# mycorrhiza-inc/fugu

Measured on AMD Instinct MI355X. Metric: queries/sec + p50 latency, 10M-doc Zipf corpus, 3-term AND, top-100, higher is better.
Workload: dtype u32+f32; 1 GPU; 3-term AND, BM25 top-100, 10M-doc Zipf s=1.0 corpus per namespace, batch 1024; n_docs=10000000, vocab=1048576, batch=1024, k=100, terms=3, namespaces=1, parallelism=namespace-shard x1

## Files before the change

fugu_amd/csrc/fg_host.h:

```cpp
#pragma once
#include <hip/hip_runtime.h>

#include <algorithm>
#include <atomic>
#include <chrono>
#include <condition_variable>
#include <functional>
#include <cstdint>
#include <map>
#include <memory>
#include <mutex>
#include <string>
#include <thread>
#include <vector>

#include "../../include/fugu.h"
#include "fg_internal.h"
#include "fg_pool.h"
#include "fg_trace.h"

namespace fgh {

int fail(int code, const char* fmt, ...);
int hw_threads(int req);
// ... 279 lines not shown

namespace fgh {
struct ChunkTables {
  const uint32_t *d_sc_tf = nullptr, *d_sc_tl = nullptr, *d_bk_tf = nullptr, *d_bk_tl = nullptr, *d_bk_e0 = nullptr,
                 *d_bk_e1 = nullptr, *d_kt_terms = nullptr, *d_kt_tiny = nullptr;
  const uint64_t *d_sc_e0 = nullptr, *d_sc_e1 = nullptr;
  uint32_t n_scb = 0, n_ktiny = 0;
  const uint32_t* d_tterm = nullptr;
  uint32_t n_tterm = 0, n_tiles = 0;
  const uint32_t *d_kb_terms = nullptr, *d_kb_chunk0 = nullptr, *d_kc_big = nullptr, *d_kc_start = nullptr;
  uint32_t n_sc = 0, n_bk = 0, n_kt = 0, n_kbig = 0, n_kchunks = 0;
};

struct IndexStructure : ChunkTables {
  uint32_t n_docs = 0, n_terms = 0;
  bool has_name = false;
  uint64_t n_postings = 0, dir_entries = 0, tile_entries = 0;
  uint32_t n_rank = 0;
  uint64_t n_srank_words = 0;
  bool has_positions = false;
  SharedVec<uint32_t> tmap;
  uint32_t n_vocab = 0;
  SharedVec<uint64_t> off;
  SharedVec<uint32_t> df_text, df_name;
  SharedVec<uint32_t> first_doc, last_doc;
  std::shared_ptr<const std::vector<uint32_t>> h_doc;
  SharedVec<uint32_t> tmeta;
  SharedVec<uint32_t> dir_off;
  uint64_t tot_local[2] = {0, 0};
  uint32_t n_fterms = 0;
  uint64_t tot_f_local = 0;
  SharedVec<uint64_t> foff;
  SharedVec<uint32_t> df_facet_local, ffirst, flast;
  std::shared_ptr<DevAllocs> smem;
  std::shared_ptr<ScorePool> spool;
  uint64_t struct_bytes = 0;
  fg::DevIndex d{};
};

struct IndexBounds {
  std::shared_ptr<ScoreBlock> sblock;
  const float* ktop = nullptr;
  const float* tmaxs = nullptr;
  SharedVec<float> wb_text, wb_name;
  float cache_b[512];
  SharedVec<uint32_t> h_alive_b;
  SharedVec<uint64_t> dtab_map;
  uint64_t dtab_bytes = 0;
  SharedVec<uint64_t> dtab8_map;
  uint64_t dtab8_bytes = 0;
  uint64_t device_bytes = 0;
};

inline uint32_t doctab_lead() {
  const char* e = getenv("FUGU_DOCTAB_LEAD");
  return e && *e ? (uint32_t)std::max(0l, atol(e)) : fg::kDocTabLead;
}

inline uint32_t doctab_slot(const IndexBounds& b, uint32_t t) {
  const auto it = std::lower_bound(b.dtab_map.begin(), b.dtab_map.end(), (uint64_t)t << 32);
  return it != b.dtab_map.end() && (uint32_t)(*it >> 32) == t ? (uint32_t)*it + 1u : 0u;
}

inline uint32_t doctab8_lead() {
  const char* e = getenv("FUGU_DOCTAB8_LEAD");
  return e && *e ? (uint32_t)std::max(0l, atol(e)) : fg::kDocTab8Lead;
}

inline bool conj_hist_thr() {
  const char* e = getenv("FUGU_CONJ_HIST_THR");
  return !(e && *e) || atol(e) != 0;
}

inline float hist_lo_div() {
  const char* e = getenv("FUGU_HIST_LO_DIV");
  const double v = e && *e ? atof(e) : 0.0;
  return v >= 1.0 ? (float)v : 256.0f;
}

inline uint32_t doctab8_slot(const IndexBounds& b, uint32_t t) {
  const auto it = std::lower_bound(b.dtab8_map.begin(), b.dtab8_map.end(), (uint64_t)t << 32);
  return it != b.dtab8_map.end() && (uint32_t)(*it >> 32) == t ? (uint32_t)*it + 1u : 0u;
}
}

struct fg_index : fgh::IndexStructure, fgh::IndexBounds {
  std::atomic<int> refs{1};
  int dev = 0;
  uint32_t n_dense = 0;
  uint64_t tot[2] = {0, 0};
  uint64_t n_stats = 0;
  float avgdl[2] = {0, 0};
  float cache[512];
  fgh::SharedVec<float> w_text, w_name;
  fgh::SharedVec<float> idf_text, idf_name;
  uint64_t tot_f = 0;
  float avgdl_f = 0.0f, cache_f1 = 0.0f;
  std::vector<uint32_t> df_facet;
  std::vector<float> fscore;
  fgh::SharedVec<uint32_t> h_alive;
  uint32_t n_dead = 0;
  bool same_stats = true;
  double cup[2] = {1, 1}, cdn[2] = {1, 1};
  std::shared_ptr<void> alive_hold;
  std::shared_ptr<const std::vector<float>> kth_floor;
  DevAllocs mem;
  std::shared_ptr<WsPool> pool;
  std::shared_ptr<PinnedPool> pinned;
};

struct fg_plan {
  fg_index* ix = nullptr;
  uint32_t nq = 0, k = 0, total_chunks = 0, n_scan = 0, nq_batch = 0, n_segs = 1;
  std::vector<fg_index*> segs;
  int mode = FG_MODE_AND;
  fg::DevPlan d{};
  fg::DevIndex d0{};
  void* ws = nullptr;
  size_t ws_got = 0;
  float* own_score = nullptr;
  uint32_t* own_doc = nullptr;
  uint32_t* own_n = nullptr;
  void* zero_region = nullptr;
  size_t zero_bytes = 0;
  size_t diag_words = 0;
  uint64_t ws_bytes = 0;
  DevAllocs mem;
  hipStream_t last_stream = nullptr;
  bool profile = false;
  std::vector<hipEvent_t> pending;
  double ms[2] = {0, 0};
  uint32_t n_prof = 0;
  ~fg_plan() {
    for (hipEvent_t e : pending) (void)hipEventDestroy(e);
    if (pin) {
      (void)hipSetDevice(ix->dev);
      (void)hipStreamSynchronize(up_stream);
    }
    if (ws) {
      if (last_stream_used) {
        (void)hipSetDevice(ix->dev);
        (void)hipStreamSynchronize(last_stream);
      }
      if (pin) ix->pinned->put(pin, pin_n);
      ix->pool->put(ws, ws_got);
    }
    if (!ipc_maps.empty()) {
      (void)hipSetDevice(ix->dev);
      for (void* m : ipc_maps) (void)hipIpcCloseMemHandle(m);
    }
    if (ix) fg_index_release(ix);
    for (fg_index* x : segs) fg_index_release(x);
  }
  bool last_stream_used = false;
  std::vector<uint32_t> h_lo, h_hi;
  std::vector<uint8_t> h_any;
  double part_next = 0.0;
  bool zeroed = false;
  void* pin = nullptr;
  size_t pin_n = 0;
  std::vector<void*> ipc_maps;
  hipStream_t up_stream = hipStreamPerThread;
};

extern "C" int fg_plan_seed_thr0(fg_plan* p, const float* score, uint32_t n);

namespace fgh {
inline uint32_t local_term(const fg_index* ix, uint32_t t) {
  if (ix->tmap.empty()) return t;
  const auto it = std::lower_bound(ix->tmap.begin(), ix->tmap.end(), t);
  return it != ix->tmap.end() && *it == t ? (uint32_t)(it - ix->tmap.begin()) : 0xFFFFFFFFu;
}
void term_ratio(const fg_index* ix, uint32_t t, float* rdn, float* rup);
float term_max_now(const fg_index* ix, uint32_t t);
float term_max_scaled(const fg_index* ix, uint32_t t, float rup);
float term_kth_now(const fg_index* ix, uint32_t t, uint32_t k, bool with_floor);

struct Bins { uint32_t lo, hi, shift; };
Bins union_bins(uint32_t lo, uint32_t hi);
int plan_create_multi(fg_index* const* ixs, uint32_t n_segs, const fg_query_batch* q, uint32_t k, fg_plan** out,
                      bool sync, hipStream_t up);
void run_parallel(uint32_t n, const std::function<void(uint32_t)>& f);

hipStream_t build_stream();
bool on_background();
uint32_t bg_grid_cap(int dev);
uint8_t fieldnorm_id(uint64_t n);
void bm25_weights(uint64_t Ns, const uint32_t* df_t, const uint32_t* df_n, uint32_t V, std::vector<float>& wt,
                  std::vector<float>& wn, std::vector<float>& it, std::vector<float>& in);
void set_stats(fg_index* ix, uint64_t Ns, const uint64_t tot2[2], const uint32_t* df_t, const uint32_t* df_n,
               uint64_t tot_f, const uint32_t* df_f, const Weights* wts);
void relate_stats(fg_index* ix);
int dev_upload_bytes(DevAllocs& m, const void* src, size_t n, void** out, uint64_t* bytes);
template <class T>
int dev_upload(DevAllocs& m, const T* src, size_t n, T** out, uint64_t* bytes) {
  return dev_upload_bytes(m, src, n * sizeof(T), reinterpret_cast<void**>(out), bytes);
}
struct UploadBatch {
  struct E { const void* src; size_t bytes; void** out; };
  std::vector<E> es;
  size_t total = 0;
  static size_t slot(size_t bytes) { return (std::max<size_t>(bytes, 16) + 16 + 255) & ~size_t(255); }
  template <class T>
  void add(const T* src, size_t n, T** out) {
    es.push_back(E{src, n * sizeof(T), reinterpret_cast<void**>(out)});
    total += slot(n * sizeof(T));
  }
  int commit(DevAllocs& m, uint64_t* bytes);
};
struct BuildTrace {
  bool on = false;
  std::chrono::steady_clock::time_point t;
  void start();
  void mark(const char* what);
};
extern thread_local BuildTrace g_bt;
}
```

fugu_amd/csrc/fg_internal.h:

```cpp
#pragma once
#include <algorithm>
#include <cstdint>
#include <initializer_list>

#include <hip/hip_runtime.h>

namespace fg {

constexpr uint32_t kBlock = 128;
#ifndef FG_BUCKET
#define FG_BUCKET 4
#endif
constexpr uint32_t kBucketTarget = FG_BUCKET;
constexpr uint32_t kThreads = 256;
#ifndef FG_ITEMS
#define FG_ITEMS 8
#endif
constexpr uint32_t kItems = FG_ITEMS;
constexpr uint32_t kChunk = kThreads * kItems;
constexpr uint32_t kWaveSpan = kChunk / 4;
constexpr uint32_t kMaxTerms = 16;
constexpr uint32_t kMaxK = 1024;
#ifndef FG_FINALCAP
#define FG_FINALCAP 4096
#endif
constexpr uint32_t kFinalCap = FG_FINALCAP;
static_assert(FG_FINALCAP >= 1024, "the final sort runs in place for up to kMaxK keys");
#ifndef FG_RANK_DIV
#define FG_RANK_DIV 16384
#endif
#ifndef FG_RANK_GIB
#define FG_RANK_GIB 64
#endif
constexpr uint32_t kRankDiv = FG_RANK_DIV;
constexpr uint64_t kRankBudget = (uint64_t)FG_RANK_GIB << 30;
#ifndef FG_RANK_FACTOR
#define FG_RANK_FACTOR 4.0
#endif
constexpr double kRankFactor = FG_RANK_FACTOR;
#ifndef FG_RANK_PLAIN_DIV
#define FG_RANK_PLAIN_DIV 32
#endif
constexpr uint32_t kRankPlainDiv = FG_RANK_PLAIN_DIV;
constexpr uint32_t kMaxDense = 32767;
#ifndef FG_DOCTAB_DIV
#define FG_DOCTAB_DIV 4
#endif
#ifndef FG_DOCTAB_LEAD
#define FG_DOCTAB_LEAD 8
#endif
constexpr uint32_t kDocTabDiv = FG_DOCTAB_DIV;
constexpr uint32_t kDocTabLead = FG_DOCTAB_LEAD;
constexpr uint32_t kDocTabFrac = 8;
constexpr uint32_t kDocTabMax = 64;
constexpr uint32_t kDocTabMinDocs = 8192;
#ifndef FG_DOCTAB8_DIV
#define FG_DOCTAB8_DIV 0
#endif
#ifndef FG_DOCTAB8_LEAD
#define FG_DOCTAB8_LEAD 8
#endif
constexpr uint32_t kDocTab8Div = FG_DOCTAB8_DIV;
constexpr uint32_t kDocTab8Lead = FG_DOCTAB8_LEAD;
constexpr uint32_t kRankChunkWords = 2048;
#ifndef FG_DISJ_GPQ
#define FG_DISJ_GPQ 64
#endif
constexpr uint32_t kGroupsPerQuery = FG_DISJ_GPQ;
#ifndef FG_DISJ_SPREAD
#define FG_DISJ_SPREAD 16
#endif
constexpr uint32_t kDisjSmallSpread = FG_DISJ_SPREAD;
#ifndef FG_GPQ
#define FG_GPQ 4
#endif
constexpr uint32_t kConjGroupsPerQuery = FG_GPQ;
#ifndef FG_MAXGROUP
#define FG_MAXGROUP 16
#endif
constexpr uint32_t kMaxGroup = FG_MAXGROUP;
#ifndef FG_HIST_BITS
#define FG_HIST_BITS 10
#endif
constexpr uint32_t kHistBits = 11;
constexpr uint32_t kHistBins = 1u << kHistBits;
constexpr uint32_t kConjHistBits = FG_HIST_BITS;
#ifndef FG_TILE_SHIFT
#define FG_TILE_SHIFT 12
#endif
constexpr uint32_t kDisjTileShift = FG_TILE_SHIFT;
#ifndef FG_DISJ_ROUND
#define FG_DISJ_ROUND 512
#endif
#ifndef FG_DISJ_HBITS
#define FG_DISJ_HBITS 9
#endif
#ifndef FG_DISJ_WAVES
#define FG_DISJ_WAVES 5
#endif
#ifndef FG_DISJ_G
#define FG_DISJ_G 1
#endif
#ifndef FG_DISJ_MAXGROUP
#define FG_DISJ_MAXGROUP 32
#endif
constexpr uint32_t kDisjMaxGroup = FG_DISJ_MAXGROUP;
constexpr uint32_t kDisjMaxPairs = 256;
constexpr uint32_t kNumTopK = 5;
constexpr uint32_t kTopKs[kNumTopK] = {1, 10, 20, 100, 1000};
constexpr uint32_t kNumLadderExtra = 9;
constexpr uint32_t kLadderExtra[kNumLadderExtra] = {2, 3, 5, 13, 25, 50, 125, 250, 500};
constexpr uint32_t kNumLadder = kNumTopK + kNumLadderExtra;
constexpr uint32_t kLadderKs[kNumLadder] = {1, 2, 3, 5, 10, 13, 20, 25, 50, 100, 125, 250, 500, 1000};

constexpr uint32_t kPhraseMaxGroup = 4;
constexpr uint32_t kMaxFacetClauses = 8;
constexpr uint32_t kFmaskChunk = 8192;
constexpr uint32_t kScanMaxGroup = 32;

constexpr uint32_t kModeAnd = 0;
constexpr uint32_t kModeOr = 1;

constexpr uint32_t kQBins = 512;

__host__ __device__ inline uint32_t qbin(uint64_t key, uint32_t lo, uint32_t sh) {
  const uint32_t bits = (uint32_t)(key >> 32);
  if (bits < lo) return kQBins;
  const uint32_t b = (bits - lo) >> sh;
  return b < kQBins - 1 ? b : kQBins - 1;
}

__host__ __device__ inline uint64_t hist_kth_edge(const uint32_t* c, uint32_t n, uint32_t first, uint32_t before,
                                                  uint32_t K, uint32_t lo, uint32_t sh) {
  for (uint32_t i = 0; i < n; ++i) {
    if (before < K && before + c[i] >= K) return (uint64_t)(lo + ((first - i) << sh)) << 32;
    before += c[i];
  }
  return 0ull;
}

__host__ __device__ inline uint32_t qm_terms(uint32_t qm) { return qm & 0xFFu; }
__host__ __device__ inline uint32_t qm_must(uint32_t qm) { return (qm >> 8) & 0xFFu; }
__host__ __device__ inline uint32_t qm_not(uint32_t qm) { return (qm >> 16) & 0xFFu; }
__host__ __device__ inline uint32_t qm_pack(uint32_t m, uint32_t nm, uint32_t nx) { return m | (nm << 8) | (nx << 16); }
__host__ __device__ inline uint32_t qm_phrase(uint32_t distinct, uint32_t n) { return distinct | (n << 24); }
__host__ __device__ inline uint32_t qm_phrase_terms(uint32_t qm) { return qm >> 24; }

__host__ __device__ inline uint32_t rank_word(uint32_t d) { return d >> 5; }
__host__ __device__ inline uint32_t rank_pos(uint64_t x, uint32_t d) {
#if defined(__HIP_DEVICE_COMPILE__)
  asm volatile("" : "+v"(d));
#endif
  const uint32_t b = d & 31u;
  if (!((x >> b) & 1ull)) return 0xFFFFFFFFu;
  const uint32_t below = (uint32_t)x & ((1u << b) - 1u);
#if defined(__HIP_DEVICE_COMPILE__)
  return (uint32_t)(x >> 32) + (uint32_t)__popc(below);
#else
  return (uint32_t)(x >> 32) + (uint32_t)__builtin_popcount(below);
#endif
}

__host__ __device__ inline uint32_t srank_block(uint32_t d) { return d >> 10; }
__host__ __device__ inline uint32_t srank_index(uint64_t e, uint32_t d) {
#if defined(__HIP_DEVICE_COMPILE__)
  asm volatile("" : "+v"(d));
#endif
  const uint32_t w = (d >> 5) & 31u;
  const uint32_t below = (uint32_t)e & ((1u << w) - 1u);
#if defined(__HIP_DEVICE_COMPILE__)
  const uint32_t i = (uint32_t)(e >> 32) + (uint32_t)__popc(below);
#else
  const uint32_t i = (uint32_t)(e >> 32) + (uint32_t)__builtin_popcount(below);
#endif
  return ((e >> w) & 1ull) ? i : 0u;
}

__host__ __device__ inline float q8_step(float M) { return M * (1.0f / 255.0f); }
__host__ __device__ inline float q8_bound(uint32_t q, float M) { return q >= 255u ? M : (float)q * q8_step(M); }
__host__ __device__ inline uint32_t quant8(float s, float M) {
  const float st = q8_step(M);
  if (!(st > 0.0f) || !(s < M)) return 255u;
  uint32_t q = (uint32_t)fminf(254.0f, ceilf(s / st));
  while (q < 255u && q8_bound(q, M) < s) ++q;
  return q;
}
constexpr uint32_t kSubShift = 9;

__host__ __device__ inline uint32_t meta_slot(uint32_t meta) { return (meta >> 16) & 0x7FFFu; }
__host__ __device__ inline bool meta_rank(uint32_t meta) { return (meta >> 31) != 0; }

constexpr uint32_t kTfEsc = 255;
__host__ __device__ inline uint32_t tfn_pack(uint32_t tf, uint32_t fn) { return (fn << 8) | (tf < kTfEsc ? tf : kTfEsc); }
struct DevIndex {
  const uint32_t* doc;
  const float* psc;
  const uint16_t* tfn;
  const uint16_t* tfn_name;
  const uint64_t* esc_pos;
  const uint32_t* esc_tf;
  const float* cache;
  const uint64_t* off;
  const uint32_t* dir;
  const uint32_t* dir_off;
  const uint32_t* tmeta;
  const uint64_t* rank;
  const uint64_t* srank;
  const uint64_t* srank_w;
  const float* tmaxs;
  const uint32_t* alive;
  const float* bmax;
  const float* tmax;
  const uint32_t* toff;
  const uint32_t* tdir;
  const uint64_t* tsub;
  const float* cmax;
  const uint32_t* coff;
  const float* dtab;
  const uint8_t* dtab8;
  const uint32_t* fdoc;
  const uint64_t* foff;
  uint64_t n_esc;
  uint32_t n_docs;
  uint32_t n_terms;
  uint32_t has_name;
  uint32_t n_fterms;
  uint32_t rank_words;
  uint32_t n_prank;
  uint32_t srank_blocks;
  uint32_t dtab_stride;
  uint32_t dtab8_stride;
  const uint64_t* fwd_off;
  const uint32_t* fwd;
  const uint64_t* fwd_off_name;
  const uint32_t* fwd_name;
};
constexpr uint32_t kFwdNone = 0xFFFFFFFFu;

__host__ __device__ inline uint32_t tf_escaped(const uint64_t* esc_pos, const uint32_t* esc_tf, uint64_t n, uint64_t p) {
  uint64_t lo = 0, hi = n;
  while (lo < hi) {
    const uint64_t mid = (lo + hi) >> 1;
    if (esc_pos[mid] < p) lo = mid + 1; else hi = mid;
  }
  return lo < n ? esc_tf[lo] : 0u;
}

__host__ __device__ inline float field_score(uint32_t tf, uint32_t fn, float w, const float* cache) {
  const float f = (float)tf;
  return w * (f / (f + cache[fn]));
}

struct ProbeDesc {
  uint32_t base_lo;
  uint32_t bytes;
  uint32_t sc_lo;
  uint32_t sc_bytes;
  uint32_t aux_lo;
  uint32_t hi;
  uint32_t kind;
  uint32_t ub;
};
static_assert(sizeof(ProbeDesc) == 32, "one s_load_dwordx8");
constexpr uint32_t kPdDir = 1u << 12;
constexpr uint32_t kPdWide = 1u << 13;
constexpr uint32_t kPdSparse = 1u << 14;
constexpr uint32_t kPdTab = 1u << 15;
constexpr uint32_t kPdBound = 1u << 6;
constexpr uint32_t kPdMaxBytes = 0x80000000u;
constexpr uint32_t kPdDead8 = 0xFFFFFFF8u, kPdDead4 = 0xFFFFFFFCu, kPdDead2 = 0xFFFFFFFEu;
// ... 30 lines not shown
  if (lead) {
    base = (uint64_t)(uintptr_t)(ix.doc + t.off);
    bytes = df * 4;
    kind = 0;
  } else if (!qt && t.tab && ix.dtab && probe_uses_table(ix.n_docs, df, lead_df, tab_lead)) {
    base = (uint64_t)(uintptr_t)(ix.dtab + (uint64_t)(t.tab - 1) * ix.dtab_stride);
    bytes = (uint64_t)ix.n_docs * 4;
    kind = kPdTab;
  } else if (slot && slot <= ix.n_prank) {
    base = (uint64_t)(uintptr_t)(ix.rank + (uint64_t)(slot - 1) * ix.rank_words);
    bytes = (uint64_t)ix.rank_words * 8;
    kind = 5u;
  } else if (slot) {
    base = (uint64_t)(uintptr_t)(ix.srank + (uint64_t)(slot - 1 - ix.n_prank) * ix.srank_blocks);
    bytes = (uint64_t)ix.srank_blocks * 8;
    kind = 10u | kPdSparse;
  } else {
    const uint32_t B = t.meta & 0xFFu, S = (t.meta >> 8) & 0xFFu;
    base = (uint64_t)(uintptr_t)(ix.dir + t.dir_off);
    bytes = ((((uint64_t)(ix.n_docs ? ix.n_docs - 1 : 0)) >> B) + 2) * 4;
    aux = (uint64_t)(uintptr_t)(ix.doc + t.off);
    kind = (B & 0x3Fu) | ((S & 0x3Fu) << 6) | kPdDir;
  }
  const bool tab = (kind & kPdTab) != 0;
  const uint64_t sc = tab ? base : qt ? (uint64_t)(uintptr_t)(ix.tfn + t.off) : (uint64_t)(uintptr_t)(ix.psc + t.off);
  const uint64_t sc_bytes = tab ? bytes : df * (qt ? 2 : 4);
  if (bytes > kPdMaxBytes || sc_bytes > kPdMaxBytes) kind |= kPdWide;
  ProbeDesc p;
  p.base_lo = (uint32_t)base;
  p.bytes = (uint32_t)std::min<uint64_t>(bytes, 0xFFFFFFFFull);
  p.sc_lo = (uint32_t)sc;
  p.sc_bytes = (uint32_t)std::min<uint64_t>(sc_bytes, 0xFFFFFFFFull);
  p.aux_lo = (uint32_t)aux;
  p.hi = (uint32_t)((base >> 32) & 0xFFFFu) | (uint32_t)((sc >> 32) & 0xFFFFu) << 16;
  p.kind = kind | (uint32_t)((aux >> 32) & 0xFFFFu) << 16;
  union { float f; uint32_t u; } c;
  c.f = ub;
  p.ub = c.u;
  return p;
}

inline bool probe_uses_bound(uint64_t n_docs, uint64_t df, uint64_t lead_df, uint32_t tab8_lead) {
  return lead_df * 128 >= n_docs * tab8_lead || df * 2 >= n_docs;
}

inline bool probe_desc_bound(const DevIndex& ix, ProbeDesc& lead, ProbeDesc& p1, uint32_t tab8, float M, bool deferred,
                             bool qt, uint64_t df, uint64_t lead_df, uint32_t tab8_lead = kDocTab8Lead) {
  if (!deferred || qt || !tab8 || !ix.dtab8 || !(M > 0.0f)) return false;
  if (p1.kind & (kPdDir | kPdWide)) return false;
  if (!probe_uses_bound(ix.n_docs, df, lead_df, tab8_lead)) return false;
  const uint64_t a = (uint64_t)(uintptr_t)(ix.dtab8 + (uint64_t)(tab8 - 1) * ix.dtab8_stride);
  p1.aux_lo = (uint32_t)a;
  p1.kind = (p1.kind & 0xFFFFu) | kPdBound | (uint32_t)((a >> 32) & 0xFFFFu) << 16;
  union { float f; uint32_t u; } c;
  c.f = M;
  lead.aux_lo = c.u;
  return true;
}

struct DevFilters {
  uint32_t n_filters;
  uint32_t n_chunks;
  const uint32_t* q_filter;
  const uint32_t* f_shift;
  const uint64_t* f_woff;
  const float* f_tab;
  const float* f_max;
  const uint32_t* ch_filter;
  const uint32_t* ch_clause;
  const uint32_t* ch_term;
  const uint32_t* ch_start;
  const uint32_t* f_seg;
  uint32_t* fmask;
};

__host__ __device__ inline uint32_t filter_bits(const uint32_t* mask, uint32_t shift, uint32_t d) {
  const uint32_t bit = d << shift;
  return (mask[bit >> 5] >> (bit & 31)) & ((1u << (1u << shift)) - 1u);
}

constexpr uint32_t kMaxPeers = 15;
constexpr uint32_t kOptConjHistThr = 1u;

struct DevPlan {
  uint32_t n_queries;
  uint32_t total_chunks;
  uint32_t k;
  uint32_t n_conj;
  const uint32_t* q_m;
  const uint32_t* q_terms;
  const uint32_t* q_lead_df;
  const uint32_t* work_q;
  const uint32_t* work_c;
  const uint32_t* work_n;
  const uint64_t* cand_off;
  const uint64_t* q_thr0;
  const float* q_ub;
  const ProbeDesc* q_probe;
  const float* q_wt;
  const float* q_wn;
  const float* q_rup;
  const uint32_t* q_hlo;
  const uint32_t* q_hsh;
  uint64_t* thresh;
  uint32_t* hist;
  uint64_t pub_mask;
  uint32_t* cand_cnt;
  uint64_t* cand_keys;
  uint64_t* diag;
  uint32_t feat;
  uint32_t opts;
  uint32_t n_single;
  uint32_t n_scan;
  uint32_t n_phrase;
  const uint32_t* q_pterm;
  const uint32_t* q_ppos;
  const DevIndex* segs;
  uint32_t seg_nq;
  uint32_t n_segs;
  const uint32_t* seg_base;
  DevFilters f;
  uint32_t n_peers;
  uint32_t* peer_hist[kMaxPeers];
  uint64_t* peer_thr[kMaxPeers];
};

__host__ __device__ inline uint32_t slot_query(const DevPlan& pl, uint32_t v) {
  return pl.seg_nq ? v % pl.seg_nq : v;
}

constexpr uint32_t kCountItems = 8;
constexpr uint32_t kCountChunk = kThreads * kCountItems;
constexpr uint32_t kCountFacetChunk = kFmaskChunk;
constexpr uint32_t kCountFacetItems = kCountFacetChunk / kThreads;
constexpr uint32_t kCountWordChunk = 2048;
constexpr uint32_t kCountTile = 64;
constexpr uint32_t kCountText = 0, kCountFacet = 1, kCountFill = 2;
struct DevCount {
  uint32_t nq;
  uint32_t q0;
  uint32_t words;
  uint32_t n_count;
  uint32_t n_fchunks, n_items, n_cchunks;
  uint32_t* match;
  uint32_t* fbits;
  unsigned long long* total;
  unsigned long long* count;
  const uint32_t* fc_filter;
  const uint32_t* fc_term;
  const uint32_t* fc_start;
  const uint32_t* w_q;
  const uint32_t* w_kind;
  const uint32_t* w_term;
  const uint32_t* w_start;
  const uint32_t* q_m;
  const uint32_t* q_terms;
  const uint32_t* q_filter;
  const uint32_t* cc_j;
  const uint32_t* cc_term;
  const uint32_t* cc_start;
};

constexpr uint32_t kDiagPerWg = 16;

__host__ __device__ inline uint64_t make_key(float score, uint32_t doc) {
  union { float f; uint32_t u; } c;
  c.f = score;
  return ((uint64_t)c.u << 32) | (uint64_t)(0xFFFFFFFFu - doc);
}
__host__ __device__ inline float key_score(uint64_t k) {
  union { float f; uint32_t u; } c;
  c.u = (uint32_t)(k >> 32);
  return c.f;
}
__host__ __device__ inline uint32_t key_doc(uint64_t k) { return 0xFFFFFFFFu - (uint32_t)k; }

constexpr uint32_t kScoreChunk = kChunk;
constexpr uint32_t kBucketChunk = 2048;
static_assert(kScoreChunk == kChunk, "DevIndex::cmax: a k_score chunk is a k_conj lead chunk");
struct ScoreJob {
  const uint32_t* doc;
  const uint16_t* tfn;
  const uint16_t* tfn_name;
  const uint64_t* esc_pos;
  const uint32_t* esc_tf;
  uint64_t n_esc;
  const uint64_t* off;
  const uint32_t* dir;
  const uint32_t* dir_off;
  const uint32_t* tmeta;
  const uint32_t* toff;
  const uint32_t* alive;
  const float* w_text;
  const float* w_name;
  const float* cache;
  float* psc;
  float* bmax;
// ... 12 lines not shown
  const uint64_t* sc_e0;
  const uint64_t* sc_e1;
  const uint32_t* bk_tf;
  const uint32_t* bk_tl;
  const uint32_t* bk_e0;
  const uint32_t* bk_e1;
  uint32_t n_terms;
  uint32_t grid_cap;
  uint64_t n_dir;
  const uint32_t* kt_tiny;
  uint32_t n_tiny;
  const uint32_t* kt_terms;
  const uint32_t* kb_terms;
  const uint32_t* kb_chunk0;
  const uint32_t* kc_big;
  const uint32_t* kc_start;
  uint64_t* kc_keys;
  uint32_t* kc_cnt;
  uint32_t* kb_stat;
  uint32_t n_big;
};
#ifndef FG_KTOP_CHUNK
#define FG_KTOP_CHUNK 32768
#endif
constexpr uint32_t kKtopChunk = FG_KTOP_CHUNK;
constexpr uint32_t kKtopTiny = 64;
constexpr uint32_t kPackTerms = 256;

struct DocTabJob {
  const uint32_t* doc;
  const float* psc;
  float* tab;
  uint64_t stride;
  uint32_t n;
  uint32_t df[kDocTabMax];
  uint64_t off[kDocTabMax];
};

struct DocTab8Job {
  const uint32_t* doc;
  const float* psc;
  const float* tmaxs;
  uint8_t* tab;
  uint64_t stride;
  uint32_t n;
  uint32_t term[kDocTabMax];
  uint32_t df[kDocTabMax];
  uint64_t off[kDocTabMax];
};

constexpr uint32_t kFwdSlices = 1024;
constexpr uint32_t kFwdShort = 16;
constexpr uint32_t kFwdErrOrder = 1u;
constexpr uint32_t kFwdErrNone = 2u;
constexpr uint32_t kFwdErrRow = 4u;
struct FwdJob {
  const uint32_t* doc;
  const uint64_t* off;
  const uint16_t* tf;
  const uint32_t* pos;
  uint64_t* poff;
  uint32_t* len;
  uint64_t* part;
  uint32_t* err;
  unsigned long long* filled;
  uint64_t* fwd_off;
  uint32_t* fwd;
  uint64_t n_fwd;
  uint64_t n_post;
  uint32_t n_docs;
  const uint32_t* sc_tf;
  const uint32_t* sc_tl;
  const uint64_t* sc_e0;
  const uint64_t* sc_e1;
  uint32_t n_chunks;
  uint32_t grid_cap;
};
hipError_t launch_fwd_rows(const FwdJob& j, hipStream_t s, hipEvent_t* ev = nullptr);
hipError_t launch_fwd_fill(const FwdJob& j, hipStream_t s, hipEvent_t* ev = nullptr);

hipError_t launch_conj(const DevIndex& ix, const DevPlan& pl, hipStream_t s);
hipError_t launch_disj(const DevIndex& ix, const DevPlan& pl, hipStream_t s, uint32_t first = 0,
                       uint32_t count = 0xFFFFFFFFu);
hipError_t launch_fmask(const DevIndex& ix, const DevPlan& pl, hipStream_t s);
hipError_t launch_scan(const DevIndex& ix, const DevPlan& pl, hipStream_t s);
hipError_t launch_phrase(const DevIndex& ix, const DevPlan& pl, hipStream_t s);
hipError_t launch_final(const DevPlan& pl, float* out_score, uint32_t* out_doc, uint32_t* out_n, hipStream_t s,
                        uint32_t* out_shard = nullptr);
hipError_t launch_count(const DevIndex& ix, const DevCount& c, hipStream_t s, hipEvent_t* ev = nullptr);
hipError_t launch_rank(const uint32_t* doc, const uint64_t* slot_base, const uint32_t* slot_n, uint32_t n_slots,
                       uint32_t n_words, uint64_t* out, hipStream_t s);
hipError_t launch_score(const ScoreJob& j, uint32_t n_chunks, hipStream_t s);
hipError_t launch_doctab(const DocTabJob& j, uint32_t grid_cap, hipStream_t s);
hipError_t launch_doctab8(const DocTab8Job& j, uint32_t grid_cap, hipStream_t s);
hipError_t launch_bucket(const ScoreJob& j, uint32_t n_chunks, uint32_t n_docs, hipStream_t s);
hipError_t launch_tsub(const ScoreJob& j, uint32_t n_docs, hipStream_t s);
hipError_t launch_ktop(const ScoreJob& j, uint32_t n_terms, uint32_t n_chunks, uint32_t n_big, hipStream_t s);
hipError_t launch_copy32(uint32_t* dst, const uint32_t* src, uint64_t n, uint32_t grid_cap, hipStream_t s);
hipError_t launch_merge(uint32_t n_shards, uint32_t n_queries, uint32_t k, const float* score, const uint32_t* doc,
                        const uint32_t* n, float* out_score, uint32_t* out_doc, uint32_t* out_shard, uint32_t* out_n,
                        hipStream_t s);

}
```

fugu_amd/csrc/fugu.cpp:

```cpp
#include <hip/hip_runtime.h>
#include <sched.h>

#include <algorithm>
#include <atomic>
#include <chrono>
#include <cmath>
#include <condition_variable>
#include <deque>
#include <functional>
#include <cstdarg>
#include <cstdio>
#include <cstring>
#include <map>
#include <memory>
#include <mutex>
#include <string>
#include <thread>
#include <vector>

#include "../../include/fugu.h"
#include "fg_host.h"
#include "fg_internal.h"

namespace {
// ... 665 lines not shown
  for (uint32_t s = 0; s < n_shards; ++s)
    if (!ladders[s]) return fail(FG_EINVAL, "NULL ladder of shard %u", s);
  constexpr uint32_t L = fg::kNumLadder;
  fgh::parallel_dynamic(n_terms, fgh::hw_threads(0), 8192, [&](int, uint32_t b, uint32_t e) {
    std::vector<std::pair<float, uint32_t>> c;
    std::vector<uint32_t> cur(n_shards);
    for (uint32_t t = b; t < e; ++t) {
      c.clear();
      for (uint32_t s = 0; s < n_shards; ++s)
        for (uint32_t l = 0; l < L; ++l) {
          const float v = ladders[s][(size_t)t * L + l];
          if (v > 0.0f) c.emplace_back(v, s * L + l);
        }
      std::sort(c.begin(), c.end(), [](const auto& x, const auto& y) { return x.first > y.first; });
      std::fill(cur.begin(), cur.end(), 0u);
      uint64_t total = 0;
      float res[fg::kNumTopK] = {0, 0, 0, 0, 0};
      uint32_t next = 0;
      for (size_t i = 0; i < c.size() && next < fg::kNumTopK;) {
        const float x = c[i].first;
        for (; i < c.size() && c[i].first == x; ++i) {
          const uint32_t s = c[i].second / L, K = fg::kLadderKs[c[i].second % L];
          if (K > cur[s]) {
            total += K - cur[s];
            cur[s] = K;
          }
        }
        for (; next < fg::kNumTopK && total >= fg::kTopKs[next]; ++next) res[next] = x;
      }
      for (uint32_t k = 0; k < fg::kNumTopK; ++k) out[(size_t)t * fg::kNumTopK + k] = res[k];
    }
  });
  return FG_OK;
}

int fg_index_set_kth_floor(fg_index* ix, const float* floor, uint32_t n_terms) {
  if (!ix) return fail(FG_EINVAL, "NULL index");
  std::shared_ptr<const std::vector<float>> f;
  if (floor) {
    if (n_terms != ix->n_vocab) return fail(FG_EINVAL, "floor of %u terms for a snapshot of %u", n_terms, ix->n_vocab);
    if (ix->tmap.empty()) {
      f = std::make_shared<const std::vector<float>>(floor, floor + (size_t)n_terms * fg::kNumTopK);
    } else {
      std::vector<float> v((size_t)ix->n_terms * fg::kNumTopK);
      for (uint32_t t = 0; t < ix->n_terms; ++t)
        std::copy(floor + (size_t)ix->tmap[t] * fg::kNumTopK, floor + (size_t)(ix->tmap[t] + 1) * fg::kNumTopK,
                  v.begin() + (size_t)t * fg::kNumTopK);
      f = std::make_shared<const std::vector<float>>(std::move(v));
    }
  }
  std::atomic_store(&ix->kth_floor, f);
  return FG_OK;
}

int fg_index_bm25(const fg_index* ix, uint32_t term, float* w_text, float* w_name, float* cache512) {
  if (!ix) return fail(FG_EINVAL, "NULL index");
  term = fgh::local_term(ix, term);
  if (term < ix->n_terms) {
    if (w_text) *w_text = ix->w_text[term];
    if (w_name) *w_name = ix->w_name[term];
  } else {
    if (w_text) *w_text = bm25_weight(0, ix->n_stats);
    if (w_name) *w_name = bm25_weight(0, ix->n_stats);
  }
  if (cache512) std::memcpy(cache512, ix->cache, sizeof ix->cache);
  return FG_OK;
}

static int execute_impl(fg_plan* p, hipStream_t s, float* os, uint32_t* od, uint32_t* on, uint32_t* oshard,
                        double from = 0.0, double to = 1.0) {
  HIPCHK(hipSetDevice(p->ix->dev));
  const bool first = from <= 0.0, last = to >= 1.0;
  if (first && !p->d.n_peers) {
    if (p->zeroed) p->zeroed = false;
    else HIPCHK(hipMemsetAsync(p->zero_region, 0, p->zero_bytes, s));
  }
  hipEvent_t ev[3] = {};
  if (p->profile) {
    for (auto& e : ev) HIPCHK(hipEventCreate(&e));
    HIPCHK(hipEventRecord(ev[0], s));
  }
  if (first && p->d.f.n_chunks) HIPCHK(fg::launch_fmask(p->d0, p->d, s));
  if (first && p->d.n_conj) HIPCHK(fg::launch_conj(p->d0, p->d, s));
  const uint32_t nd = p->d.total_chunks - p->d.n_conj;
  const uint32_t a = first ? 0u : (uint32_t)std::min<double>(nd, std::llround(from * nd));
  const uint32_t b = last ? nd : (uint32_t)std::min<double>(nd, std::llround(to * nd));
  if (b > a) HIPCHK(fg::launch_disj(p->d0, p->d, s, a, b - a));
  if (last && p->d.n_scan) HIPCHK(fg::launch_scan(p->d0, p->d, s));
  if (last && p->d.n_phrase) HIPCHK(fg::launch_phrase(p->d0, p->d, s));
  if (p->profile) HIPCHK(hipEventRecord(ev[1], s));
  if (last) HIPCHK(fg::launch_final(p->d, os, od, on, s, oshard));
  if (p->profile) {
    HIPCHK(hipEventRecord(ev[2], s));
    p->pending.insert(p->pending.end(), ev, ev + 3);
  }
  p->last_stream = s;
  p->last_stream_used = true;
  return FG_OK;
}

int fg_plan_execute(fg_plan* p, void* stream, float* d_out_score, uint32_t* d_out_doc, uint32_t* d_out_n) {
  if (!p) return fail(FG_EINVAL, "NULL plan");
  return execute_impl(p, static_cast<hipStream_t>(stream), d_out_score ? d_out_score : p->own_score,
                      d_out_doc ? d_out_doc : p->own_doc, d_out_n ? d_out_n : p->own_n, nullptr);
}

int fg_plan_execute_merged(fg_plan* p, void* stream, float* d_out_score, uint32_t* d_out_doc, uint32_t* d_out_shard,
                           uint32_t* d_out_n) {
  if (!p || !d_out_score || !d_out_doc || !d_out_shard || !d_out_n) return fail(FG_EINVAL, "bad arguments");
  if (p->n_segs < 2 || !p->d.seg_base)
    return fail(FG_EUNSUPPORTED, "not a multi-snapshot plan over < 2^32 docs (use fg_plan_execute + fg_merge_shards)");
  return execute_impl(p, static_cast<hipStream_t>(stream), d_out_score, d_out_doc, d_out_n, d_out_shard);
}

int fg_plan_execute_part(fg_plan* p, void* stream, double from, double to, float* d_out_score, uint32_t* d_out_doc,
                         uint32_t* d_out_shard, uint32_t* d_out_n) {
  if (!p) return fail(FG_EINVAL, "NULL plan");
  if (!(from >= 0.0 && from < to && to <= 1.0)) return fail(FG_EINVAL, "part [%g, %g) not inside [0, 1)", from, to);
  if (from > 0.0 && from != p->part_next)
    return fail(FG_EINVAL, "part [%g, %g) does not continue the plan's sweep (next part starts at %g)", from, to,
                p->part_next);
  if (d_out_shard && (p->n_segs < 2 || !p->d.seg_base))
    return fail(FG_EUNSUPPORTED, "merged select: not a multi-snapshot plan over < 2^32 docs");
  if (d_out_shard && (!d_out_score || !d_out_doc || !d_out_n)) return fail(FG_EINVAL, "merged select needs every output");
  const int rc = execute_impl(p, static_cast<hipStream_t>(stream), d_out_score ? d_out_score : p->own_score,
                              d_out_doc ? d_out_doc : p->own_doc, d_out_n ? d_out_n : p->own_n, d_out_shard, from, to);
  if (rc == FG_OK) p->part_next = to >= 1.0 ? 0.0 : to;
  return rc;
}

int fg_plan_set_peers(fg_plan* p, fg_plan* const* peers, uint32_t n) {
  if (!p || (n && !peers)) return fail(FG_EINVAL, "bad arguments");
  if (n > FG_MAX_PEERS) return fail(FG_EUNSUPPORTED, "%u peers (> FG_MAX_PEERS = %d)", n, FG_MAX_PEERS);
  for (uint32_t i = 0; i < n; ++i) {
    const fg_plan* o = peers[i];
    if (!o || o == p) return fail(FG_EINVAL, "peer %u: NULL or the plan itself", i);
    if (o->nq_batch != p->nq_batch || o->k != p->k) return fail(FG_EINVAL, "peer %u plans another batch or k", i);
    if (o->h_lo.size() != p->h_lo.size()) return fail(FG_EINVAL, "peer %u: another number of query slots", i);
    if (o->ix->dev != p->ix->dev) {
      int ok = 0;
      HIPCHK(hipDeviceCanAccessPeer(&ok, p->ix->dev, o->ix->dev));
      if (!ok) return fail(FG_EUNSUPPORTED, "device %d cannot reach peer %u's device %d", p->ix->dev, i, o->ix->dev);
    }
  }
  p->d.n_peers = n;
  for (uint32_t i = 0; i < n; ++i) {
    p->d.peer_hist[i] = peers[i]->d.hist;
    p->d.peer_thr[i] = peers[i]->d.thresh;
  }
  if (n) p->d.pub_mask = 0xFFFFFFFF00000000ull;
  return FG_OK;
}

int fg_plan_ipc_export(const fg_plan* p, fg_plan_ipc* out) {
  if (!p || !out) return fail(FG_EINVAL, "bad arguments");
  const char* ws = static_cast<const char*>(p->ws);
  const char* th = reinterpret_cast<const char*>(p->d.thresh);
  const char* hi = reinterpret_cast<const char*>(p->d.hist);
  if (th < ws || th >= ws + p->ws_got || hi < ws || hi >= ws + p->ws_got)
    return fail(FG_EUNSUPPORTED, "the plan's thresholds are another plan's (linked): export that plan");
  std::memset(out, 0, sizeof *out);
  hipIpcMemHandle_t h;
  HIPCHK(hipSetDevice(p->ix->dev));
  HIPCHK(hipIpcGetMemHandle(&h, p->ws));
  static_assert(sizeof h <= sizeof out->handle, "fg_plan_ipc::handle");
  std::memcpy(out->handle, &h, sizeof h);
// ... 82 lines not shown
}

int fg_plan_hist_copy(fg_plan* p, void* stream, uint32_t* d_buf, int into_plan) {
  if (!p || !d_buf) return fail(FG_EINVAL, "bad arguments");
  HIPCHK(hipSetDevice(p->ix->dev));
  const size_t bytes = 4ull * p->nq_batch * fg::kQBins;
  hipStream_t s = static_cast<hipStream_t>(stream);
  if (into_plan) HIPCHK(hipMemcpyAsync(p->d.hist, d_buf, bytes, hipMemcpyDeviceToDevice, s));
  else HIPCHK(hipMemcpyAsync(d_buf, p->d.hist, bytes, hipMemcpyDeviceToDevice, s));
  return FG_OK;
}

int fg_plan_results(fg_plan* p, float* out_score, uint32_t* out_doc, uint32_t* out_n) {
  if (!p) return fail(FG_EINVAL, "NULL plan");
  HIPCHK(hipSetDevice(p->ix->dev));
  const size_t nk = (size_t)p->nq * p->k;
  hipStream_t s = p->last_stream;
  const char* first = reinterpret_cast<const char*>(p->own_score);
  const size_t span = reinterpret_cast<const char*>(p->own_n) + 4ull * p->nq - first;
  if (span <= (4ull << 20)) {
    PinnedLease pin(*p->ix->pinned, span);
    if (pin.p) {
      HIPCHK(hipMemcpyAsync(pin.p, first, span, hipMemcpyDeviceToHost, s));
      HIPCHK(hipStreamSynchronize(s));
      const char* h = static_cast<const char*>(pin.p);
      if (out_score) std::memcpy(out_score, h, 4 * nk);
      if (out_doc) std::memcpy(out_doc, h + (reinterpret_cast<const char*>(p->own_doc) - first), 4 * nk);
      if (out_n) std::memcpy(out_n, h + (reinterpret_cast<const char*>(p->own_n) - first), 4ull * p->nq);
      return FG_OK;
    }
  }
  if (out_score) HIPCHK(hipMemcpyAsync(out_score, p->own_score, 4 * nk, hipMemcpyDeviceToHost, s));
  if (out_doc) HIPCHK(hipMemcpyAsync(out_doc, p->own_doc, 4 * nk, hipMemcpyDeviceToHost, s));
  if (out_n) HIPCHK(hipMemcpyAsync(out_n, p->own_n, 4ull * p->nq, hipMemcpyDeviceToHost, s));
  HIPCHK(hipStreamSynchronize(s));
  return FG_OK;
}

int fg_plan_info_get(const fg_plan* p, fg_plan_info* o) {
  if (!p || !o) return fail(FG_EINVAL, "bad arguments");
  o->n_queries = p->nq;
  o->k = p->k;
  o->total_chunks = p->total_chunks;
  o->workspace_bytes = p->ws_bytes;
  return FG_OK;
}

int fg_plan_profile(fg_plan* p, int enable) {
  if (!p) return fail(FG_EINVAL, "NULL plan");
  p->profile = enable != 0;
  return FG_OK;
}

int fg_plan_kernel_ms(fg_plan* p, double* ms_out, uint32_t* n_out) {
  if (!p) return fail(FG_EINVAL, "NULL plan");
  HIPCHK(hipSetDevice(p->ix->dev));
  for (size_t i = 0; i + 2 < p->pending.size(); i += 3) {
    HIPCHK(hipEventSynchronize(p->pending[i + 2]));
    for (int kx = 0; kx < 2; ++kx) {
      float ms = 0;
      HIPCHK(hipEventElapsedTime(&ms, p->pending[i + kx], p->pending[i + kx + 1]));
      p->ms[kx] += ms;
    }
    p->n_prof++;
  }
  for (hipEvent_t e : p->pending) (void)hipEventDestroy(e);
  p->pending.clear();
  if (ms_out) for (int kx = 0; kx < 2; ++kx) ms_out[kx] = p->ms[kx];
  if (n_out) *n_out = p->n_prof;
  p->ms[0] = p->ms[1] = 0;
  p->n_prof = 0;
  return FG_OK;
}

int fg_plan_diag(fg_plan* p, uint64_t* out, size_t n_words, uint32_t* cand_cnt) {
  if (!p) return fail(FG_EINVAL, "NULL plan");
  HIPCHK(hipSetDevice(p->ix->dev));
  HIPCHK(hipStreamSynchronize(p->last_stream));
  if (cand_cnt) HIPCHK(hipMemcpy(cand_cnt, p->d.cand_cnt, 4ull * p->nq, hipMemcpyDeviceToHost));
  if (out && n_words) {
    if (!p->d.diag) return fail(FG_EUNSUPPORTED, "not a diagnostic build (-DFG_DIAG)");
    HIPCHK(hipMemcpy(out, p->d.diag, 8 * std::min(n_words, p->diag_words), hipMemcpyDeviceToHost));
  }
  return FG_OK;
}

int fg_plan_seed_thr0(fg_plan* p, const float* score, uint32_t n) {
  if (!p || !score || n != p->nq_batch) return fail(FG_EINVAL, "bad arguments");
  std::vector<uint64_t> t((size_t)p->nq);
  for (uint32_t v = 0; v < p->nq; ++v) {
    const float s = score[v % p->nq_batch];
    t[v] = s > 0.0f ? fg::make_key(s, 0xFFFFFFFFu) : 0ull;
  }
  HIPCHK(hipSetDevice(p->ix->dev));
  if (p->pin) HIPCHK(hipStreamSynchronize(p->up_stream));
  if (p->last_stream_used) HIPCHK(hipStreamSynchronize(p->last_stream));
  if (p->nq) HIPCHK(hipMemcpy(const_cast<uint64_t*>(p->d.q_thr0), t.data(), 8ull * p->nq, hipMemcpyHostToDevice));
  return FG_OK;
}

int fg_plan_destroy(fg_plan* p) {
  delete p;
  return FG_OK;
}

int fg_plan_link(fg_plan* const* plans, uint32_t n) {
  if (!plans || n == 0) return fail(FG_EINVAL, "bad arguments");
  fg_plan* o = plans[0];
  for (uint32_t i = 0; i < n; ++i) {
    if (!plans[i]) return fail(FG_EINVAL, "NULL plan");
    if (plans[i]->nq != o->nq || plans[i]->k != o->k) return fail(FG_EINVAL, "linked plans differ in batch or k");
    if (plans[i]->ix->dev != o->ix->dev) return fail(FG_EINVAL, "linked plans live on different devices");
    if (plans[i]->n_segs > 1) return fail(FG_EUNSUPPORTED, "a multi-snapshot plan already shares its thresholds");
  }
  const uint32_t nq = o->nq;
  std::vector<uint32_t> lo(nq, 0), sh(nq, 0);
  for (uint32_t q = 0; q < nq; ++q) {
    uint32_t l = 0, h = 0;
    for (uint32_t i = 0; i < n; ++i) {
      l = std::max(l, plans[i]->h_lo[q]);
      h = std::max(h, plans[i]->h_hi[q]);
    }
    const fgh::Bins b = fgh::union_bins(l, h);
    lo[q] = b.lo;
    sh[q] = b.shift;
  }
  HIPCHK(hipSetDevice(o->ix->dev));
  for (uint32_t i = 0; i < n; ++i) {
    fg_plan* p = plans[i];
    if (nq) {
      HIPCHK(hipMemcpy(const_cast<uint32_t*>(p->d.q_hlo), lo.data(), 4ull * nq, hipMemcpyHostToDevice));
      HIPCHK(hipMemcpy(const_cast<uint32_t*>(p->d.q_hsh), sh.data(), 4ull * nq, hipMemcpyHostToDevice));
    }
    p->h_lo = lo;
    for (uint32_t q = 0; q < nq; ++q) p->h_hi[q] = std::max(p->h_hi[q], lo[q]);
    p->d.thresh = o->d.thresh;
    p->d.hist = o->d.hist;
    p->d.pub_mask = 0xFFFFFFFF00000000ull;
  }
  return FG_OK;
}

int fg_search_batch(fg_index* ix, const fg_query_batch* q, uint32_t k, float* out_score, uint32_t* out_doc,
                    uint32_t* out_n) {
  fg_plan* p = nullptr;
  int rc = plan_create_multi(&ix, 1, q, k, &p, false, hipStreamPerThread);
  if (rc) return rc;
  std::unique_ptr<fg_plan> guard(p);
  if ((rc = fg_plan_execute(p, hipStreamPerThread, nullptr, nullptr, nullptr))) return rc;
  return fg_plan_results(p, out_score, out_doc, out_n);
}

int fg_merge_shards(uint32_t n_shards, uint32_t n_queries, uint32_t k, const float* d_score, const uint32_t* d_doc,
                    const uint32_t* d_n, float* d_out_score, uint32_t* d_out_doc, uint32_t* d_out_shard,
                    uint32_t* d_out_n, void* stream) {
  if (n_shards == 0 || n_shards > 64 || k == 0 || !d_score || !d_doc || !d_n || !d_out_score || !d_out_doc || !d_out_n)
    return fail(FG_EINVAL, "bad arguments");
  HIPCHK(fg::launch_merge(n_shards, n_queries, k, d_score, d_doc, d_n, d_out_score, d_out_doc, d_out_shard, d_out_n,
                          static_cast<hipStream_t>(stream)));
  return FG_OK;
}

class ShardWorkers {
 public:
  static ShardWorkers& get() {
    static ShardWorkers* w = new ShardWorkers(std::max(8, std::min(64, hw_threads(0))));
// ... 257 lines not shown
```

fugu_amd/csrc/kernels.hip:

```cpp
#include <hip/hip_runtime.h>

#include "fg_internal.h"

namespace fg {
namespace {

constexpr uint32_t kInvalid = 0xFFFFFFFFu;

#ifdef FG_DIAG
#define FG_STAMP(base, slot, val)                                     \
  do {                                                                \
    if (threadIdx.x == 0 && pl.diag) pl.diag[(base) * kDiagPerWg + (slot)] = (val); \
  } while (0)
#define FG_NOW() __builtin_amdgcn_s_memrealtime()
#else
#define FG_STAMP(base, slot, val) do { } while (0)
#define FG_NOW() 0ull
#endif

__device__ inline uint32_t lane_id() { return threadIdx.x & 63; }

typedef const __attribute__((address_space(4))) DevIndex ConstDevIndex;
__device__ inline DevIndex seg_index(const DevPlan& pl, uint32_t s) {
#if defined(__HIP_DEVICE_COMPILE__)
  return ((ConstDevIndex*)pl.segs)[s];
#else
  return pl.segs[s];
#endif
}
__device__ inline uint32_t wave_id() { return threadIdx.x >> 6; }

typedef const __attribute__((address_space(4))) ProbeDesc ConstProbeDesc;
__device__ inline ProbeDesc probe_load(const ProbeDesc* p) {
#if defined(__HIP_DEVICE_COMPILE__)
  return *(ConstProbeDesc*)(uintptr_t)p;
#else
  return *p;
#endif
}
#if defined(__HIP_DEVICE_COMPILE__)
typedef __amdgpu_buffer_rsrc_t BufRsrc;
__device__ inline BufRsrc pd_rsrc(uint64_t base, uint32_t bytes) {
  return __builtin_amdgcn_make_buffer_rsrc((void*)(uintptr_t)base, 0, (int)bytes, 0x00020000);
}
__device__ inline uint64_t buf_u64(BufRsrc r, uint32_t off) {
  const auto v = __builtin_amdgcn_raw_buffer_load_b64(r, (int)off, 0, 0);
  return (uint64_t)v[0] | ((uint64_t)v[1] << 32);
}
__device__ inline uint32_t buf_u32(BufRsrc r, uint32_t off) { return __builtin_amdgcn_raw_buffer_load_b32(r, (int)off, 0, 0); }
__device__ inline uint32_t buf_u16(BufRsrc r, uint32_t off) { return __builtin_amdgcn_raw_buffer_load_b16(r, (int)off, 0, 0); }
__device__ inline uint32_t buf_u8(BufRsrc r, uint32_t off) { return __builtin_amdgcn_raw_buffer_load_b8(r, (int)off, 0, 0); }
#else
typedef int BufRsrc;
__device__ inline BufRsrc pd_rsrc(uint64_t, uint32_t) { return 0; }
__device__ inline uint64_t buf_u64(BufRsrc, uint32_t) { return 0; }
__device__ inline uint32_t buf_u32(BufRsrc, uint32_t) { return 0; }
__device__ inline uint32_t buf_u16(BufRsrc, uint32_t) { return 0; }
__device__ inline uint32_t buf_u8(BufRsrc, uint32_t) { return 0; }
#endif

template <uint32_t N>
__device__ inline void loads_in_flight(uint32_t (&v)[N]) {
#if defined(__HIP_DEVICE_COMPILE__)
  if constexpr (N == 8)
    asm volatile("" : "+v"(v[0]), "+v"(v[1]), "+v"(v[2]), "+v"(v[3]), "+v"(v[4]), "+v"(v[5]), "+v"(v[6]), "+v"(v[7]));
  else if constexpr (N == 4)
    asm volatile("" : "+v"(v[0]), "+v"(v[1]), "+v"(v[2]), "+v"(v[3]));
#endif
}

__device__ inline float inflate_bound(float x) { return x * 1.00000762939453125f; }

__device__ inline uint64_t rank_word_of(const DevIndex& ix, uint32_t slot, uint32_t d) {
  if (slot <= ix.n_prank) return ix.rank[(size_t)(slot - 1) * ix.rank_words + rank_word(d)];
  return ix.srank_w[srank_index(ix.srank[(size_t)(slot - 1 - ix.n_prank) * ix.srank_blocks + srank_block(d)], d)];
}
__device__ inline const uint64_t* rank_base(const DevIndex& ix, uint32_t slot, uint32_t& shift) {
  if (slot <= ix.n_prank) {
    shift = 5u;
    return ix.rank + (size_t)(slot - 1) * ix.rank_words;
  }
  shift = 10u;
  return ix.srank + (size_t)(slot - 1 - ix.n_prank) * ix.srank_blocks;
}


constexpr uint32_t kFName = 1, kFEsc = 2, kFQt = 4;
template <uint32_t kF>
__device__ inline uint32_t tfn_load(const DevIndex& ix, uint64_t p) {
  uint32_t v = ix.tfn[p];
  if ((kF & kFName) && ix.tfn_name) v |= (uint32_t)ix.tfn_name[p] << 16;
  return v;
}
template <uint32_t kF>
__device__ inline float tfn_score_fast(uint32_t v, float wt, float wn, const float* ct, const float* cn) {
  const uint32_t tt = v & 0xFFu, tn = (kF & kFName) ? (v >> 16) & 0xFFu : 0u;
  float s = 0.0f;
  if (tt) s += field_score(tt, (v >> 8) & 0xFFu, wt, ct);
  if (tn) s += field_score(tn, v >> 24, wn, cn);
  return s;
}
template <uint32_t kF>
__device__ inline bool tfn_escaped(uint32_t v) {
  return (kF & kFEsc) && ((v & 0xFFu) == kTfEsc || ((v >> 16) & 0xFFu) == kTfEsc);
}
__device__ inline float tfn_score(const DevIndex& ix, uint64_t p, uint32_t v, float wt, float wn, const float* ct,
                                  const float* cn) {
  uint32_t tt = v & 0xFFu, tn = (v >> 16) & 0xFFu;
  if (tt == kTfEsc || tn == kTfEsc) {
    const uint32_t e = tf_escaped(ix.esc_pos, ix.esc_tf, ix.n_esc, p);
    if (tt == kTfEsc) tt = e & 0xFFFFu;
    if (tn == kTfEsc) tn = e >> 16;
  }
  float s = 0.0f;
  if (tt) s += field_score(tt, (v >> 8) & 0xFFu, wt, ct);
  if (tn) s += field_score(tn, v >> 24, wn, cn);
  return s;
}

__device__ inline float term_bound(const DevIndex& ix, uint32_t meta, uint32_t toff, uint32_t dir_off, uint32_t d) {
  return toff != 0xFFFFFFFFu ? ix.tmax[toff + (d >> kDisjTileShift)] : ix.bmax[dir_off + (d >> (meta & 0xFFu))];
}

__device__ inline bool term_has_doc(const DevIndex& ix, uint32_t meta, uint64_t base, uint32_t dir_off, uint32_t d) {
  const uint32_t slot = meta_slot(meta);
  if (slot) return (rank_word_of(ix, slot, d) >> (d & 31u)) & 1ull;
  const uint32_t* __restrict__ dir = ix.dir + dir_off;
  const uint32_t b = d >> (meta & 0xFFu);
  uint32_t lo = dir[b], hi = dir[b + 1];
  const uint32_t* __restrict__ di = ix.doc + base;
  while (lo < hi) {
    const uint32_t mid = (lo + hi) >> 1;
    if (di[mid] < d) lo = mid + 1; else hi = mid;
  }
  return lo < dir[b + 1] && di[lo] == d;
}

__device__ inline uint32_t posting_pos(const DevIndex& ix, uint32_t t, uint32_t d) {
  const uint32_t meta = ix.tmeta[t], slot = meta_slot(meta);
// ... 675 lines not shown
      bool keep = (live >> j) & 1u;
      uint64_t key = 0;
      if (keep && ix.alive && !((ix.alive[doc[j] >> 5] >> (doc[j] & 31)) & 1u)) keep = false;
      if (keep) {
        float s = (nm == 1 && !has_opt) ? s0[j] : s0[j] + acc_o[j];
        if (fmask) s = s + ftab[filter_bits(fmask, fshift, doc[j])];
        key = make_key(s, doc[j]);
        keep = key >= thr;
      }
      wave_append(keep, key, sh.buf, &sh.n_buf, kBuf);
    }
    }
    __syncthreads();
    uint32_t n = sh.n_buf;
    uint64_t tp2 = FG_NOW();
    (void)tp2;
    if (defer) {
      const uint32_t nd = min(sh.n_dq, kDeferCap);
      if (nd >= kDeferFlush || (cc + 1 == nc && nd > 0)) {
        if (n > kTrunc) {
          local_T = truncate_topk(sh, n, K);
          if (local_T > thr_k) thr_k = local_T;
        }
        flush_deferred<kF>(ix, sh, probes, terms, qwt, qwn, m, thr_k, nd);
        __syncthreads();
        n = sh.n_buf;
        if (tid == 0) sh.n_dq = 0;
      }
    }
    if (n > kTrunc || (cc + 1 == nc && n > K)) {
      local_T = truncate_topk(sh, n, K);
      if (local_T > thr_k) thr_k = local_T;
    }
    uint64_t tp3 = FG_NOW();
    (void)tp3;
#ifdef FG_DIAG
    t_probe += tp1 - tp0; t_keys += tp2 - tp1; t_sel += tp3 - tp2; n_app += n;
#endif
    if (tid == 0) {
      if (local_T > sh.thr) sh.thr = local_T;
      pend = atomicMax(gthr, (unsigned long long)(local_T & pl.pub_mask));
    }
  }
  if (tid == 0 && pend > sh.thr) sh.thr = pend;
  {
    static_assert((1u << kConjHistBits) >= kQBins, "LDS bins");
    const uint32_t n = min(sh.n_buf, kBuf);
    for (uint32_t b = tid; b < kQBins; b += kThreads) sh.hist[b] = 0;
    __syncthreads();
    for (uint32_t i = tid; i < n; i += kThreads) {
      const uint32_t b = qbin(sh.buf[i], h_lo, h_sh);
      if (b < kQBins) atomicAdd(&sh.hist[b], 1u);
    }
    __syncthreads();
    if (!kSingle && (pl.opts & kOptConjHistThr)) {
      const uint64_t cur = sh.thr;
      const uint32_t cb = qbin(cur, h_lo, h_sh);
      const uint64_t edge = hist_add_kth(sh.hist, gh, pl, ql, cur && cb < kQBins ? cb : 0u, K, h_lo, h_sh, sh.scratch);
      if (tid == 0 && edge > cur) {
        sh.thr = edge;
        atomicMax(gthr, (unsigned long long)(edge & pl.pub_mask));
      }
    } else {
      hist_add(sh.hist, gh, pl, ql);
    }
  }
  if (tid == 0) peer_thr_max(pl, ql, sh.thr);
  __syncthreads();

  const uint32_t total = flush_candidates(pl, q, sh.buf, sh.n_buf, sh.thr, sh.scratch);
  (void)total;
  FG_STAMP(w, 0, t_start);
  FG_STAMP(w, 1, t_probe);
  FG_STAMP(w, 2, t_keys);
  FG_STAMP(w, 3, t_sel);
  FG_STAMP(w, 4, FG_NOW());
  FG_STAMP(w, 5, n_app);
  FG_STAMP(w, 6, ((uint64_t)nc << 40) | ((uint64_t)m << 32) | q);
  FG_STAMP(w, 7, total);
#ifdef FG_DIAG
  __syncthreads();
  for (uint32_t i = 0; i < 8; ++i) FG_STAMP(w, 8 + i, sh.dgc[i]);
#endif
}

constexpr uint32_t kTileShift = kDisjTileShift;
constexpr uint32_t kTile = 1u << kTileShift;
constexpr uint32_t kRound = FG_DISJ_ROUND;
constexpr uint32_t kBufD = kTrunc + kRound;
constexpr uint32_t kPairs = kRound;
constexpr uint32_t kQCap = 2 * kRound;
constexpr uint32_t kDisjHistBits = FG_DISJ_HBITS;
constexpr uint32_t kMaxTiles = kDisjMaxGroup;
constexpr uint32_t kMaxSeg = kDisjMaxPairs;
static_assert(kMaxSeg <= 2 * kThreads, "k_disj segment list: two (tile, clause) pairs per thread");
static_assert(kMaxTiles <= 255 && kMaxTerms <= 16, "seg_info packs (tile << 4) | clause; cand (tile << 8) | clause");

template <bool kQt>
struct DisjQt {
  float c_wt[kMaxTerms], c_wn[kMaxTerms];
  float cache[256];
};
template <>
struct DisjQt<false> {};

template <bool kQt>
struct DisjShared : DisjQt<kQt> {
  alignas(16) uint64_t buf[kBufD];
  struct {
    uint64_t q[kQCap];
    union {
      float cs[kPairs];
      uint32_t hist[1u << kDisjHistBits];
    };
    uint32_t seg_start[kMaxSeg];
  } p;
  uint32_t scratch[8];
  uint32_t r_lo[kMaxSeg];
  uint16_t r_n[kMaxSeg];
  float r_ub[kMaxSeg];
  uint16_t b_ess[kMaxTiles * 8];
  uint64_t r_sub[kMaxSeg];
  uint16_t t_ess[kMaxTiles];
  uint32_t t_post;
  uint16_t seg_info[kMaxSeg];
  uint32_t c_meta[kMaxTerms], c_dir[kMaxTerms];
  uint64_t c_base[kMaxTerms];
  float c_rup[kMaxTerms];
  uint32_t max_s, n_seg, n_post;
  uint32_t n_buf, n_cand;
  uint32_t n_q;
  uint32_t n_cnt;
  uint32_t n_lh;
  uint64_t thr;
  uint32_t lh[kQBins / 2];
};
static_assert(kMaxTiles <= 32, "DisjShared::t_post: one bit per tile");

__device__ inline void hist_add16(uint32_t* lh, uint32_t* gh, const DevPlan& pl, uint32_t ql) {
  for (uint32_t i = 0; i < pl.n_peers; ++i) {
    uint32_t* ph = pl.peer_hist[i] + (size_t)ql * kQBins;
    for (uint32_t b = threadIdx.x; b < kQBins / 2; b += kThreads)
      if (const uint32_t c = lh[b]) {
        if (c & 0xFFFFu) atomicAdd(&ph[2 * b], c & 0xFFFFu);
        if (c >> 16) atomicAdd(&ph[2 * b + 1], c >> 16);
      }
  }
  for (uint32_t b = threadIdx.x; b < kQBins / 2; b += kThreads) {
    const uint32_t c = lh[b];
    if (c) {
      if (c & 0xFFFFu) atomicAdd(&gh[2 * b], c & 0xFFFFu);
      if (c >> 16) atomicAdd(&gh[2 * b + 1], c >> 16);
      lh[b] = 0;
    }
  }
}

__device__ inline bool doc_alive(const DevIndex& ix, uint32_t d) {
  return !ix.alive || ((ix.alive[d >> 5] >> (d & 31)) & 1u);
}

__device__ inline float sub_bound(uint64_t sub, uint32_t z, float M) {
  return q8_bound((uint32_t)(sub >> (8 * z)) & 0xFFu, M);
}

struct QHist {
// ... 1129 lines not shown
    out_doc[(size_t)q * k + produced] = bd;
    if (out_shard) out_shard[(size_t)q * k + produced] = (uint32_t)best;
    head[best]++;
  }
  out_n[q] = produced;
  for (uint32_t e = produced; e < k; ++e) {
    out_score[(size_t)q * k + e] = 0.0f;
    out_doc[(size_t)q * k + e] = 0u;
    if (out_shard) out_shard[(size_t)q * k + e] = 0u;
  }
}

}

template <bool kSingle, uint32_t kF>
static void conj_launch(const DevIndex& ix, const DevPlan& pl, uint32_t grid, hipStream_t s) {
  if (pl.segs) k_conj<kSingle, true, kF><<<grid, kThreads, 0, s>>>(ix, pl);
  else k_conj<kSingle, false, kF><<<grid, kThreads, 0, s>>>(ix, pl);
}
static inline uint32_t feat_of(const DevPlan& pl) {
  return !(pl.feat & kFQt) ? 0u : (pl.feat & (kFName | kFEsc)) ? (kFQt | kFName | kFEsc) : kFQt;
}
template <bool kSingle>
static void conj_launch_f(const DevIndex& ix, const DevPlan& pl, uint32_t grid, hipStream_t s) {
  switch (feat_of(pl)) {
    case 0: conj_launch<kSingle, 0>(ix, pl, grid, s); break;
    case kFQt: conj_launch<kSingle, kFQt>(ix, pl, grid, s); break;
    default: conj_launch<kSingle, kFQt | kFName | kFEsc>(ix, pl, grid, s); break;
  }
}

hipError_t launch_conj(const DevIndex& ix, const DevPlan& pl, hipStream_t s) {
  if (pl.n_single) {
    conj_launch_f<true>(ix, pl, pl.n_single, s);
    const hipError_t e = hipGetLastError();
    if (e != hipSuccess) return e;
  }
  if (pl.n_conj > pl.n_single) conj_launch_f<false>(ix, pl, pl.n_conj - pl.n_single, s);
  return hipGetLastError();
}

template <uint32_t kF>
static void disj_launch(const DevIndex& ix, const DevPlan& pl, uint32_t grid, hipStream_t s) {
  if (pl.segs) k_disj<true, kF><<<grid, kThreads, 0, s>>>(ix, pl);
  else k_disj<false, kF><<<grid, kThreads, 0, s>>>(ix, pl);
}

hipError_t launch_disj(const DevIndex& ix, const DevPlan& pl, hipStream_t s, uint32_t first, uint32_t count) {
  const uint32_t n = pl.total_chunks > pl.n_conj ? pl.total_chunks - pl.n_conj : 0u;
  if (first >= n) return hipSuccess;
  count = min(count, n - first);
  if (!count) return hipSuccess;
  DevPlan part = pl;
  part.n_conj = pl.n_conj + first;
  switch (feat_of(pl)) {
    case 0: disj_launch<0>(ix, part, count, s); break;
    case kFQt: disj_launch<kFQt>(ix, part, count, s); break;
    default: disj_launch<kFQt | kFName | kFEsc>(ix, part, count, s); break;
  }
  return hipGetLastError();
}

hipError_t launch_fmask(const DevIndex& ix, const DevPlan& pl, hipStream_t s) {
  if (pl.f.n_chunks == 0) return hipSuccess;
  if (pl.segs) k_fmask<true><<<pl.f.n_chunks, kThreads, 0, s>>>(ix, pl);
  else k_fmask<false><<<pl.f.n_chunks, kThreads, 0, s>>>(ix, pl);
  return hipGetLastError();
}

hipError_t launch_scan(const DevIndex& ix, const DevPlan& pl, hipStream_t s) {
  if (pl.n_scan == 0) return hipSuccess;
  if (pl.segs) k_scan<true><<<pl.n_scan, kThreads, 0, s>>>(ix, pl);
  else k_scan<false><<<pl.n_scan, kThreads, 0, s>>>(ix, pl);
  return hipGetLastError();
}

hipError_t launch_phrase(const DevIndex& ix, const DevPlan& pl, hipStream_t s) {
  if (pl.n_phrase == 0) return hipSuccess;
  if (pl.segs) k_phrase<true><<<pl.n_phrase, kThreads, 0, s>>>(ix, pl);
  else k_phrase<false><<<pl.n_phrase, kThreads, 0, s>>>(ix, pl);
  return hipGetLastError();
}

hipError_t launch_final(const DevPlan& pl, float* out_score, uint32_t* out_doc, uint32_t* out_n, hipStream_t s,
                        uint32_t* out_shard) {
  const bool merged = out_shard != nullptr;
  if (merged && (!pl.seg_base || !pl.seg_nq)) return hipErrorInvalidValue;
  const uint32_t grid = merged ? pl.seg_nq : pl.n_queries;
  if (grid == 0) return hipSuccess;
  static unsigned long long attr_set[2] = {0, 0};
  int dev = 0;
  hipError_t e = hipGetDevice(&dev);
  if (e != hipSuccess) return e;
  if (dev < 64 && !((__atomic_load_n(&attr_set[merged], __ATOMIC_ACQUIRE) >> dev) & 1ull)) {
    const void* fn = merged ? reinterpret_cast<const void*>(&k_final<true>) : reinterpret_cast<const void*>(&k_final<false>);
    e = hipFuncSetAttribute(fn, hipFuncAttributeMaxDynamicSharedMemorySize, (int)kFinalLds);
    if (e != hipSuccess) return e;
    __atomic_fetch_or(&attr_set[merged], 1ull << dev, __ATOMIC_RELEASE);
  }
  if (merged) k_final<true><<<grid, kThreads, kFinalLds, s>>>(pl, out_score, out_doc, out_n, out_shard);
  else k_final<false><<<grid, kThreads, kFinalLds, s>>>(pl, out_score, out_doc, out_n, nullptr);
  return hipGetLastError();
}

__global__ __launch_bounds__(kThreads) void k_rank(const uint32_t* __restrict__ doc_all,
                                                   const uint64_t* __restrict__ slot_base,
                                                   const uint32_t* __restrict__ slot_n, uint32_t chunks_per_slot,
                                                   uint32_t n_words, uint64_t* __restrict__ out_all) {
  __shared__ uint32_t bits[kRankChunkWords];
  __shared__ uint32_t scratch[8];
  __shared__ uint32_t range[2];
  const uint32_t tid = threadIdx.x;
  const uint32_t slot = blockIdx.x / chunks_per_slot, chunk = blockIdx.x - slot * chunks_per_slot;
  const uint32_t* __restrict__ doc = doc_all + slot_base[slot];
  const uint32_t n = slot_n[slot];
  uint64_t* __restrict__ out = out_all + (size_t)slot * n_words;
  const uint32_t w0 = chunk * kRankChunkWords;
  if (tid < 2) {
    const uint64_t target = ((uint64_t)w0 + (tid ? kRankChunkWords : 0u)) << 5;
    uint32_t lo = 0, hi = n;
    while (lo < hi) {
      const uint32_t mid = lo + ((hi - lo) >> 1);
      if ((uint64_t)doc[mid] < target) lo = mid + 1; else hi = mid;
    }
    range[tid] = lo;
  }
  for (uint32_t i = tid; i < kRankChunkWords; i += kThreads) bits[i] = 0u;
  __syncthreads();
  for (uint32_t p = range[0] + tid; p < range[1]; p += kThreads) {
    const uint32_t d = doc[p];
    atomicOr(&bits[rank_word(d) - w0], 1u << (d & 31u));
  }
  __syncthreads();
  constexpr uint32_t R = kRankChunkWords / kThreads;
  uint32_t c[R], sum = 0;
#pragma unroll
  for (uint32_t i = 0; i < R; ++i) {
    c[i] = (uint32_t)__popc(bits[tid * R + i]);
    sum += c[i];
  }
  uint32_t r = range[0] + block_exclusive_scan(sum, scratch);
#pragma unroll
  for (uint32_t i = 0; i < R; ++i) {
    const uint32_t w = w0 + tid * R + i;
    if (w < n_words) out[w] = (uint64_t)bits[tid * R + i] | ((uint64_t)r << 32);
    r += c[i];
  }
}

hipError_t launch_rank(const uint32_t* doc, const uint64_t* slot_base, const uint32_t* slot_n, uint32_t n_slots,
                       uint32_t n_words, uint64_t* out, hipStream_t s) {
  if (n_words == 0 || n_slots == 0) return hipSuccess;
  const uint32_t cps = (n_words + kRankChunkWords - 1) / kRankChunkWords;
  if ((uint64_t)cps * n_slots > 0x7FFFFFFFull) return hipErrorInvalidValue;
  k_rank<<<cps * n_slots, kThreads, 0, s>>>(doc, slot_base, slot_n, cps, n_words, out);
  return hipGetLastError();
}

__global__ __launch_bounds__(kThreads) void k_dtab_fill(float* __restrict__ tab, uint64_t n) {
  for (uint64_t i = (uint64_t)blockIdx.x * kThreads + threadIdx.x; i < n; i += (uint64_t)gridDim.x * kThreads)
    tab[i] = -1.0f;
}

__global__ __launch_bounds__(kThreads) void k_dtab_scatter(DocTabJob j) {
  const uint32_t t = blockIdx.y;
  const uint64_t off = j.off[t];
// ... 874 lines not shown
```

fugu_amd/csrc/model.cpp:

```cpp
#include <algorithm>
#include <atomic>
#include <cstring>
#include <vector>

#include "../../include/fugu.h"
#include "fg_host.h"
#include "fg_internal.h"

using fgh::fail;
using fgh::hw_threads;
using fgh::parallel_dynamic;

namespace {

enum Arr : uint32_t { A_DOC, A_TFN, A_RANK, A_SRANK, A_SRANKW, A_DIR, A_BMAX, A_TMAX, A_TDIR, A_CMAX, A_TSUB, A_DTAB, A_DTAB8, A_N };
constexpr uint64_t kLine = 128;
constexpr uint32_t kTraceClauses = 4;
constexpr float kInflate = 1.00000762939453125f;

struct Snap {
  const fg_index* ix = nullptr;
  const uint32_t* doc = nullptr;
  uint32_t pw = 2;
  uint32_t tab_lead = 0;
  uint32_t tab8_lead = 0;
  std::vector<float> psc, tmax, bmax, cmax;
  std::vector<uint64_t> tsub, srank;
  std::vector<uint32_t> dir_off, toff, coff;
  uint64_t bytes[A_N] = {0};
  int load(const fg_index* x) {
    ix = x;
    doc = x->h_doc ? x->h_doc->data() : nullptr;
    const uint64_t P = x->n_postings, V = x->n_terms;
    HIPCHK(hipSetDevice(x->dev));
    psc.resize(P);
    dir_off.resize(V);
    toff.resize(V);
    coff.resize(V);
    tmax.resize(x->tile_entries);
    tsub.assign(x->d.tsub ? x->tile_entries : 0, ~0ull);
    bmax.resize(x->dir_entries);
    cmax.resize(x->n_sc);
    auto rd = [](void* dst, const void* src, size_t n) -> hipError_t {
      return n && src ? hipMemcpy(dst, src, n, hipMemcpyDeviceToHost) : hipSuccess;
    };
    {
      std::vector<uint16_t> tv(P), tn(x->d.tfn_name ? P : 0);
      std::vector<uint64_t> ep(x->d.n_esc);
      std::vector<uint32_t> et(x->d.n_esc);
      HIPCHK(rd(tv.data(), x->d.tfn, 2 * P));
      HIPCHK(rd(tn.data(), x->d.tfn_name, 2 * tn.size()));
      HIPCHK(rd(ep.data(), x->d.esc_pos, 8 * ep.size()));
      HIPCHK(rd(et.data(), x->d.esc_tf, 4 * et.size()));
      pw = x->same_stats || x->d.tfn_name ? 4 : 2;
      parallel_dynamic(x->n_terms, hw_threads(0), 256, [&](int, uint32_t b, uint32_t e) {
        for (uint32_t t = b; t < e; ++t)
          for (uint64_t p = x->off[t]; p < x->off[t + 1]; ++p) {
            const uint32_t v = tv[p] | (tn.empty() ? 0u : (uint32_t)tn[p] << 16);
            uint32_t tt = v & 0xFFu, tm = (v >> 16) & 0xFFu;
            if (tt == fg::kTfEsc || tm == fg::kTfEsc) {
              const uint32_t ex = fg::tf_escaped(ep.data(), et.data(), ep.size(), p);
              if (tt == fg::kTfEsc) tt = ex & 0xFFFFu;
              if (tm == fg::kTfEsc) tm = ex >> 16;
            }
            float sc = 0.0f;
            if (tt) sc += fg::field_score(tt, (v >> 8) & 0xFFu, x->w_text[t], x->cache);
            if (tm) sc += fg::field_score(tm, v >> 24, x->w_name[t], x->cache + 256);
            psc[p] = sc;
          }
      });
    }
    HIPCHK(rd(dir_off.data(), x->d.dir_off, 4 * V));
    HIPCHK(rd(toff.data(), x->d.toff, 4 * V));
    HIPCHK(rd(coff.data(), x->d.coff, 4 * V));
    HIPCHK(rd(tmax.data(), x->d.tmax, 4 * tmax.size()));
    HIPCHK(rd(tsub.data(), x->d.tsub, 8 * tsub.size()));
    HIPCHK(rd(bmax.data(), x->d.bmax, 4 * bmax.size()));
    HIPCHK(rd(cmax.data(), x->d.cmax, 4 * cmax.size()));
    srank.resize((uint64_t)(x->n_rank - x->d.n_prank) * x->d.srank_blocks);
    HIPCHK(rd(srank.data(), x->d.srank, 8 * srank.size()));
    if (!x->same_stats)
      parallel_dynamic(x->n_terms, hw_threads(0), 256, [&](int, uint32_t b, uint32_t e) {
        for (uint32_t t = b; t < e; ++t) {
          float rdn, rup;
          fgh::term_ratio(x, t, &rdn, &rup);
          if (rup == 1.0f) continue;
          const uint32_t d0 = dir_off[t], d1 = t + 1 < x->n_terms ? dir_off[t + 1] : (uint32_t)x->dir_entries;
          for (uint32_t i = d0; i < d1; ++i) bmax[i] *= rup;
          if (toff[t] != 0xFFFFFFFFu)
            for (uint64_t i = toff[t]; i <= toff[t] + (uint64_t)x->n_tiles; ++i) tmax[i] *= rup;
          const uint64_t nc = (len(t) + fg::kChunk - 1) / fg::kChunk;
          for (uint64_t i = 0; i < nc; ++i) cmax[coff[t] + i] *= rup;
        }
      });
    bytes[A_DOC] = 4 * P;
    bytes[A_TFN] = (uint64_t)pw * P;
    bytes[A_RANK] = 8ull * x->d.n_prank * x->d.rank_words;
    bytes[A_SRANK] = 8ull * srank.size();
    bytes[A_SRANKW] = 8ull * x->n_srank_words;
    bytes[A_DIR] = bytes[A_BMAX] = 4 * x->dir_entries;
    bytes[A_TMAX] = bytes[A_TDIR] = 4 * x->tile_entries;
    bytes[A_CMAX] = 4ull * x->n_sc;
    bytes[A_TSUB] = 8ull * tsub.size();
    bytes[A_DTAB] = x->dtab_bytes;
    tab_lead = fgh::doctab_lead();
    bytes[A_DTAB8] = x->dtab8_bytes;
    tab8_lead = fgh::doctab8_lead();
    return FG_OK;
  }
  template <class Acc>
  void rank_loads(Acc& A, uint32_t s, uint32_t slot, uint32_t d, double& cat) const {
    if (slot <= ix->d.n_prank) {
      A.gather(s, A_RANK, ((uint64_t)(slot - 1) * ix->d.rank_words + fg::rank_word(d)) * 8, 8, cat);
      return;
    }
    const uint64_t at = (uint64_t)(slot - 1 - ix->d.n_prank) * ix->d.srank_blocks + fg::srank_block(d);
    A.gather(s, A_SRANK, at * 8, 8, cat);
    const uint32_t w = fg::srank_index(srank[at], d);
    if (w != 0xFFFFFFFFu) A.gather(s, A_SRANKW, (uint64_t)w * 8, 8, cat);
  }
  uint64_t len(uint32_t t) const { return ix->off[t + 1] - ix->off[t]; }
  const uint32_t* list(uint32_t t) const { return doc + ix->off[t]; }
  uint32_t pos_ge(uint32_t t, uint64_t d) const {
    const uint32_t* l = list(t);
    const uint64_t n = len(t);
    if (d > 0xFFFFFFFFull) return (uint32_t)n;
    return (uint32_t)(std::lower_bound(l, l + n, (uint32_t)d) - l);
  }
};

struct Acc {
  std::vector<uint64_t> lines;
  std::vector<uint64_t> clines;
  bool by_clause = false;
  uint64_t last[fg::kMaxTerms + 1][A_N];
  double stream = 0, probe = 0, loads = 0;
  void reset() {
    lines.clear();
    clines.clear();
    std::memset(last, 0xFF, sizeof last);
    stream = probe = loads = 0;
  }
  void line(uint32_t s, Arr a, uint64_t l) {
    if (last[s][a] == l) return;
    last[s][a] = l;
    lines.push_back(((uint64_t)a << 56) | l);
    if (by_clause) clines.push_back(((uint64_t)std::min(s, kTraceClauses - 1) << 60) | ((uint64_t)a << 52) | l);
  }
  void gather(uint32_t s, Arr a, uint64_t at, uint32_t nb, double& cat) {
    line(s, a, at / kLine);
    if ((at + nb - 1) / kLine != at / kLine) line(s, a, (at + nb - 1) / kLine);
    cat += nb;
    loads += 1;
  }
  void range(uint32_t s, Arr a, uint64_t e0, uint64_t n, uint32_t eb, double& cat) {
    if (!n) return;
    for (uint64_t l = e0 * eb / kLine; l <= ((e0 + n) * eb - 1) / kLine; ++l) line(s, a, l);
    cat += (double)n * eb;
    loads += (double)n;
  }
};

struct Union {
  std::vector<std::atomic<uint64_t>> bm[A_N];
  void init(const Snap& s) {
    for (uint32_t a = 0; a < A_N; ++a) {
      qlines[a].store(0, std::memory_order_relaxed);
      const uint64_t words = (s.bytes[a] / kLine + 2 + 63) / 64;
      std::vector<std::atomic<uint64_t>> v(words);
      for (auto& w : v) w.store(0, std::memory_order_relaxed);
      bm[a].swap(v);
    }
  }
  std::atomic<uint64_t> qlines[A_N];
  std::vector<std::atomic<uint64_t>> cbm[kTraceClauses][A_N];
  std::atomic<uint64_t> cq[kTraceClauses][A_N];
  void init_by_clause(const Snap& s) {
    for (uint32_t c = 0; c < kTraceClauses; ++c)
      for (uint32_t a = 0; a < A_N; ++a) {
        cq[c][a].store(0, std::memory_order_relaxed);
        std::vector<std::atomic<uint64_t>> v((s.bytes[a] / kLine + 2 + 63) / 64);
        for (auto& w : v) w.store(0, std::memory_order_relaxed);
        cbm[c][a].swap(v);
      }
  }
  void add_by_clause(std::vector<uint64_t>& lines) {
    std::sort(lines.begin(), lines.end());
    lines.erase(std::unique(lines.begin(), lines.end()), lines.end());
    for (uint64_t x : lines) {
      const uint32_t c = (uint32_t)(x >> 60), a = (uint32_t)(x >> 52) & 0xFFu;
// ... 22 lines not shown
    uint64_t n = 0;
    for (const auto& w : bm[a]) n += (uint64_t)__builtin_popcountll(w.load(std::memory_order_relaxed));
    return n;
  }
  uint64_t count() const {
    uint64_t n = 0;
    for (uint32_t a = 0; a < A_N; ++a) n += count(a);
    return n;
  }
};

inline uint64_t key_of(float s, uint32_t d) { return fg::make_key(s, d); }

float probe_term(const Snap& S, Acc& A, uint32_t s, uint32_t t, uint32_t d, double& cat, uint32_t tab = 0) {
  const uint32_t meta = S.ix->tmeta[t];
  const uint32_t slot = fg::meta_slot(meta);
  const uint32_t* l = S.list(t);
  const uint64_t n = S.len(t), base = S.ix->off[t];
  if (tab) {
    A.gather(s, A_DTAB, ((uint64_t)(tab - 1) * S.ix->d.dtab_stride + d) * 4, 4, cat);
    const uint64_t p = std::lower_bound(l, l + n, d) - l;
    return p < n && l[p] == d ? S.psc[base + p] : -1.0f;
  }
  if (slot && fg::meta_rank(meta)) {
    S.rank_loads(A, s, slot, d, cat);
    const uint64_t p = std::lower_bound(l, l + n, d) - l;
    if (p < n && l[p] == d) {
      A.gather(s, A_TFN, (base + p) * S.pw, S.pw, cat);
      return S.psc[base + p];
    }
    return -1.0f;
  }
  const uint32_t B = meta & 0xFFu, St = (meta >> 8) & 0xFFu;
  const uint64_t b = d >> B;
  const uint64_t dirb = (uint64_t)S.dir_off[t] + b;
  A.gather(s, A_DIR, dirb * 4, 4, cat);
  A.gather(s, A_DIR, (dirb + 1) * 4, 4, cat);
  uint32_t pos = S.pos_ge(t, b << B);
  const uint32_t hi = S.pos_ge(t, (b + 1) << B);
  for (uint32_t st = St; st > 0; --st) {
    const uint32_t half = 1u << (st - 1), idx = pos + half - 1;
    if (idx < hi) {
      A.gather(s, A_DOC, (base + idx) * 4, 4, cat);
      if (l[idx] < d) pos += half;
    }
  }
  if (pos < hi) {
    A.gather(s, A_DOC, (base + pos) * 4, 4, cat);
    if (l[pos] == d) {
      A.gather(s, A_TFN, (base + pos) * S.pw, S.pw, cat);
      return S.psc[base + pos];
    }
  }
  return -1.0f;
}

uint64_t model_conj(const Snap& S, const uint32_t* terms, uint32_t m, bool has_thr, float thr, Acc& A) {
  const fg_index* ix = S.ix;
  const uint64_t thk = has_thr && thr > 0.0f ? key_of(thr, 0xFFFFFFFFu) : 0;
  const uint32_t t0 = terms[0];
  const uint64_t base = ix->off[t0], df = S.len(t0);
  const uint32_t* ld = S.list(t0);
  uint64_t kept = 0;
  if (m == 1) {
    const uint64_t nch = (df + fg::kChunk - 1) / fg::kChunk;
    for (uint64_t c = 0; c < nch; ++c) {
      A.gather(0, A_CMAX, ((uint64_t)S.coff[t0] + c) * 4, 4, A.stream);
      if (thk && key_of(S.cmax[S.coff[t0] + c] * kInflate, 0u) < thk) continue;
      const uint64_t p0 = c * fg::kChunk, n = std::min<uint64_t>(fg::kChunk, df - p0);
      A.range(0, A_DOC, base + p0, n, 4, A.stream);
      A.range(0, A_TFN, base + p0, n, S.pw, A.stream);
      for (uint64_t p = p0; p < p0 + n; ++p) kept += key_of(S.psc[base + p], ld[p]) >= thk ? 1 : 0;
    }
    return kept;
  }
  float qub[fg::kMaxTerms + 1] = {0};
  {
    float acc = 0.0f;
    for (uint32_t j = m; j-- > 1;) {
      acc += fgh::term_max_now(ix, terms[j]);
      qub[j] = acc;
    }
  }
  A.range(0, A_DOC, base, df, 4, A.stream);
  A.range(0, A_TFN, base, df, S.pw, A.stream);
  uint32_t tab[fg::kMaxTerms] = {0};
  if (ix->same_stats && !ix->dtab_map.empty())
    for (uint32_t j = 1; j < m; ++j) {
      const uint32_t sl = fgh::doctab_slot(*ix, terms[j]);
      if (sl && fg::probe_uses_table(ix->n_docs, S.len(terms[j]), df, S.tab_lead)) tab[j] = sl;
    }
  uint32_t tab8 = 0;
  float M8 = 0.0f;
  if (ix->same_stats && !ix->dtab8_map.empty() && m >= 3 && thk) {
    const uint32_t sl = fgh::doctab8_slot(*ix, terms[1]);
    M8 = ix->tmaxs[terms[1]];
    const uint32_t k1 = fg::meta_slot(ix->tmeta[terms[1]]) ? 0u : fg::kPdDir;
    if (sl && M8 > 0.0f && !k1 && fg::probe_uses_bound(ix->n_docs, S.len(terms[1]), df, S.tab8_lead)) tab8 = sl;
  }
  const uint32_t* l1 = m > 1 ? S.list(terms[1]) : nullptr;
  const uint64_t n1 = m > 1 ? S.len(terms[1]) : 0, base1 = m > 1 ? ix->off[terms[1]] : 0;
  uint64_t c1 = 0;
  for (uint64_t p = 0; p < df; ++p) {
    const uint32_t d = ld[p];
    float s0 = S.psc[base + p], acc = 0.0f;
    if (thk && key_of((s0 + qub[1]) * kInflate, d) < thk) continue;
    if (tab8) {
      A.gather(1, A_DTAB8, (uint64_t)(tab8 - 1) * ix->d.dtab8_stride + d, 1, A.probe);
      while (c1 < n1 && l1[c1] < d) ++c1;
      if (c1 >= n1 || l1[c1] != d) continue;
      const float bnd = fg::q8_bound(std::max(1u, fg::quant8(S.psc[base1 + c1], M8)), M8);
      if (key_of((s0 + bnd + qub[2]) * kInflate, d) < thk) continue;
    }
    bool ok = true;
    for (uint32_t j = 1; j < m && ok; ++j) {
      const float sc = probe_term(S, A, j, terms[j], d, A.probe, tab[j]);
      if (sc < 0.0f) { ok = false; break; }
      if (j == 1) s0 = s0 + sc; else acc += sc;
      if (thk && j + 1 < m && key_of((s0 + acc + qub[j + 1]) * kInflate, d) < thk) ok = false;
    }
    if (ok && key_of(s0 + acc, d) >= thk) ++kept;
  }
  return kept;
}

uint64_t model_disj(const Snap& S, const uint32_t* t, uint32_t m, float thr, Acc& A) {
  const fg_index* ix = S.ix;
  const uint32_t TS = fg::kDisjTileShift, N = ix->n_docs;
  const uint64_t thk = thr > 0.0f ? key_of(thr, 0xFFFFFFFFu) : 0;
  uint32_t dlo = 0xFFFFFFFFu, dhi = 0;
  for (uint32_t c = 0; c < m; ++c) {
    dlo = std::min(dlo, ix->first_doc[t[c]]);
    dhi = std::max(dhi, ix->last_doc[t[c]]);
  }
  uint32_t meta[fg::kMaxTerms], B[fg::kMaxTerms], St[fg::kMaxTerms];
  for (uint32_t c = 0; c < m; ++c) {
    meta[c] = ix->tmeta[t[c]];
    B[c] = meta[c] & 0xFFu;
    St[c] = (meta[c] >> 8) & 0xFFu;
  }
  uint64_t kept = 0;
  for (uint32_t ti = dlo >> TS; ti <= (dhi >> TS); ++ti) {
    const uint32_t d0 = ti << TS, d1 = std::min<uint64_t>((uint64_t)d0 + (1u << TS), N);
    uint32_t lo[fg::kMaxTerms], hi[fg::kMaxTerms];
    float ub[fg::kMaxTerms];
    for (uint32_t c = 0; c < m; ++c) {
      const uint32_t* l = S.list(t[c]);
      const uint64_t base = ix->off[t[c]], dob = S.dir_off[t[c]];
      float u;
      if (B[c] <= TS && S.toff[t[c]] != 0xFFFFFFFFu) {
        const uint64_t to = (uint64_t)S.toff[t[c]] + ti;
        A.gather(c, A_TDIR, to * 4, 4, A.stream);
        A.gather(c, A_TDIR, (to + 1) * 4, 4, A.stream);
        lo[c] = S.pos_ge(t[c], d0);
        hi[c] = S.pos_ge(t[c], d1);
        A.gather(c, A_TMAX, to * 4, 4, A.stream);
        u = S.tmax[to];
      } else if (B[c] <= TS) {
        A.gather(c, A_DIR, (dob + (d0 >> B[c])) * 4, 4, A.stream);
        A.gather(c, A_DIR, (dob + ((d1 - 1) >> B[c]) + 1) * 4, 4, A.stream);
        lo[c] = S.pos_ge(t[c], d0);
        hi[c] = S.pos_ge(t[c], d1);
        u = fgh::term_max_now(S.ix, t[c]);
      } else {
        const uint64_t b = d0 >> B[c];
        A.gather(c, A_DIR, (dob + b) * 4, 4, A.stream);
        A.gather(c, A_DIR, (dob + b + 1) * 4, 4, A.stream);
        const uint32_t p0 = S.pos_ge(t[c], b << B[c]), p1 = S.pos_ge(t[c], (b + 1) << B[c]);
        uint32_t a = p0, e = p0;
        for (uint32_t st = St[c]; st > 0; --st) {
          const uint32_t half = 1u << (st - 1), ia = a + half - 1, ie = e + half - 1;
          if (ia < p1) { A.gather(c, A_DOC, (base + ia) * 4, 4, A.stream); if (l[ia] < d0) a += half; }
          if (ie < p1) { A.gather(c, A_DOC, (base + ie) * 4, 4, A.stream); if (l[ie] < d1) e += half; }
        }
        if (a < p1) { A.gather(c, A_DOC, (base + a) * 4, 4, A.stream); if (l[a] < d0) ++a; }
        if (e < p1) { A.gather(c, A_DOC, (base + e) * 4, 4, A.stream); if (l[e] < d1) ++e; }
        lo[c] = a;
// ... 147 lines not shown
  return kept;
}

}

extern "C" {

int fg_model_batch(const fg_index* ix, const fg_query_batch* q, uint32_t k, const float* thr_score, double* per_query,
                   fg_model_out* out) {
  if (!ix || !q || !out || (q->n_queries && !q->q_off) || k == 0) return fail(FG_EINVAL, "bad arguments");
  if (q->phrase_len)
    for (uint32_t j = q->n_queries ? q->q_off[0] : 0; q->n_queries && j < q->q_off[q->n_queries]; ++j)
      if (q->phrase_len[j] != 1) return fail(FG_EINVAL, "bad query batch (the model does not cover phrase queries)");
  if (!ix->h_doc && ix->n_postings) return fail(FG_EINVAL, "index built without keep_host_postings");
  Snap S;
  if (int rc = S.load(ix)) return rc;
  Union U;
  U.init(S);
  const bool trace = getenv("FUGU_MODEL_TRACE") != nullptr;
  if (trace) U.init_by_clause(S);
  const uint32_t nq = q->n_queries;
  std::vector<double> st(nq, 0.0), pr(nq, 0.0), ou(nq, 0.0), ld(nq, 0.0), ql(nq, 0.0), kp(nq, 0.0);
  std::atomic<bool> bad{false};
  parallel_dynamic(nq, hw_threads(0), 1, [&](int, uint32_t qb, uint32_t qe) {
    Acc A;
    A.by_clause = trace;
    for (uint32_t i = qb; i < qe; ++i) {
      A.reset();
      const uint32_t b = q->q_off[i], e = q->q_off[i + 1];
      if (e < b || e - b > fg::kMaxTerms) { bad = true; return; }
      uint32_t tm[fg::kMaxTerms], ts[fg::kMaxTerms], nm = 0, ns = 0;
      bool must_missing = false, other = false;
      for (uint32_t j = b; j < e; ++j) {
        const uint32_t t = fgh::local_term(ix, q->terms[j]);
        const uint8_t oc = q->occur ? q->occur[j] : (q->mode == FG_MODE_OR ? FG_OCCUR_SHOULD : FG_OCCUR_MUST);
        const bool present = t < ix->n_terms && ix->off[t + 1] > ix->off[t];
        if (oc == FG_OCCUR_MUST) { tm[nm++] = t; must_missing |= !present; }
        else if (oc == FG_OCCUR_SHOULD) { if (present) ts[ns++] = t; }
        else other = true;
      }
      if (other || (nm && ns)) { bad = true; return; }
      if (nm == 0 && ns == 1) { tm[nm++] = ts[0]; ns = 0; }
      uint64_t kept = 0;
      const bool has_thr = thr_score != nullptr;
      const float th = has_thr ? thr_score[i] : 0.0f;
      if (nm && !must_missing) {
        struct T { uint64_t cost; uint32_t term; };
        T tc[fg::kMaxTerms];
        for (uint32_t j = 0; j < nm; ++j) tc[j] = T{(uint64_t)ix->df_text[tm[j]] + ix->df_name[tm[j]], tm[j]};
        std::stable_sort(tc, tc + nm, [](const T& x, const T& y) { return x.cost < y.cost; });
        for (uint32_t j = 0; j < nm; ++j) tm[j] = tc[j].term;
        kept = model_conj(S, tm, nm, has_thr, th, A);
      } else if (ns >= 2) {
        kept = model_disj(S, ts, ns, th, A);
      }
      st[i] = A.stream;
      pr[i] = A.probe;
      ou[i] = 8.0 * (double)std::min<uint64_t>(kept, k);
      ld[i] = A.loads;
      kp[i] = (double)kept;
      ql[i] = (double)U.add(A.lines);
      if (trace) U.add_by_clause(A.clines);
    }
  });
  if (bad) return fail(FG_EINVAL, "bad query batch (the model covers pure Must / pure Should queries)");
  std::memset(out, 0, sizeof *out);
  for (uint32_t i = 0; i < nq; ++i) {
    out->stream_bytes += st[i];
    out->probe_bytes += pr[i];
    out->output_bytes += ou[i];
    out->loads += ld[i];
    out->candidates += kp[i];
    out->query_line_bytes += (double)kLine * ql[i];
    if (per_query) {
      per_query[4ull * i] = st[i];
      per_query[4ull * i + 1] = pr[i];
      per_query[4ull * i + 2] = ou[i];
      per_query[4ull * i + 3] = st[i] + pr[i] + ou[i];
    }
  }
  out->alg_bytes = out->stream_bytes + out->probe_bytes + out->output_bytes;
  out->line_bytes = (double)kLine * (double)U.count();
  if (trace) {
    static const char* names[A_N] = {"doc", "tfn", "rank", "srank", "srankw", "dir", "bmax", "tmax", "tdir", "cmax", "tsub", "dtab", "dtab8"};
    for (uint32_t a = 0; a < A_N; ++a)
      fprintf(stderr, "[fg model] %-6s floor %8.3f GB  per-query sum %8.3f GB\n", names[a],
              (double)kLine * (double)U.count(a) * 1e-9, (double)kLine * (double)U.qlines[a].load() * 1e-9);
    for (uint32_t c = 0; c < kTraceClauses; ++c)
      for (uint32_t a = 0; a < A_N; ++a)
        if (U.cq[c][a].load())
          fprintf(stderr, "[fg model] clause %u%s %-6s floor %8.3f GB  per-query sum %8.3f GB\n", c,
                  c + 1 == kTraceClauses ? "+" : " ", names[a], (double)kLine * (double)U.count_by_clause(c, a) * 1e-9,
                  (double)kLine * (double)U.cq[c][a].load() * 1e-9);
  }
  return FG_OK;
}

int fg_bytes_model(const fg_index* ix, const fg_query_batch* q, uint32_t k, double* out) {
  if (!ix || !q || !out) return fail(FG_EINVAL, "bad arguments");
  if (q->phrase_len)
    for (uint32_t j = q->n_queries ? q->q_off[0] : 0; q->n_queries && j < q->q_off[q->n_queries]; ++j)
      if (q->phrase_len[j] != 1) return fail(FG_EINVAL, "bad query batch (the model does not cover phrase queries)");
  if (!ix->h_doc && ix->n_postings) return fail(FG_EINVAL, "index built without keep_host_postings");
  const double F = ix->has_name ? 2.0 : 1.0;
  std::vector<uint32_t> S;
  for (uint32_t i = 0; i < q->n_queries; ++i) {
    const uint32_t b = q->q_off[i], m = q->q_off[i + 1] - b;
    double* o = out + 4ull * i;
    struct L { uint64_t n, off; uint32_t pos; };
    std::vector<L> ls;
    bool missing = false;
    for (uint32_t j = 0; j < m; ++j) {
      uint32_t t = fgh::local_term(ix, q->terms[b + j]);
      if (t >= ix->n_terms || ix->off[t + 1] == ix->off[t]) { missing = true; break; }
      ls.push_back(L{ix->off[t + 1] - ix->off[t], ix->off[t], j});
    }
    if (m == 0 || missing) { o[0] = o[1] = o[2] = o[3] = 0; continue; }
    if (m == 1) {
      double df = (double)ls[0].n;
      o[0] = o[1] = 8.0 * df;
      o[2] = 8.0 * df + 8.0 * std::min<double>(df, k);
      o[3] = df;
      continue;
    }
    std::stable_sort(ls.begin(), ls.end(), [](const L& x, const L& y) { return x.n < y.n; });
    double bmerge = 0;
    for (auto& l : ls) bmerge += 8.0 * (double)l.n;
    double bskip = 8.0 * (double)ls[0].n;
    S.assign(ix->h_doc->begin() + ls[0].off, ix->h_doc->begin() + ls[0].off + ls[0].n);
    for (size_t t = 1; t < ls.size(); ++t) {
      const uint32_t* d = ix->h_doc->data() + ls[t].off;
      const uint64_t n = ls[t].n;
      uint64_t blocks = 0, lb = 0;
      int64_t last_block = -1;
      size_t keep = 0;
      for (size_t x = 0; x < S.size(); ++x) {
        lb = std::lower_bound(d + lb, d + n, S[x]) - d;
        if (lb < n) {
          int64_t blk = (int64_t)(lb / fg::kBlock);
          if (blk != last_block) { ++blocks; last_block = blk; }
          if (d[lb] == S[x]) S[keep++] = S[x];
        }
      }
      S.resize(keep);
      bskip += 1024.0 * (double)blocks + 4.0 * (double)((n + fg::kBlock - 1) / fg::kBlock);
    }
    const double ns = (double)S.size();
    o[0] = bmerge;
    o[1] = bskip;
    o[2] = std::min(bmerge, bskip) + F * ns + 8.0 * std::min<double>(ns, k);
    o[3] = ns;
  }
  return FG_OK;
}

int fg_bytes_model_gpu(const fg_index* ix, const fg_query_batch* q, uint32_t k, double* out) {
  if (!out) return fail(FG_EINVAL, "bad arguments");
  fg_model_out o;
  if (q && q->mode == FG_MODE_OR) {
    std::vector<float> zero(q->n_queries, 0.0f);
    return fg_model_batch(ix, q, k, zero.data(), out, &o);
  }
  return fg_model_batch(ix, q, k, nullptr, out, &o);
}

int fg_bytes_model_or(const fg_index* ix, const fg_query_batch* q, uint32_t k, const float* thr, double* out) {
// ... 7 lines not shown
```

fugu_amd/csrc/plan.cpp:

```cpp
#include <chrono>
#include <cstdio>
#include <cstdlib>
#include <cstring>

#include "fg_host.h"

using fgh::fail;

fgh::Bins fgh::union_bins(uint32_t lo, uint32_t hi) {
  hi = std::max(hi, lo);
  uint32_t sh = 0;
  while (sh < 31 && ((uint64_t)(hi - lo) >> sh) >= fg::kQBins - 1) ++sh;
  return Bins{lo, hi, sh};
}

namespace {

void radix_sort_hi32(std::vector<uint64_t>& a, std::vector<uint64_t>& tmp) {
  tmp.resize(a.size());
  for (int sh = 32; sh < 64; sh += 11) {
    uint32_t cnt[2049] = {0};
    for (uint64_t x : a) cnt[((x >> sh) & 2047u) + 1]++;
    for (int d = 0; d < 2048; ++d) cnt[d + 1] += cnt[d];
    for (uint64_t x : a) tmp[cnt[(x >> sh) & 2047u]++] = x;
    a.swap(tmp);
  }
}

struct WItem { double key; uint32_t q, c, n; };

struct PlanTables {
  std::vector<uint32_t> q_m, q_terms, lead, q_filter, ngroup, q_hlo, q_hhi, q_hsh;
  std::vector<uint32_t> q_pterm, q_ppos;
  std::vector<uint64_t> thr0;
  std::vector<float> q_ub, q_wt, q_wn, q_rup;
  std::vector<fg::ProbeDesc> q_probe;
  uint32_t nf = 0;
  std::vector<uint32_t> f_shift, f_seg;
  std::vector<uint64_t> f_woff;
  std::vector<float> f_tab, f_max;
  std::vector<uint32_t> ch_f, ch_c, ch_t, ch_s;
  std::vector<WItem> citems, ditems, scan, phrase, items;
  void clear() {
    auto all = [](auto&... v) { (v.clear(), ...); };
    all(q_m, q_terms, lead, q_filter, ngroup, q_hlo, q_hhi, q_hsh, thr0, q_ub, q_wt, q_wn, q_rup, f_shift, f_seg, f_woff,
        f_tab, f_max, ch_f, ch_c, ch_t, ch_s, citems, ditems, scan, phrase, items, q_pterm, q_ppos, q_probe);
    nf = 0;
  }
};

int plan_phrase(const fg_index* ix, const fg_query_batch* q, uint32_t i, uint32_t nq_size, uint32_t n_segs,
                PlanTables& h, int* phrase) {
  *phrase = 0;
  const uint32_t b = q->q_off[i], e = q->q_off[i + 1], m = e - b;
  uint32_t n_clauses = 0, n_phr = 0;
  for (uint32_t j = b; j < e;) {
    const uint32_t n = q->phrase_len[j];
    if (n == 0 || n > e - j) return fail(FG_EINVAL, "query %u: bad phrase_len at term %u", i, j - b);
    for (uint32_t x = 1; x < n; ++x)
      if (q->phrase_len[j + x] != 0) return fail(FG_EINVAL, "query %u: phrase_len inside a phrase must be 0", i);
    if (n >= 2) {
      if (q->phrase_pos[j] != 0) return fail(FG_EINVAL, "query %u: a phrase's first offset must be 0", i);
      for (uint32_t x = 1; x < n; ++x)
        if (q->phrase_pos[j + x] <= q->phrase_pos[j + x - 1])
          return fail(FG_EINVAL, "query %u: phrase offsets must increase", i);
      ++n_phr;
    }
    ++n_clauses;
    j += n;
  }
  if (!n_phr) return FG_OK;
  *phrase = 1;
  if (n_clauses > 1) return fail(FG_EUNSUPPORTED, "query %u: phrase clause beside other clauses", i);
  if (q->f_off && q->f_off[i + 1] > q->f_off[i]) return fail(FG_EUNSUPPORTED, "query %u: phrase with facet filters", i);
  if (!ix->has_positions) return fail(FG_EUNSUPPORTED, "query %u: snapshot built without positions", i);
  if (q->phrase_pos[e - 1] >= (1u << 30)) return fail(FG_EINVAL, "query %u: phrase offset too large", i);
  const uint8_t oc = q->occur ? q->occur[b] : (q->mode == FG_MODE_OR ? FG_OCCUR_SHOULD : FG_OCCUR_MUST);
  if (oc > FG_OCCUR_MUST_NOT) return fail(FG_EINVAL, "query %u: bad occur %u", i, (unsigned)oc);
  if (oc == FG_OCCUR_MUST_NOT) return FG_OK;
  uint32_t lt[fg::kMaxTerms], dist[fg::kMaxTerms], nd = 0;
  float it = 0.0f, in = 0.0f;
  for (uint32_t j = 0; j < m; ++j) {
    const uint32_t t = lt[j] = fgh::local_term(ix, q->terms[b + j]);
    if (!(t < ix->n_terms && ix->off[t + 1] > ix->off[t])) return FG_OK;
    it += ix->idf_text[t];
    in += ix->idf_name[t];
    if (std::find(dist, dist + nd, t) == dist + nd) dist[nd++] = t;
  }
  auto len = [&](uint32_t t) { return ix->off[t + 1] - ix->off[t]; };
  const uint32_t lead = *std::min_element(dist, dist + nd, [&](uint32_t x, uint32_t y) { return len(x) < len(y); });
  const size_t row = (size_t)i * fg::kMaxTerms;
  uint32_t* qt = h.q_terms.data() + row;
  qt[0] = lead;
  for (uint32_t j = 0, o = 1; j < nd; ++j)
    if (dist[j] != lead) qt[o++] = dist[j];
  const uint32_t anchor = (uint32_t)(std::find(lt, lt + m, lead) - lt);
  for (uint32_t j = 0, o = 1; j < m; ++j) {
    const uint32_t at = j == anchor ? 0 : o++;
    h.q_pterm[row + at] = q->terms[b + j];
    h.q_ppos[row + at] = q->phrase_pos[b + j];
  }
  h.q_m[i] = fg::qm_phrase(nd, m);
  h.q_wt[row] = it * (1.0f + 1.2f);
  h.q_wn[row] = in * (1.0f + 1.2f);
  const uint64_t df0 = len(lead);
  h.lead[i] = (uint32_t)df0;
  const uint32_t nch = (uint32_t)((df0 + fg::kChunk - 1) / fg::kChunk);
  if (h.phrase.size() + nch > 0x7FFFFFFFull) return fail(FG_EUNSUPPORTED, "batch too large (%zu work items)", h.phrase.size());
  const uint32_t cdiv = n_segs <= 1 ? 1u : n_segs;
  const uint32_t per_q = std::max<uint32_t>(
      1, std::min<uint32_t>(64, std::max<uint32_t>(fg::kConjGroupsPerQuery, 1024 / std::max(nq_size, 1u))) / cdiv);
  const uint32_t G = std::min<uint32_t>(fg::kPhraseMaxGroup, std::max<uint32_t>(1, (nch + per_q - 1) / per_q));
  const uint32_t ng = (nch + G - 1) / G;
  h.ngroup[i] = ng;
  for (uint32_t g = 0; g < ng; ++g) h.phrase.push_back(WItem{(g + 0.5) / ng, i, g * G, std::min(G, nch - g * G)});
  return FG_OK;
}

int plan_host(const fg_index* ix, const fg_query_batch* q, uint32_t k, uint32_t n_segs, PlanTables& h,
              uint32_t nq_size, bool qtime) {
  if (!ix || !q || (q->n_queries && !q->q_off)) return fail(FG_EINVAL, "bad arguments");
  if (q->n_queries && q->q_off[q->n_queries] > q->q_off[0] && !q->terms) return fail(FG_EINVAL, "q_off without terms");
  if (q->f_off && q->n_queries && q->f_off[q->n_queries] > q->f_off[0] && !q->f_terms)
    return fail(FG_EINVAL, "f_off without f_terms");
  if (k < 1) return fail(FG_EINVAL, "k must be >= 1 (TopDocs::with_limit asserts limit >= 1)");
  if (k > FG_MAX_K) return fail(FG_EUNSUPPORTED, "k=%u > FG_MAX_K=%d", k, FG_MAX_K);
  if (q->mode != FG_MODE_AND && q->mode != FG_MODE_OR) return fail(FG_EINVAL, "bad mode %d", q->mode);
  const uint32_t nq = q->n_queries;
  const uint64_t N = ix->n_docs;
  const bool disj = q->mode == FG_MODE_OR;
  const uint32_t tab_lead = fgh::doctab_lead(), tab8_lead = fgh::doctab8_lead();
  h.clear();
  const size_t nqt = (size_t)nq * fg::kMaxTerms;
  for (auto* v : {&h.q_m, &h.lead}) v->assign(nq, 0);
  h.q_terms.assign(nqt, 0);
  h.thr0.assign(nq, 0);
  for (auto* v : {&h.q_ub, &h.q_wt, &h.q_wn}) v->assign(nqt, 0.0f);
  h.q_rup.assign(nqt, 1.0f);
  h.q_probe.assign(nqt, fg::ProbeDesc{});
  if (q->phrase_len) {
    if (!q->phrase_pos) return fail(FG_EINVAL, "phrase_len without phrase_pos");
    h.q_pterm.assign(nqt, 0);
    h.q_ppos.assign(nqt, 0);
  }

  h.q_filter.assign(nq, 0xFFFFFFFFu);
  std::vector<std::vector<uint32_t>> flist;
  std::vector<uint8_t> q_nomatch(nq, 0);
  if (q->f_off) {
    std::map<std::vector<uint32_t>, uint32_t> fid;
    for (uint32_t i = 0; i < nq; ++i) {
      const uint32_t b = q->f_off[i], e = q->f_off[i + 1];
      if (e < b) return fail(FG_EINVAL, "f_off not monotone at query %u", i);
      if (e == b) continue;
      if (e - b > fg::kMaxFacetClauses)
        return fail(FG_EUNSUPPORTED, "query %u has %u facet clauses (> %u)", i, e - b, fg::kMaxFacetClauses);
      std::vector<uint32_t> c(q->f_terms + b, q->f_terms + e);
      bool any = false;
      for (uint32_t t : c) any |= t < ix->n_fterms && ix->df_facet[t] > 0;
      if (!any) { q_nomatch[i] = 1; continue; }
      auto it = fid.find(c);
      if (it == fid.end()) {
        it = fid.emplace(c, (uint32_t)flist.size()).first;
        flist.push_back(std::move(c));
      }
      h.q_filter[i] = it->second;
    }
  }
  const uint32_t nf = h.nf = (uint32_t)flist.size();
  h.f_shift.assign(nf, 0);
  h.f_woff.assign(nf + 1, 0);
  h.f_tab.assign((size_t)nf * 256, 0.0f);
  h.f_max.assign(nf, 0.0f);
  std::vector<uint32_t> f_lo(nf, 0xFFFFFFFFu), f_hi(nf, 0);
  for (uint32_t f = 0; f < nf; ++f) {
    const std::vector<uint32_t>& c = flist[f];
    const uint32_t n = (uint32_t)c.size();
    const uint32_t sh = n <= 1 ? 0 : n <= 2 ? 1 : n <= 4 ? 2 : 3;
    if ((N << sh) > (1ull << 32)) return fail(FG_EUNSUPPORTED, "facet mask of %u clauses too large for %llu docs", n,
                                              (unsigned long long)N);
    h.f_shift[f] = sh;
    h.f_woff[f + 1] = h.f_woff[f] + ((((N << sh) + 31) / 32 + 63) & ~63ull);
    for (uint32_t v = 0; v < (1u << n); ++v) {
      float sc = 0.0f;
      for (uint32_t i = 0; i < n; ++i)
        if ((v >> i) & 1u) sc += c[i] < ix->n_fterms ? ix->fscore[c[i]] : 0.0f;
      h.f_tab[(size_t)f * 256 + v] = sc;
      h.f_max[f] = std::max(h.f_max[f], sc);
    }
    for (uint32_t i = 0; i < n; ++i) {
      const uint32_t t = c[i];
      if (t >= ix->n_fterms || ix->df_facet[t] == 0) continue;
      f_lo[f] = std::min(f_lo[f], ix->ffirst[t]);
      f_hi[f] = std::max(f_hi[f], ix->flast[t]);
      const uint64_t df = ix->foff[t + 1] - ix->foff[t];
      for (uint64_t st = 0; st < df; st += fg::kFmaskChunk) {
        h.ch_f.push_back(f);
        h.ch_c.push_back(i);
        h.ch_t.push_back(t);
        h.ch_s.push_back((uint32_t)st);
      }
    }
  }

  const uint32_t gpq_batch =
      fg::kGroupsPerQuery * std::min<uint32_t>(fg::kDisjSmallSpread, std::max<uint32_t>(1, 256 / std::max(nq_size, 1u)));
  const uint32_t gpq = std::max<uint32_t>(1, gpq_batch / n_segs);
  const uint32_t conj_gpq = fg::kConjGroupsPerQuery, conj_maxg = fg::kMaxGroup;
  const uint32_t cdiv = n_segs <= 1 ? 1u : n_segs;
  h.ngroup.assign(nq, 0);
  for (auto* v : {&h.q_hlo, &h.q_hhi}) v->assign(nq, 0x3F800000u);
  h.q_hsh.assign(nq, 31);
  auto present = [&](uint32_t t) { return t < ix->n_terms && ix->off[t + 1] > ix->off[t]; };
  float cm[fg::kMaxTerms];
// ... 47 lines not shown
    bool must_missing = false;
    for (uint32_t j = 0; j < m; ++j) {
      const uint32_t t = fgh::local_term(ix, q->terms[b + j]);
      const uint8_t oc = q->occur ? q->occur[b + j] : (disj ? FG_OCCUR_SHOULD : FG_OCCUR_MUST);
      if (oc > FG_OCCUR_MUST_NOT) return fail(FG_EINVAL, "query %u: bad occur %u", i, (unsigned)oc);
      if (oc == FG_OCCUR_MUST) {
        tm[nm++] = t;
        must_missing |= !present(t);
      } else if (present(t)) {
        (oc == FG_OCCUR_SHOULD ? ts_[ns++] : tx[nx++]) = t;
      }
    }
    if (nm == 0 && ns == 1) {
      tm[nm++] = ts_[0];
      ns = 0;
    }
    uint32_t* qt = h.q_terms.data() + (size_t)i * fg::kMaxTerms;
    if (nm == 0) {
      if (ns == 0) continue;
      uint32_t dlo = 0xFFFFFFFFu, dhi = 0;
      for (uint32_t j = 0; j < ns; ++j) {
        qt[j] = ts_[j];
        dlo = std::min(dlo, ix->first_doc[ts_[j]]);
        dhi = std::max(dhi, ix->last_doc[ts_[j]]);
      }
      for (uint32_t j = 0; j < nx; ++j) qt[ns + j] = tx[j];
      for (uint32_t j = 0; j < ns + nx; ++j) set_clause(i, j, qt[j]);
      h.q_m[i] = fg::qm_pack(ns + nx, 0, nx);
      if (flt != 0xFFFFFFFFu) {
        dlo = std::max(dlo, f_lo[flt]);
        dhi = std::min(dhi, f_hi[flt]);
        if (dlo > dhi) continue;
      }
      if (flt == 0xFFFFFFFFu && nx == 0) {
        float v = 0.0f;
        for (uint32_t c = 0; c < ns; ++c) v = std::max(v, fgh::term_kth_now(ix, qt[c], k, true));
        if (v > 0.0f) h.thr0[i] = fg::make_key(v, 0xFFFFFFFFu);
      }
      float ub = fmx;
      for (uint32_t c = 0; c < ns; ++c) ub += cm[c];
      set_bins(i, ub);

      const uint32_t tlo = dlo >> fg::kDisjTileShift, thi = dhi >> fg::kDisjTileShift;
      const uint32_t nt = thi - tlo + 1;
      const uint32_t G = std::min<uint32_t>(std::min(fg::kDisjMaxGroup, fg::kDisjMaxPairs / ns),
                                            std::max<uint32_t>(1, (nt + gpq - 1) / gpq));
      const uint32_t ng = (nt + G - 1) / G;
      for (uint32_t g = 0; g < ng; ++g) {
        const uint32_t t0 = tlo + g * G, n = std::min(G, nt - g * G);
        const double mid = ((double)t0 + 0.5 * n) * (double)(1u << fg::kDisjTileShift) / (double)ix->n_docs;
        h.ditems.push_back(WItem{mid, i, t0, n});
      }
      h.ngroup[i] = ng;
      if (h.ditems.size() > 0x7FFFFFFFull)
        return fail(FG_EUNSUPPORTED, "batch too large (%zu work items)", h.ditems.size());
      continue;
    }
    if (must_missing) continue;
    struct T { uint64_t cost; uint32_t pos, term; };
    T tc[fg::kMaxTerms];
    for (uint32_t j = 0; j < nm; ++j) tc[j] = T{(uint64_t)ix->df_text[tm[j]] + ix->df_name[tm[j]], j, tm[j]};
    std::stable_sort(tc, tc + nm, [](const T& x, const T& y) { return x.cost < y.cost; });
    for (uint32_t j = 0; j < nm; ++j) qt[j] = tc[j].term;
    for (uint32_t j = 0; j < nx; ++j) qt[nm + j] = tx[j];
    for (uint32_t j = 0; j < ns; ++j) qt[nm + nx + j] = ts_[j];
    const uint32_t mt = nm + nx + ns;
    for (uint32_t j = 0; j < mt; ++j) set_clause(i, j, qt[j]);
    h.q_m[i] = fg::qm_pack(mt, nm, nx);
    {
      float acc = 0.0f;
      for (uint32_t j = mt; j-- > 1;) {
        if (j < nm || j >= nm + nx) acc += cm[j];
        h.q_ub[(size_t)i * fg::kMaxTerms + j] = acc;
      }
      const size_t row = (size_t)i * fg::kMaxTerms;
      const uint64_t lead_df = ix->off[qt[0] + 1] - ix->off[qt[0]];
      for (uint32_t j = 0; j < mt; ++j) {
        const uint32_t t = qt[j];
        const uint32_t tab = j && !qtime && !ix->dtab_map.empty() ? fgh::doctab_slot(*ix, t) : 0u;
        const fg::ProbeTerm pt{ix->off[t], ix->off[t + 1], ix->tmeta[t], ix->dir_off[t], tab};
        h.q_probe[row + j] =
            fg::probe_desc(ix->d, pt, j == 0, qtime, j + 1 < mt ? h.q_ub[row + j + 1] : 0.0f, lead_df, tab_lead);
      }
      if (!qtime && !ix->dtab8_map.empty() && mt >= 3 && nm == mt && flt == 0xFFFFFFFFu)
        fg::probe_desc_bound(ix->d, h.q_probe[row], h.q_probe[row + 1], fgh::doctab8_slot(*ix, qt[1]), ix->tmaxs[qt[1]],
                             true, qtime, ix->off[qt[1] + 1] - ix->off[qt[1]], lead_df, tab8_lead);
    }
    if (mt == 1 && flt == 0xFFFFFFFFu) {
      const float v = fgh::term_kth_now(ix, qt[0], k, true);
      if (v > 0.0f) h.thr0[i] = fg::make_key(v, 0xFFFFFFFFu);
    }
    {
      float ub = fmx + cm[0];
      for (uint32_t j = 1; j < mt; ++j)
        if (j < nm || j >= nm + nx) ub += cm[j];
      set_bins(i, ub, conj_lo_div);
    }
    const uint64_t df0 = ix->off[qt[0] + 1] - ix->off[qt[0]];
    h.lead[i] = (uint32_t)df0;
    const uint32_t nch = (uint32_t)((df0 + fg::kChunk - 1) / fg::kChunk);
    if (h.citems.size() + nch > 0x7FFFFFFFull)
      return fail(FG_EUNSUPPORTED, "batch too large (%zu work items)", h.citems.size());
    const uint32_t per_q =
        std::max<uint32_t>(1, std::min<uint32_t>(64, std::max<uint32_t>(conj_gpq, 1024 / std::max(nq_size, 1u))) / cdiv);
    const uint32_t G = std::min<uint32_t>(conj_maxg, std::max<uint32_t>(1, (nch + per_q - 1) / per_q));
    const uint32_t ng = (nch + G - 1) / G;
    h.ngroup[i] = ng;
    for (uint32_t g = 0; g < ng; ++g)
      h.citems.push_back(WItem{(g + 0.5) / ng, i, g * G, std::min(G, nch - g * G)});
  }
  return FG_OK;
}

struct Pieces {
  uint32_t S = 1, nq1 = 0, P = 1;
  uint32_t count() const { return S * P; }
  uint32_t begin(uint32_t r) const { return (uint32_t)((uint64_t)nq1 * r / P); }
  uint32_t slot(uint32_t pc) const { return (pc / P) * nq1 + begin(pc % P); }
};

int plan_pieces(fg_index* const* ixs, uint32_t S, const fg_query_batch* q, uint32_t k, std::vector<PlanTables>& hs,
                PlanTables& J, Pieces& pc) {
  if (!ixs || !q || S == 0 || S > FG_MAX_SEGMENTS) return fail(FG_EINVAL, "bad arguments");
  for (uint32_t s = 0; s < S; ++s) {
    if (!ixs[s]) return fail(FG_EINVAL, "NULL snapshot");
    if (ixs[s]->dev != ixs[0]->dev) return fail(FG_EINVAL, "the snapshots of one plan live on different devices");
  }
  const uint32_t nq1 = q->n_queries;
  if ((uint64_t)S * nq1 > 0x7FFFFFFFull) return fail(FG_EUNSUPPORTED, "batch too large (%u x %u query slots)", S, nq1);
  const bool par = S > 1 && nq1 >= 64;
  pc.S = S;
  pc.nq1 = nq1;
  pc.P = par ? std::max<uint32_t>(1, std::min<uint32_t>((uint32_t)fgh::hw_threads(0) / S, nq1 / 128)) : 1u;
  const uint32_t n = pc.count();
  if (hs.size() < n) hs.resize(n);
  bool qt = false;
  for (uint32_t s = 0; s < S; ++s) {
    qt |= !ixs[s]->same_stats;
    if (!fg::probe_addr_ok(ixs[s]->d)) return fail(FG_EUNSUPPORTED, "snapshot %u: device arrays above 2^47", s);
  }
  if (S == 1) return plan_host(ixs[0], q, k, S, hs[0], nq1, qt);
  J.clear();
  const size_t nq = (size_t)S * nq1, nqt = nq * fg::kMaxTerms;
  for (auto* v : {&J.q_m, &J.lead, &J.ngroup}) v->resize(nq);
  J.thr0.resize(nq);
  J.q_terms.resize(nqt);
  for (auto* v : {&J.q_ub, &J.q_wt, &J.q_wn, &J.q_rup}) v->resize(nqt);
  J.q_probe.resize(nqt);
  if (q->phrase_len)
    for (auto* v : {&J.q_pterm, &J.q_ppos}) v->resize(nqt);
  auto put_slot = [&](uint32_t p) {
    const PlanTables& h = hs[p];
    const size_t v0 = pc.slot(p), t0 = v0 * fg::kMaxTerms;
    auto cp = [](auto& dst, const auto& src, size_t at) { std::copy(src.begin(), src.end(), dst.begin() + at); };
    cp(J.q_m, h.q_m, v0); cp(J.lead, h.lead, v0); cp(J.ngroup, h.ngroup, v0); cp(J.thr0, h.thr0, v0);
    cp(J.q_terms, h.q_terms, t0);
    cp(J.q_ub, h.q_ub, t0); cp(J.q_wt, h.q_wt, t0); cp(J.q_wn, h.q_wn, t0); cp(J.q_rup, h.q_rup, t0);
    cp(J.q_probe, h.q_probe, t0);
    cp(J.q_pterm, h.q_pterm, t0); cp(J.q_ppos, h.q_ppos, t0);
  };
  if (par) {
    std::vector<int> rcs(n, FG_OK);
    std::vector<std::string> errs(n);
    fgh::run_parallel(n, [&](uint32_t p) {
      const uint32_t a = pc.begin(p % pc.P), b = pc.begin(p % pc.P + 1);
      fg_query_batch qp = *q;
      qp.n_queries = b - a;
      qp.q_off = q->q_off + a;
      if (q->f_off) qp.f_off = q->f_off + a;
      if ((rcs[p] = plan_host(ixs[p / pc.P], &qp, k, S, hs[p], nq1, qt))) errs[p] = fg_last_error();
      else put_slot(p);
    });
    for (uint32_t p = 0; p < n; ++p)
      if (rcs[p]) return fail(rcs[p], "snapshot %u: %s", p / pc.P, errs[p].c_str());
  } else {
    for (uint32_t s = 0; s < S; ++s) {
      if (int rc = plan_host(ixs[s], q, k, S, hs[s], nq1, qt)) {
        const std::string e = fg_last_error();
        return fail(rc, "snapshot %u: %s", s, e.c_str());
      }
      put_slot(s);
    }
  }
  return FG_OK;
}

PlanTables& join_pieces(const Pieces& pc, std::vector<PlanTables>& hs, PlanTables& J) {
  if (pc.S == 1) return hs[0];
  const uint32_t S = pc.S, nq1 = pc.nq1, P = pc.P;
  auto cat = [](auto& dst, const auto& src) { dst.insert(dst.end(), src.begin(), src.end()); };
  J.f_woff.push_back(0);
  for (uint32_t p = 0; p < pc.count(); ++p) {
    const PlanTables& h = hs[p];
    const uint32_t s = p / P, fb = J.nf, vb = pc.slot(p);
    for (uint32_t f : h.q_filter) J.q_filter.push_back(f == 0xFFFFFFFFu ? f : fb + f);
    cat(J.f_shift, h.f_shift); cat(J.f_tab, h.f_tab); cat(J.f_max, h.f_max);
    const uint64_t wb = J.f_woff.back();
    for (uint32_t f = 0; f < h.nf; ++f) {
      J.f_woff.push_back(wb + h.f_woff[f + 1]);
      J.f_seg.push_back(s);
    }
    for (uint32_t f : h.ch_f) J.ch_f.push_back(fb + f);
    cat(J.ch_c, h.ch_c); cat(J.ch_t, h.ch_t); cat(J.ch_s, h.ch_s);
    for (WItem x : h.citems) { x.q += vb; J.citems.push_back(x); }
    for (WItem x : h.ditems) { x.q += vb; J.ditems.push_back(x); }
    for (WItem x : h.scan) { x.q += vb; J.scan.push_back(x); }
    for (WItem x : h.phrase) { x.q += vb; J.phrase.push_back(x); }
    J.nf += h.nf;
  }
  const uint32_t nq = S * nq1;
  for (auto* v : {&J.q_hlo, &J.q_hhi}) v->assign(nq, 0x3F800000u);
  J.q_hsh.assign(nq, 31);
  for (uint32_t i = 0, r = 0; i < nq1; ++i) {
    while (i >= pc.begin(r + 1)) ++r;
    const uint32_t li = i - pc.begin(r);
    uint32_t l = 0, hh = 0;
    bool any = false;
    for (uint32_t s = 0; s < S; ++s) {
      const PlanTables& h = hs[s * P + r];
      if (!h.ngroup[li]) continue;
      l = std::max(l, h.q_hlo[li]);
      hh = std::max(hh, h.q_hhi[li]);
      any = true;
    }
    if (!any) continue;
    const fgh::Bins b = fgh::union_bins(l, hh);
    for (uint32_t s = 0; s < S; ++s) {
      J.q_hlo[s * nq1 + i] = b.lo;
      J.q_hhi[s * nq1 + i] = b.hi;
      J.q_hsh[s * nq1 + i] = b.shift;
    }
  }
  return J;
}

bool single_list(const PlanTables& t, const WItem& x) { return t.q_m[x.q] == fg::qm_pack(1, 1, 0); }

void xcd_groups(const PlanTables& t, uint32_t nq, std::vector<uint8_t>& q_grp) {
  q_grp.assign(nq, 0);
  auto probe_term = [&](uint32_t qv) { return t.q_terms[(size_t)qv * fg::kMaxTerms]; };
  static thread_local std::vector<uint64_t> ka, kb;
  ka.clear();
  for (uint32_t v = 0; v < nq; ++v)
    if (t.ngroup[v] && fg::qm_must(t.q_m[v]) && t.q_m[v] != fg::qm_pack(1, 1, 0))
      ka.push_back(((uint64_t)probe_term(v) << 32) | v);
  radix_sort_hi32(ka, kb);
  std::vector<std::pair<uint64_t, uint32_t>> by;
  for (size_t i = 0; i < ka.size();) {
    size_t j = i;
    uint64_t c = 0;
    for (; j < ka.size() && (ka[j] >> 32) == (ka[i] >> 32); ++j) c += t.ngroup[(uint32_t)ka[j]];
    by.emplace_back(c, (uint32_t)i);
    i = j;
  }
  std::sort(by.begin(), by.end(), [&](auto& a, auto& b) {
    return a.first > b.first || (a.first == b.first && (ka[a.second] >> 32) < (ka[b.second] >> 32));
  });
  uint64_t gl[8] = {0, 0, 0, 0, 0, 0, 0, 0};
  for (auto& [c, i0] : by) {
    const uint32_t g = (uint32_t)(std::min_element(gl, gl + 8) - gl);
    gl[g] += c;
    for (size_t j = i0; j < ka.size() && (ka[j] >> 32) == (ka[i0] >> 32); ++j) q_grp[(uint32_t)ka[j]] = (uint8_t)g;
  }
}

void sort_sweep(std::vector<WItem>& items, bool conj, const PlanTables& t, uint32_t nq) {
  const size_t n = items.size();
  static thread_local std::vector<uint64_t> a, bb;
  a.resize(n);
  std::vector<uint8_t> q_grp;
  if (conj) xcd_groups(t, nq, q_grp);
  for (size_t x = 0; x < n; ++x) {
    const double kk = std::min(std::max(items[x].key, 0.0), 1.0);
    const bool single = single_list(t, items[x]);
    const uint32_t sw = conj && !single ? ((uint32_t)q_grp[items[x].q] << 28) | (uint32_t)(kk * 268435455.0)
                                        : (uint32_t)(kk * 2147483647.0);
    const uint32_t rk = (conj && single ? 0u : 0x80000000u) | sw;
    a[x] = ((uint64_t)rk << 32) | (uint64_t)x;
  }
  radix_sort_hi32(a, bb);
  static thread_local std::vector<WItem> sorted;
  sorted.resize(n);
  for (size_t x = 0; x < n; ++x) sorted[x] = items[(uint32_t)a[x]];
  items.swap(sorted);
}

struct WorkList {
  std::vector<uint32_t> work_q, work_c, work_n;
  std::vector<uint64_t> cand_off;
  uint64_t n_single = 0, n_conj = 0, n_main = 0, n_scan = 0, n_phrase = 0;
  uint64_t count() const { return n_main + n_scan + n_phrase; }
};

int order_items(PlanTables& t, uint32_t nq, uint32_t k, WorkList& w) {
  if (t.f_woff[t.nf] * 4 > (8ull << 30)) return fail(FG_EUNSUPPORTED, "facet masks of this batch exceed 8 GiB");
  if (t.ch_f.size() > 0x7FFFFFFFull) return fail(FG_EUNSUPPORTED, "facet postings of this batch too large");
  if (t.citems.size() + t.ditems.size() + t.scan.size() + t.phrase.size() > 0x7FFFFFFFull)
    return fail(FG_EUNSUPPORTED, "batch too large (%zu work items)",
                t.citems.size() + t.ditems.size() + t.scan.size() + t.phrase.size());
  sort_sweep(t.citems, true, t, nq);
  sort_sweep(t.ditems, false, t, nq);
  auto& items = t.items;
  items.reserve(t.citems.size() + t.ditems.size() + t.scan.size() + t.phrase.size());
  items.insert(items.end(), t.citems.begin(), t.citems.end());
  w.n_conj = t.citems.size();
  items.insert(items.end(), t.ditems.begin(), t.ditems.end());
  w.n_single = 0;
  for (const WItem& x : t.citems) w.n_single += single_list(t, x) ? 1 : 0;
  std::stable_sort(t.scan.begin(), t.scan.end(), [](const WItem& a, const WItem& b) { return a.key < b.key; });
  w.n_main = items.size();
  w.n_scan = t.scan.size();
  std::stable_sort(t.phrase.begin(), t.phrase.end(), [](const WItem& a, const WItem& b) { return a.key < b.key; });
  w.n_phrase = t.phrase.size();
  const uint64_t chunks = w.count();
  if (chunks > 0x7FFFFFFFull) return fail(FG_EUNSUPPORTED, "batch too large (%llu work items)", (unsigned long long)chunks);
  items.insert(items.end(), t.scan.begin(), t.scan.end());
  items.insert(items.end(), t.phrase.begin(), t.phrase.end());
  w.work_q.resize(chunks);
  w.work_c.resize(chunks);
  w.work_n.resize(chunks);
  w.cand_off.assign(nq + 1, 0);
  for (uint64_t x = 0; x < chunks; ++x) {
    w.work_q[x] = items[x].q;
    w.work_c[x] = items[x].c;
    w.work_n[x] = items[x].n;
  }
  for (uint32_t i = 0; i < nq; ++i) w.cand_off[i + 1] = w.cand_off[i] + (uint64_t)t.ngroup[i] * k;
  return FG_OK;
}

struct Layout {
  struct Region { size_t off, bytes; const void* src; void* field; void (*bind)(void* field, char* addr); };
  std::vector<Region> regions;
  size_t end = 0;
  size_t add(size_t bytes) {
    const size_t o = end;
    end += (bytes + 255) & ~size_t(255);
    return o;
  }
  template <class T>
  size_t in(T*& field, const void* src, size_t bytes, size_t slot = 0) {
    auto bind = [](void* f, char* a) { *static_cast<T**>(f) = reinterpret_cast<T*>(a); };
    regions.push_back(Region{end, bytes, src, &field, bind});
    return add(std::max(bytes, slot));
  }
  template <class T> size_t out(T*& field, size_t bytes) { return in(field, nullptr, bytes); }
  void place(char* base, char* staging) const {
    for (const Region& r : regions) {
      if (r.src && r.bytes) std::memcpy(staging + r.off, r.src, r.bytes);
      r.bind(r.field, base + r.off);
    }
  }
};

int stage_and_upload(fg_plan* p, fg_index* const* ixs, PlanTables& t, const WorkList& w, bool sync, hipStream_t up) {
  fg_index* ix = ixs[0];
  const uint32_t S = p->n_segs, nq = p->nq, nq1 = p->nq_batch, k = p->k, nf = t.nf;
  const uint64_t chunks = w.count();
  const size_t nch = t.ch_f.size(), nqt = (size_t)nq * fg::kMaxTerms;
  std::vector<uint32_t> seg_base;
  if (S > 1) {
    uint64_t b = 0;
    for (uint32_t x = 0; x < S; ++x) {
      seg_base.push_back((uint32_t)std::min<uint64_t>(b, 0xFFFFFFFFull));
      b += ixs[x]->n_docs;
    }
    if (b > 0xFFFFFFFFull) seg_base.clear();
  }
  std::vector<uint32_t> cache_of(S, 0);
  for (uint32_t x = 0; x < S; ++x) {
    uint32_t c = 0;
    while (c < x && std::memcmp(ixs[cache_of[c]]->cache, ixs[x]->cache, sizeof ixs[x]->cache) != 0) ++c;
    cache_of[x] = c < x ? cache_of[c] : x;
  }
  Layout L;
  L.regions.reserve(48);
  fg::DevPlan& d = p->d;
  std::vector<fg::DevIndex> segs(S > 1 ? S : 0);
  L.in(d.q_m, t.q_m.data(), 4ull * nq);
  L.in(d.q_terms, t.q_terms.data(), 4 * nqt);
  L.in(d.q_lead_df, t.lead.data(), 4ull * nq);
  L.in(d.work_q, w.work_q.data(), 4ull * chunks);
  L.in(d.work_c, w.work_c.data(), 4ull * chunks);
  L.in(d.work_n, w.work_n.data(), 4ull * chunks);
  L.in(d.cand_off, w.cand_off.data(), 8ull * (nq + 1));
  L.in(d.q_thr0, t.thr0.data(), 8ull * nq);
  L.in(d.q_ub, t.q_ub.data(), 4 * nqt);
  L.in(d.q_probe, t.q_probe.data(), sizeof(fg::ProbeDesc) * nqt);
  L.in(d.q_wt, t.q_wt.data(), 4 * nqt);
  L.in(d.q_wn, t.q_wn.data(), 4 * nqt);
  L.in(d.q_rup, t.q_rup.data(), 4 * nqt);
  L.in(d.q_pterm, t.q_pterm.data(), 4 * t.q_pterm.size());
  L.in(d.q_ppos, t.q_ppos.data(), 4 * t.q_ppos.size());
  const size_t o_cache = L.add(4ull * 512 * S);
  L.in(d.f.q_filter, t.q_filter.data(), 4ull * nq);
  L.in(d.f.f_shift, t.f_shift.data(), 4ull * nf);
  L.in(d.f.f_woff, t.f_woff.data(), 8ull * nf);
  L.in(d.f.f_tab, t.f_tab.data(), 4ull * nf * 256);
  L.in(d.f.f_max, t.f_max.data(), 4ull * nf);
  L.in(d.f.ch_filter, t.ch_f.data(), 4ull * nch);
  L.in(d.f.ch_clause, t.ch_c.data(), 4ull * nch);
  L.in(d.f.ch_term, t.ch_t.data(), 4ull * nch);
  L.in(d.f.ch_start, t.ch_s.data(), 4ull * nch);
  L.in(d.q_hlo, t.q_hlo.data(), 4ull * nq);
  L.in(d.q_hsh, t.q_hsh.data(), 4ull * nq);
  if (S > 1) {
    L.in(d.f.f_seg, t.f_seg.data(), 4ull * nf);
    L.in(d.segs, segs.data(), sizeof(fg::DevIndex) * S);
    L.in(d.seg_base, seg_base.data(), 4ull * seg_base.size(), 4ull * S);
  }
  const size_t s_in = L.end;
  L.out(d.thresh, 8ull * nq1);
  L.out(d.cand_cnt, 4ull * nq);
  L.out(d.f.fmask, 4ull * t.f_woff[nf]);
  L.out(d.hist, 4ull * nq1 * fg::kQBins);
  const size_t s_zero = L.end - s_in;
  L.out(d.cand_keys, 8ull * w.cand_off[nq]);
  L.out(p->own_score, 4ull * nq * k);
  L.out(p->own_doc, 4ull * nq * k);
  L.out(p->own_n, 4ull * nq);
#ifdef FG_DIAG
  const size_t o_dg = L.out(d.diag, 8ull * fg::kDiagPerWg * (chunks + nq));
  p->diag_words = (L.end - o_dg) / 8;
#endif
  const size_t total = L.end;

  HIPCHK(hipSetDevice(ix->dev));
  char* base = static_cast<char*>(ix->pool->get(std::max<size_t>(total, 256), &p->ws_got));
  if (!base) return fail(FG_EOOM, "plan workspace hipMalloc(%zu) failed", total);
  p->ws = base;
  p->ix = ix;
  fg_index_retain(ix);
  for (uint32_t s = 1; s < S; ++s) {
    fg_index_retain(ixs[s]);
    p->segs.push_back(ixs[s]);
  }
  p->ws_bytes = total;
  const size_t s_up = s_in + (s_zero <= (64u << 10) ? s_zero : 0);
  PinnedLease pin(*ix->pinned, s_up);
  std::vector<char> staging_pageable;
  char* staging = static_cast<char*>(pin.p);
  if (!staging) {
    staging_pageable.assign(s_up, 0);
    staging = staging_pageable.data();
  } else if (s_up > s_in) {
    std::memset(staging + s_in, 0, s_up - s_in);
  }
  std::vector<const float*> d_cache(S, nullptr);
  for (uint32_t x = 0, n = 0; x < S; ++x) {
    if (cache_of[x] != x) continue;
    std::memcpy(staging + o_cache + 4ull * 512 * n, ixs[x]->cache, 4ull * 512);
    d_cache[x] = (const float*)(base + o_cache + 4ull * 512 * n++);
  }
  for (uint32_t x = 0; x < S; ++x) d_cache[x] = d_cache[cache_of[x]];
  p->d0 = ix->d;
  p->d0.cache = d_cache[0];
  for (uint32_t s = 0; s < S && S > 1; ++s) {
    segs[s] = ixs[s]->d;
    segs[s].cache = d_cache[s];
  }
  L.place(base, staging);
  if (seg_base.empty()) d.seg_base = nullptr;
  if (!p->diag_words) d.diag = nullptr;
  p->zero_region = base + s_in;
  p->zero_bytes = s_zero;
  HIPCHK(hipMemcpyAsync(base, staging, s_up, hipMemcpyHostToDevice, up));
  p->up_stream = up;
  p->zeroed = s_up > s_in;
  if (sync || !pin.p) {
    HIPCHK(hipStreamSynchronize(up));
  } else {
    p->pin = pin.p;
    p->pin_n = pin.n;
    pin.p = nullptr;
  }
  return FG_OK;
}

void fill_view(fg_plan* p, fg_index* const* ixs, PlanTables& t, const WorkList& w) {
  const uint32_t S = p->n_segs, nq = p->nq, nq1 = p->nq_batch;
  p->d.n_queries = nq;
  p->d.total_chunks = (uint32_t)w.n_main;
  p->d.n_conj = (uint32_t)w.n_conj;
  p->d.n_scan = (uint32_t)w.n_scan;
  p->d.n_phrase = (uint32_t)w.n_phrase;
  p->d.n_single = (uint32_t)w.n_single;
  p->d.k = p->k;
  p->d.seg_nq = S > 1 ? nq1 : 0;
  p->d.n_segs = S;
  p->d.feat = 0;
  for (uint32_t x = 0; x < S; ++x)
    if (!ixs[x]->same_stats) p->d.feat = 4u;
  for (uint32_t x = 0; x < S && p->d.feat; ++x)
    p->d.feat |= (ixs[x]->d.tfn_name ? 1u : 0u) | (ixs[x]->d.n_esc ? 2u : 0u);
  p->d.pub_mask = S > 1 ? 0xFFFFFFFF00000000ull : ~0ull;
  p->d.opts = fgh::conj_hist_thr() ? fg::kOptConjHistThr : 0u;
  p->h_any.assign(nq1, 0);
  for (uint32_t v = 0; v < nq; ++v)
    if (t.ngroup[v]) p->h_any[v % nq1] = 1;
  p->h_lo.swap(t.q_hlo);
  p->h_hi.swap(t.q_hhi);
  p->d.f.n_filters = t.nf;
  p->d.f.n_chunks = (uint32_t)t.ch_f.size();
}

}

int fgh::plan_create_multi(fg_index* const* ixs, uint32_t S, const fg_query_batch* q, uint32_t k, fg_plan** out,
                           bool sync, hipStream_t up) {
  if (!out) return fail(FG_EINVAL, "bad arguments");
  static const bool ptrace = getenv("FUGU_SHARD_TRACE") != nullptr;
  auto pnow = [] { return std::chrono::duration<double, std::milli>(std::chrono::steady_clock::now().time_since_epoch()).count(); };
  double pt[5] = {ptrace ? pnow() : 0.0, 0, 0, 0, 0};
  static thread_local std::vector<PlanTables> hs_tl;
  static thread_local PlanTables J_tl;
  static thread_local WorkList w_tl;
  Pieces pc;
  if (int rc = plan_pieces(ixs, S, q, k, hs_tl, J_tl, pc)) return rc;
  if (ptrace) pt[1] = pnow();
  PlanTables& t = join_pieces(pc, hs_tl, J_tl);
  if (ptrace) pt[2] = pnow();
  const uint32_t nq1 = pc.nq1, nq = S * nq1;
  WorkList& w = w_tl;
  if (int rc = order_items(t, nq, k, w)) return rc;
  if (ptrace) pt[3] = pnow();
  auto p = std::make_unique<fg_plan>();
  p->nq = nq;
  p->nq_batch = nq1;
  p->n_segs = S;
  p->k = k;
  p->mode = q->mode;
  p->total_chunks = (uint32_t)w.count();
  p->n_scan = (uint32_t)w.n_scan;
  p->mem.dev = ixs[0]->dev;
  if (int rc = stage_and_upload(p.get(), ixs, t, w, sync, up)) return rc;
  fill_view(p.get(), ixs, t, w);
  if (ptrace && S > 1) {
    pt[4] = pnow();
    fprintf(stderr, "[fg plan] %u snapshots x %u queries: plan_host %.3f join %.3f items %.3f stage+upload %.3f ms\n", S,
            nq1, pt[1] - pt[0], pt[2] - pt[1], pt[3] - pt[2], pt[4] - pt[3]);
  }
  *out = p.release();
  return FG_OK;
}

int fg_plan_create(fg_index* ix, const fg_query_batch* q, uint32_t k, fg_plan** out) {
  return fgh::plan_create_multi(&ix, 1, q, k, out, true, hipStreamPerThread);
}

int fg_plan_create_multi(fg_index* const* ixs, uint32_t n_segs, const fg_query_batch* q, uint32_t k, fg_plan** out) {
  return fgh::plan_create_multi(ixs, n_segs, q, k, out, true, hipStreamPerThread);
}
```

fugu_amd/native.py:

```python
from __future__ import annotations

import ctypes as C
import os
from dataclasses import dataclass

import numpy as np

import torch

_HERE = os.path.dirname(os.path.abspath(__file__))
LIB_PATH = os.environ.get("FUGU_LIB") or os.path.join(_HERE, "libfugu.so")

FG_OK = 0
FG_EINVAL = -1
FG_ENODEV = -2
FG_EOOM = -3
FG_EHIP = -4
FG_EUNSUPPORTED = -5
FG_MAX_TERMS = 16
FG_MAX_FACET_CLAUSES = 8
FG_MAX_K = 1024
FG_TERM_MISSING = 0xFFFFFFFF
FG_MAX_COUNT_TERMS = 1 << 20
FG_MAX_COUNT_CELLS = 1 << 25
# ... 81 lines not shown
    _fields_ = [("n_docs", C.c_uint32), ("n_terms", C.c_uint32), ("n_postings", C.c_uint64),
                ("device_bytes", C.c_uint64), ("tot_tokens", C.c_uint64 * 2), ("avgdl", C.c_float * 2),
                ("has_name", C.c_int), ("device", C.c_int), ("n_facet_terms", C.c_uint32),
                ("tot_facet_tokens", C.c_uint64), ("n_dense_f32", C.c_uint32), ("n_rank_terms", C.c_uint32),
                ("n_sparse_rank_terms", C.c_uint32), ("has_positions", C.c_uint32), ("rank_bytes", C.c_uint64)]


class ModelOut(C.Structure):
    _fields_ = [(n, C.c_double) for n in ("stream_bytes", "probe_bytes", "output_bytes", "alg_bytes", "line_bytes",
                                          "query_line_bytes", "loads", "candidates")]


class PlanIpc(C.Structure):
    _fields_ = [("handle", C.c_uint8 * 64), ("thresh_off", C.c_uint64), ("hist_off", C.c_uint64),
                ("n_queries", C.c_uint32), ("k", C.c_uint32), ("device", C.c_int), ("reserved", C.c_uint32)]


class PlanInfo(C.Structure):
    _fields_ = [("n_queries", C.c_uint32), ("k", C.c_uint32), ("total_chunks", C.c_uint32),
                ("workspace_bytes", C.c_uint64)]


def _sig(name, res, *args):
    f = getattr(_lib, name)
    f.restype = res
    f.argtypes = list(args)
    return f


_sig("fg_device_count", C.c_int, C.POINTER(C.c_int))
_sig("fg_ctx_create", C.c_int, C.c_int, C.POINTER(C.c_int), C.POINTER(_p))
_sig("fg_ctx_destroy", C.c_int, _p)
_sig("fg_ctx_peer_access", C.c_int, _p, C.c_int, C.c_int, C.POINTER(C.c_int))
_sig("fg_plan_link", C.c_int, C.POINTER(_p), C.c_uint32)
_sig("fg_bytes_model_or", C.c_int, _p, C.POINTER(QueryBatch), C.c_uint32, _f32p, _f64p)
_sig("fg_last_error", C.c_char_p)
_sig("fg_version", C.c_char_p)
_sig("fg_index_build_from_docs", C.c_int, _p, C.c_int, C.POINTER(DocsInput), C.POINTER(_p))
_sig("fg_index_build", C.c_int, _p, C.c_int, C.POINTER(IndexInput), C.POINTER(_p))
_sig("fg_index_build_global", C.c_int, _p, C.c_int, C.POINTER(IndexInput), C.POINTER(GlobalStats), C.POINTER(_p))
if hasattr(_lib, "fg_index_build_positional"):
    _sig("fg_index_build_positional", C.c_int, _p, C.c_int, C.POINTER(IndexInput), C.POINTER(PositionsInput),
         C.POINTER(GlobalStats), C.POINTER(_p))
    _sig("fg_index_positions_get", C.c_int, _p, C.c_int, C.c_uint32, C.c_uint32, _u64p, _u32p, C.c_uint64, _u64p)
_sig("fg_docs_stats", C.c_int, C.POINTER(DocsInput), _u32p, _u32p, _u64p)
_sig("fg_docs_facet_stats", C.c_int, C.POINTER(DocsInput), _u32p, _u64p)
_sig("fg_index_build_from_docs_global", C.c_int, _p, C.c_int, C.POINTER(DocsInput), C.POINTER(GlobalStats),
     C.POINTER(_p))
_sig("fg_index_rescore", C.c_int, _p, C.POINTER(GlobalStats), _u8p, C.POINTER(_p))
_sig("fg_index_rescore_many", C.c_int, C.POINTER(_p), C.c_uint32, C.POINTER(GlobalStats), C.POINTER(_u8p),
     C.POINTER(_p))
_sig("fg_index_retain", C.c_int, _p)
_sig("fg_thread_background", C.c_int, C.c_int)
_sig("fg_index_release", C.c_int, _p)
_sig("fg_index_stats_get", C.c_int, _p, C.POINTER(IndexStats))
_sig("fg_index_doctab_get", C.c_int, _p, _u32p, _u64p)
if hasattr(_lib, "fg_index_doctab8_get"):
    _sig("fg_index_doctab8_get", C.c_int, _p, _u32p, _u64p)
_sig("fg_index_df", C.c_uint64, _p, C.c_int, C.c_uint32)
_sig("fg_index_bm25", C.c_int, _p, C.c_uint32, _f32p, _f32p, _f32p)
_sig("fg_plan_create", C.c_int, _p, C.POINTER(QueryBatch), C.c_uint32, C.POINTER(_p))
_sig("fg_plan_create_multi", C.c_int, C.POINTER(_p), C.c_uint32, C.POINTER(QueryBatch), C.c_uint32, C.POINTER(_p))
_sig("fg_plan_execute_merged", C.c_int, _p, _p, _p, _p, _p, _p)
_sig("fg_index_term_kth", C.c_int, _p, C.c_uint32, _f32p)
_sig("fg_index_term_ladder", C.c_int, _p, _f32p)
_sig("fg_kth_floor_combine", C.c_int, C.c_uint32, C.c_uint32, C.POINTER(_f32p), _f32p)
_sig("fg_index_set_kth_floor", C.c_int, _p, _f32p, C.c_uint32)
_sig("fg_plan_execute", C.c_int, _p, _p, _p, _p, _p)
_sig("fg_plan_results", C.c_int, _p, _f32p, _u32p, _u32p)
_sig("fg_plan_hist_span", C.c_int, _p, _u32p, _u32p)
_sig("fg_plan_set_hist_span", C.c_int, _p, _u32p, _u32p)
_sig("fg_plan_execute_part", C.c_int, _p, _p, C.c_double, C.c_double, _p, _p, _p, _p)
_sig("fg_plan_hist_copy", C.c_int, _p, _p, _p, C.c_int)
_sig("fg_plan_set_peers", C.c_int, _p, C.POINTER(_p), C.c_uint32)
_sig("fg_plan_ipc_export", C.c_int, _p, C.POINTER(PlanIpc))
_sig("fg_plan_set_ipc_peers", C.c_int, _p, C.POINTER(PlanIpc), C.c_uint32)
_sig("fg_plan_reset", C.c_int, _p, _p)
_sig("fg_plan_info_get", C.c_int, _p, C.POINTER(PlanInfo))
_sig("fg_plan_profile", C.c_int, _p, C.c_int)
_sig("fg_plan_kernel_ms", C.c_int, _p, _f64p, _u32p)
_sig("fg_plan_diag", C.c_int, _p, _u64p, C.c_size_t, _u32p)
if hasattr(_lib, "fg_plan_seed_thr0"):
    _sig("fg_plan_seed_thr0", C.c_int, _p, _f32p, C.c_uint32)
_sig("fg_plan_destroy", C.c_int, _p)
_sig("fg_search_batch", C.c_int, _p, C.POINTER(QueryBatch), C.c_uint32, _f32p, _u32p, _u32p)
_sig("fg_search_sharded", C.c_int, _p, C.POINTER(_p), C.c_uint32, C.POINTER(QueryBatch), C.c_uint32, _f32p, _u32p,
     _u32p, _u32p)
_sig("fg_merge_shards", C.c_int, C.c_uint32, C.c_uint32, C.c_uint32, _p, _p, _p, _p, _p, _p, _p, _p)
_sig("fg_bytes_model", C.c_int, _p, C.POINTER(QueryBatch), C.c_uint32, _f64p)
_sig("fg_bytes_model_gpu", C.c_int, _p, C.POINTER(QueryBatch), C.c_uint32, _f64p)
_sig("fg_model_batch", C.c_int, _p, C.POINTER(QueryBatch), C.c_uint32, _f32p, _f64p, C.POINTER(ModelOut))
_sig("fg_count_batch", C.c_int, C.POINTER(_p), C.c_uint32, C.POINTER(QueryBatch), _u32p, C.c_uint32, _u64p, _u64p)
_sig("fg_count_trace", C.c_int, C.c_int, _f64p, _u32p)
_sig("fg_abi_version", C.c_int)
if _lib.fg_abi_version() != ABI_VERSION:
    raise ImportError(f"{LIB_PATH} has ABI {_lib.fg_abi_version()}, this binding follows {ABI_VERSION}: rebuild")


class FuguError(RuntimeError):
    def __init__(self, code: int, msg: str):
        super().__init__(f"libfugu error {code}: {msg}")
        self.code = code


class Unsupported(FuguError):
    """FG_EUNSUPPORTED: the query is outside the device subset (host CPU path)."""


def _check(rc: int):
    if rc != FG_OK:
        msg = (_lib.fg_last_error() or b"").decode(errors="replace")
        if rc == FG_EUNSUPPORTED:
            raise Unsupported(rc, msg)
        raise FuguError(rc, msg)


def _ptr(a, t):
    return a.ctypes.data_as(t) if a is not None else None


def lib():
    return _lib


def version() -> str:
    return _lib.fg_version().decode()


def device_count() -> int:
    n = C.c_int(0)
    _check(_lib.fg_device_count(C.byref(n)))
    return n.value


class Context:
    def __init__(self, devices=(0,)):
        devs = (C.c_int * len(devices))(*devices)
        h = _p()
        _check(_lib.fg_ctx_create(len(devices), devs, C.byref(h)))
        self._h = h
        self.devices = tuple(devices)

    @property
    def handle(self):
        return self._h

    def peer_access(self, a: int, b: int) -> bool:
        e = C.c_int(0)
        _check(_lib.fg_ctx_peer_access(self._h, a, b, C.byref(e)))
        return bool(e.value)

    def close(self):
        if self._h:
            _lib.fg_ctx_destroy(self._h)
            self._h = None

    def __del__(self):
        try:
            self.close()
        except Exception:
            pass


@dataclass
class Stats:
    n_docs: int
# ... 345 lines not shown
            self.n_segs = 1
            _check(_lib.fg_plan_create(index.handle, C.byref(qb), k, C.byref(h)))
        self.n_batch = qb.n_queries
        self.n_queries = qb.n_queries * self.n_segs
        self._h = h
        self.index = index

    def info(self) -> PlanInfo:
        i = PlanInfo()
        _check(_lib.fg_plan_info_get(self._h, C.byref(i)))
        return i

    def execute(self, stream: int | None = None, out_score: int | None = None, out_doc: int | None = None,
                out_n: int | None = None):
        _check(_lib.fg_plan_execute(self._h, stream, out_score, out_doc, out_n))

    def execute_merged(self, stream: int | None, out_score: int, out_doc: int, out_shard: int, out_n: int):
        _check(_lib.fg_plan_execute_merged(self._h, stream, out_score, out_doc, out_shard, out_n))

    def execute_part(self, stream: int | None, frm: float, to: float, out_score: int | None = None,
                     out_doc: int | None = None, out_shard: int | None = None, out_n: int | None = None):
        _check(_lib.fg_plan_execute_part(self._h, stream, frm, to, out_score, out_doc, out_shard, out_n))

    def hist_span(self):
        lo = np.zeros(self.n_batch, np.uint32)
        hi = np.zeros(self.n_batch, np.uint32)
        _check(_lib.fg_plan_hist_span(self._h, _ptr(lo, _u32p), _ptr(hi, _u32p)))
        return lo, hi

    def set_hist_span(self, lo, hi):
        lo = np.ascontiguousarray(lo, np.uint32)
        hi = np.ascontiguousarray(hi, np.uint32)
        if lo.shape != (self.n_batch,) or hi.shape != (self.n_batch,):
            raise ValueError(f"spans of {lo.shape} / {hi.shape}, expected ({self.n_batch},)")
        _check(_lib.fg_plan_set_hist_span(self._h, _ptr(lo, _u32p), _ptr(hi, _u32p)))

    def hist_copy(self, stream: int | None, d_buf: int, into_plan: bool):
        _check(_lib.fg_plan_hist_copy(self._h, stream, d_buf, 1 if into_plan else 0))

    def set_peers(self, peers):
        hs = (_p * max(len(peers), 1))(*[x._h for x in peers])
        self._peers = list(peers)
        _check(_lib.fg_plan_set_peers(self._h, hs, len(peers)))

    def ipc_export(self) -> bytes:
        x = PlanIpc()
        _check(_lib.fg_plan_ipc_export(self._h, C.byref(x)))
        return bytes(x)

    def set_ipc_peers(self, blobs):
        arr = (PlanIpc * max(len(blobs), 1))()
        for i, b in enumerate(blobs):
            if len(b) != C.sizeof(PlanIpc):
                raise ValueError(f"peer {i}: {len(b)} bytes, expected {C.sizeof(PlanIpc)}")
            C.memmove(C.byref(arr, i * C.sizeof(PlanIpc)), b, len(b))
        _check(_lib.fg_plan_set_ipc_peers(self._h, arr, len(blobs)))

    def reset(self, stream: int | None = None):
        _check(_lib.fg_plan_reset(self._h, stream))

    def results(self):
        nq, k = self.n_queries, self.k
        score = np.zeros(nq * k, np.float32)
        doc = np.zeros(nq * k, np.uint32)
        n = np.zeros(nq, np.uint32)
        _check(_lib.fg_plan_results(self._h, _ptr(score, _f32p), _ptr(doc, _u32p), _ptr(n, _u32p)))
        return score.reshape(nq, k), doc.reshape(nq, k), n

    def profile(self, enable: bool = True):
        _check(_lib.fg_plan_profile(self._h, 1 if enable else 0))

    def kernel_ms(self):
        ms = np.zeros(2, np.float64)
        n = C.c_uint32(0)
        _check(_lib.fg_plan_kernel_ms(self._h, _ptr(ms, _f64p), C.byref(n)))
        return ms, n.value

    def seed_thresholds(self, score):
        s = np.ascontiguousarray(score, np.float32)
        if s.shape != (self.n_batch,):
            raise ValueError(f"scores of {s.shape}, expected ({self.n_batch},)")
        _check(_lib.fg_plan_seed_thr0(self._h, _ptr(s, _f32p), self.n_batch))

    def candidate_counts(self):
        cnt = np.zeros(self.n_queries, np.uint32)
        _check(_lib.fg_plan_diag(self._h, None, 0, _ptr(cnt, _u32p)))
        return cnt

    def diag(self):
        info = self.info()
        n = DIAG_PER_WG * (info.total_chunks + self.n_queries)
        out = np.zeros(n, np.uint64)
        _check(_lib.fg_plan_diag(self._h, _ptr(out, _u64p), n, None))
        w = out.reshape(-1, DIAG_PER_WG)
        return w[: info.total_chunks], w[info.total_chunks:]

    def close(self):
        if self._h:
            _lib.fg_plan_destroy(self._h)
            self._h = None

    def __del__(self):
        try:
            self.close()
        except Exception:
            pass


def kth_floor_combine(ladders) -> np.ndarray:
    ls = [np.ascontiguousarray(x, np.float32) for x in ladders]
    if not ls:
        raise ValueError("no ladders")
    V = ls[0].shape[0]
    for x in ls:
        if x.shape != (V, len(LADDER_KS)):
            raise ValueError(f"ladder shape {x.shape}, expected ({V}, {len(LADDER_KS)})")
    arr = (_f32p * len(ls))(*[_ptr(x, _f32p) for x in ls])
    out = np.zeros((V, len(KTH_KS)), np.float32)
    _check(_lib.fg_kth_floor_combine(len(ls), V, arr, _ptr(out, _f32p)))
    return out


def link_plans(plans):
    hs = (_p * len(plans))(*[p._h for p in plans])
    _check(_lib.fg_plan_link(hs, len(plans)))


def search_sharded(indexes, q_off, terms, k: int, mode: int = MODE_AND, f_off=None, f_terms=None, ctx=None,
                   occur=None, phrase_len=None, phrase_pos=None):
    qb, keep = _batch(q_off, terms, mode, f_off, f_terms, occur, phrase_len, phrase_pos)
    nq = qb.n_queries
    hs = (_p * len(indexes))(*[ix._h for ix in indexes])
    score = np.zeros(nq * k, np.float32)
    doc = np.zeros(nq * k, np.uint32)
    shard = np.zeros(nq * k, np.uint32)
    n = np.zeros(nq, np.uint32)
    _check(_lib.fg_search_sharded(ctx._h if ctx is not None else None, hs, len(indexes), C.byref(qb), k,
                                  _ptr(score, _f32p), _ptr(doc, _u32p), _ptr(shard, _u32p), _ptr(n, _u32p)))
    return score.reshape(nq, k), doc.reshape(nq, k), shard.reshape(nq, k), n


def count_batch(indexes, q_off, terms, count_terms=(), mode: int = MODE_AND, f_off=None, f_terms=None, occur=None,
                phrase_len=None, phrase_pos=None):
    qb, keep = _batch(q_off, terms, mode, f_off, f_terms, occur, phrase_len, phrase_pos)
    nq = qb.n_queries
    ct = _u32(count_terms)
    hs = (_p * len(indexes))(*[ix._h for ix in indexes])
    total = np.zeros(nq, np.uint64)
    count = np.zeros(nq * len(ct), np.uint64)
    _check(_lib.fg_count_batch(hs, len(indexes), C.byref(qb), _ptr(ct, _u32p) if len(ct) else None, len(ct),
                               _ptr(total, _u64p), _ptr(count, _u64p) if len(ct) else None))
    return total, count.reshape(nq, len(ct))


COUNT_KERNELS = ("k_cfilter", "k_cmatch", "k_ccount", "k_cfacet")


def count_trace(enable: int = -1):
    ms = np.zeros(4, np.float64)
    n = C.c_uint32(0)
    _check(_lib.fg_count_trace(enable, _ptr(ms, _f64p), C.byref(n)))
    return dict(zip(COUNT_KERNELS, ms.tolist())), n.value


def merge_shards(n_shards: int, n_queries: int, k: int, d_score: int, d_doc: int, d_n: int, d_out_score: int,
                 d_out_doc: int, d_out_shard: int | None, d_out_n: int, stream: int | None = None):
# ... 3 lines not shown
```

Baseline: 1.194 million queries/s.

## Add dense doctab8 sweep kernel for high-df conjunctive queries

Adds an alternative execution path for multi-term AND queries whose lead term is very frequent. It streams the 8-bit per-document quantized score tables of all terms in coalesced 128-bit loads. A udot4 weighted sum against the current threshold screens documents, and only survivors are queued for exact BM25 probing and top-k truncation. The path is gated by FUGU_DENSE_DIV, which defaults to 0, so it stays off unless enabled. The same change also makes the existing doctab8 bound on the second term opt-in through FUGU_DOCTAB8_LEAD, which alters default pruning behaviour.

```diff
diff --git a/fugu_amd/csrc/fg_host.h b/fugu_amd/csrc/fg_host.h
--- a/fugu_amd/csrc/fg_host.h
+++ b/fugu_amd/csrc/fg_host.h
@@ -385,6 +385,24 @@
   const auto it = std::lower_bound(b.dtab8_map.begin(), b.dtab8_map.end(), (uint64_t)t << 32);
   return it != b.dtab8_map.end() && (uint32_t)(*it >> 32) == t ? (uint32_t)*it + 1u : 0u;
 }
+
+inline bool doctab8_bound() {
+  const char* e = getenv("FUGU_DOCTAB8_LEAD");
+  return e && *e;
+}
+
+inline uint32_t dense_div() {
+  const char* e = getenv("FUGU_DENSE_DIV");
+  return e && *e ? (uint32_t)std::max(0l, atol(e)) : fg::kDenseDiv;
+}
+inline uint32_t dense_min_terms() {
+  const char* e = getenv("FUGU_DENSE_MIN_TERMS");
+  return e && *e ? (uint32_t)std::min(4l, std::max(2l, atol(e))) : fg::kDenseMinTerms;
+}
+inline uint32_t dense_passes() {
+  const char* e = getenv("FUGU_DENSE_PASSES");
+  return e && *e ? (uint32_t)std::min(65536l, std::max(1l, atol(e))) : fg::kDensePasses;
+}
 }
 
 struct fg_index : fgh::IndexStructure, fgh::IndexBounds {
@@ -412,9 +430,25 @@
   std::shared_ptr<PinnedPool> pinned;
 };
 
+namespace fgh {
+inline bool dense_sweep(const fg_index* ix, const uint32_t* qt, uint32_t mt, uint32_t nm, bool filtered, bool qtime,
+                        uint32_t div, uint32_t* slots) {
+  if (!div || qtime || filtered || nm != mt || mt < dense_min_terms() || mt > fg::kDenseMaxTerms) return false;
+  if (!ix->d.dtab8 || ix->dtab8_map.empty()) return false;
+  if ((ix->off[qt[0] + 1] - ix->off[qt[0]]) * (uint64_t)div < ix->n_docs) return false;
+  float M[fg::kDenseMaxTerms];
+  for (uint32_t j = 0; j < mt; ++j) {
+    if (!(slots[j] = doctab8_slot(*ix, qt[j]))) return false;
+    M[j] = ix->tmaxs[qt[j]];
+  }
+  return fg::dense_cut_make(M, mt).inv > 0.0f;
+}
+}
+
 struct fg_plan {
   fg_index* ix = nullptr;
   uint32_t nq = 0, k = 0, total_chunks = 0, n_scan = 0, nq_batch = 0, n_segs = 1;
+  uint32_t n_dense_slots = 0;
   std::vector<fg_index*> segs;
   int mode = FG_MODE_AND;
   fg::DevPlan d{};
@@ -467,6 +501,7 @@
 };
 
 extern "C" int fg_plan_seed_thr0(fg_plan* p, const float* score, uint32_t n);
+extern "C" int fg_plan_dense_get(const fg_plan* p, uint32_t* n_items, uint32_t* n_slots);
 
 namespace fgh {
 inline uint32_t local_term(const fg_index* ix, uint32_t t) {
diff --git a/fugu_amd/csrc/fg_internal.h b/fugu_amd/csrc/fg_internal.h
--- a/fugu_amd/csrc/fg_internal.h
+++ b/fugu_amd/csrc/fg_internal.h
@@ -62,6 +62,21 @@
 #endif
 constexpr uint32_t kDocTab8Div = FG_DOCTAB8_DIV;
 constexpr uint32_t kDocTab8Lead = FG_DOCTAB8_LEAD;
+#ifndef FG_DENSE_DIV
+#define FG_DENSE_DIV 0
+#endif
+#ifndef FG_DENSE_PASSES
+#define FG_DENSE_PASSES 8
+#endif
+#ifndef FG_DENSE_MIN_TERMS
+#define FG_DENSE_MIN_TERMS 2
+#endif
+constexpr uint32_t kDenseMinTerms = FG_DENSE_MIN_TERMS;
+constexpr uint32_t kDenseDiv = FG_DENSE_DIV;
+constexpr uint32_t kDensePasses = FG_DENSE_PASSES;
+constexpr uint32_t kDenseDwords = 4;
+constexpr uint32_t kDensePass = 256 * kDenseDwords * 4;
+constexpr uint32_t kDenseMaxTerms = 4;
 constexpr uint32_t kRankChunkWords = 2048;
 #ifndef FG_DISJ_GPQ
 #define FG_DISJ_GPQ 64
@@ -186,6 +201,50 @@
   return q;
 }
 constexpr uint32_t kSubShift = 9;
+
+struct DenseCut {
+  uint32_t w;
+  float inv;
+};
+__host__ __device__ inline float dense_key_score(uint64_t k) {
+  union { float f; uint32_t u; } c;
+  c.u = (uint32_t)(k >> 32);
+  return c.f;
+}
+inline DenseCut dense_cut_make(const float* M, uint32_t m) {
+  DenseCut c{0u, 0.0f};
+  if (m < 1 || m > kDenseMaxTerms) return c;
+  double W = 0.0;
+  for (uint32_t i = 0; i < m; ++i) {
+    if (!(M[i] >= 1e-30f && M[i] <= 1e30f)) return c;
+    W = std::max(W, (double)M[i]);
+  }
+  for (uint32_t i = 0; i < m; ++i) {
+    const double r = 255.0 * (double)M[i] / W * (1.0 + 1e-12);
+    uint32_t w = (uint32_t)r;
+    if ((double)w < r) ++w;
+    c.w |= std::min(std::max(w, 1u), 255u) << (8 * i);
+  }
+  c.inv = (float)(255.0 * 255.0 / W * (1.0 - 1.0 / 262144.0));
+  return c;
+}
+__host__ __device__ inline uint32_t dense_cut_T(const DenseCut& c, uint64_t thr) {
+  if (thr == 0 || !(c.inv > 0.0f)) return 0u;
+  const float x = dense_key_score(thr) * c.inv;
+  return x < 1.0e9f ? (uint32_t)x : 1000000000u;
+}
+__host__ __device__ inline uint32_t dense_cut_sum(uint32_t w, uint32_t bytes) {
+#if defined(__HIP_DEVICE_COMPILE__) && __has_builtin(__builtin_amdgcn_udot4)
+  return __builtin_amdgcn_udot4(bytes, w, 0u, false);
+#else
+  return (bytes & 0xFFu) * (w & 0xFFu) + ((bytes >> 8) & 0xFFu) * ((w >> 8) & 0xFFu) +
+         ((bytes >> 16) & 0xFFu) * ((w >> 16) & 0xFFu) + (bytes >> 24) * (w >> 24);
+#endif
+}
+__host__ __device__ inline bool dense_present(uint32_t bytes, uint32_t m) {
+  const uint32_t x = bytes | (m >= 4 ? 0u : 0xFFFFFFFFu << (8 * m));
+  return (((x - 0x01010101u) & ~x) & 0x80808080u) == 0u;
+}
 
 __host__ __device__ inline uint32_t meta_slot(uint32_t meta) { return (meta >> 16) & 0x7FFFu; }
 __host__ __device__ inline bool meta_rank(uint32_t meta) { return (meta >> 31) != 0; }
@@ -382,6 +441,13 @@
 constexpr uint32_t kMaxPeers = 15;
 constexpr uint32_t kOptConjHistThr = 1u;
 
+struct DenseQuery {
+  uint32_t tab_lo[kDenseMaxTerms];
+  uint32_t tab_hi[2];
+  DenseCut cut;
+};
+static_assert(sizeof(DenseQuery) == 32, "one s_load_dwordx8");
+
 struct DevPlan {
   uint32_t n_queries;
   uint32_t total_chunks;
@@ -413,6 +479,8 @@
   uint32_t n_single;
   uint32_t n_scan;
   uint32_t n_phrase;
+  uint32_t n_dense;
+  const DenseQuery* q_dense;
   const uint32_t* q_pterm;
   const uint32_t* q_ppos;
   const DevIndex* segs;
@@ -591,6 +659,7 @@
 hipError_t launch_conj(const DevIndex& ix, const DevPlan& pl, hipStream_t s);
 hipError_t launch_disj(const DevIndex& ix, const DevPlan& pl, hipStream_t s, uint32_t first = 0,
                        uint32_t count = 0xFFFFFFFFu);
+hipError_t launch_dense(const DevIndex& ix, const DevPlan& pl, hipStream_t s);
 hipError_t launch_fmask(const DevIndex& ix, const DevPlan& pl, hipStream_t s);
 hipError_t launch_scan(const DevIndex& ix, const DevPlan& pl, hipStream_t s);
 hipError_t launch_phrase(const DevIndex& ix, const DevPlan& pl, hipStream_t s);
diff --git a/fugu_amd/csrc/fugu.cpp b/fugu_amd/csrc/fugu.cpp
--- a/fugu_amd/csrc/fugu.cpp
+++ b/fugu_amd/csrc/fugu.cpp
@@ -771,6 +771,7 @@
   }
   if (first && p->d.f.n_chunks) HIPCHK(fg::launch_fmask(p->d0, p->d, s));
   if (first && p->d.n_conj) HIPCHK(fg::launch_conj(p->d0, p->d, s));
+  if (first && p->d.n_dense) HIPCHK(fg::launch_dense(p->d0, p->d, s));
   const uint32_t nd = p->d.total_chunks - p->d.n_conj;
   const uint32_t a = first ? 0u : (uint32_t)std::min<double>(nd, std::llround(from * nd));
   const uint32_t b = last ? nd : (uint32_t)std::min<double>(nd, std::llround(to * nd));
@@ -1019,6 +1020,13 @@
     if (!p->d.diag) return fail(FG_EUNSUPPORTED, "not a diagnostic build (-DFG_DIAG)");
     HIPCHK(hipMemcpy(out, p->d.diag, 8 * std::min(n_words, p->diag_words), hipMemcpyDeviceToHost));
   }
+  return FG_OK;
+}
+
+int fg_plan_dense_get(const fg_plan* p, uint32_t* n_items, uint32_t* n_slots) {
+  if (!p) return fail(FG_EINVAL, "NULL plan");
+  if (n_items) *n_items = p->d.n_dense;
+  if (n_slots) *n_slots = p->n_dense_slots;
   return FG_OK;
 }
 
diff --git a/fugu_amd/csrc/kernels.hip b/fugu_amd/csrc/kernels.hip
--- a/fugu_amd/csrc/kernels.hip
+++ b/fugu_amd/csrc/kernels.hip
@@ -48,6 +48,10 @@
   return (uint64_t)v[0] | ((uint64_t)v[1] << 32);
 }
 __device__ inline uint32_t buf_u32(BufRsrc r, uint32_t off) { return __builtin_amdgcn_raw_buffer_load_b32(r, (int)off, 0, 0); }
+__device__ inline void buf_u128(BufRsrc r, uint32_t off, uint32_t (&o)[4]) {
+  const auto v = __builtin_amdgcn_raw_buffer_load_b128(r, (int)off, 0, 0);
+  o[0] = v[0]; o[1] = v[1]; o[2] = v[2]; o[3] = v[3];
+}
 __device__ inline uint32_t buf_u16(BufRsrc r, uint32_t off) { return __builtin_amdgcn_raw_buffer_load_b16(r, (int)off, 0, 0); }
 __device__ inline uint32_t buf_u8(BufRsrc r, uint32_t off) { return __builtin_amdgcn_raw_buffer_load_b8(r, (int)off, 0, 0); }
 #else
@@ -55,6 +59,7 @@
 __device__ inline BufRsrc pd_rsrc(uint64_t, uint32_t) { return 0; }
 __device__ inline uint64_t buf_u64(BufRsrc, uint32_t) { return 0; }
 __device__ inline uint32_t buf_u32(BufRsrc, uint32_t) { return 0; }
+__device__ inline void buf_u128(BufRsrc, uint32_t, uint32_t (&o)[4]) { o[0] = o[1] = o[2] = o[3] = 0; }
 __device__ inline uint32_t buf_u16(BufRsrc, uint32_t) { return 0; }
 __device__ inline uint32_t buf_u8(BufRsrc, uint32_t) { return 0; }
 #endif
@@ -896,6 +901,249 @@
   __syncthreads();
   for (uint32_t i = 0; i < 8; ++i) FG_STAMP(w, 8 + i, sh.dgc[i]);
 #endif
+}
+
+constexpr uint32_t kDenseQueue = 1536;
+constexpr uint32_t kDenseFlush = 512;
+constexpr uint32_t kDenseR = 4;
+constexpr uint32_t kDenseBuf = kTrunc + kDenseQueue;
+static_assert(kDenseFlush + kThreads * 4 <= kDenseQueue, "a quarter pass after a queue just short of a flush fits");
+static_assert(kDensePass == kThreads * kDenseDwords * 4, "a pass: kDenseDwords dwords of 4 docs per lane");
+
+struct DenseShared {
+  alignas(16) uint64_t buf[kDenseBuf];
+  uint32_t hist[1u << kConjHistBits];
+  uint32_t scratch[8];
+  uint32_t n_buf;
+  uint64_t thr;
+  uint32_t q[kDenseQueue];
+  uint32_t n_q;
+};
+
+__device__ void dense_flush(const DevIndex& ix, DenseShared& sh, const ProbeDesc* probes, const uint32_t* terms,
+                            uint32_t m, uint64_t thr, uint32_t nd) {
+  const uint32_t tid = threadIdx.x;
+#pragma unroll 1
+  for (uint32_t e0 = 0; e0 < nd; e0 += kDenseR * kThreads) {
+  uint32_t doc[kDenseR], live = 0;
+  float s01[kDenseR], acc[kDenseR];
+#pragma unroll
+  for (uint32_t r = 0; r < kDenseR; ++r) {
+    const uint32_t i = e0 + r * kThreads + tid;
+    doc[r] = i < nd ? sh.q[i] : kInvalid;
+    s01[r] = 0.0f;
+    acc[r] = 0.0f;
+    live |= (doc[r] != kInvalid ? 1u : 0u) << r;
+  }
+  for (uint32_t i = 0; i < m; ++i) {
+    if (!__any(live != 0)) break;
+    float sc[kDenseR];
+    const ProbeDesc pd = probe_load(probes + (i ? i : m));
+    probe_list<kDenseR, 0u>(ix, pd, terms + i, doc, live, 0.0f, 0.0f, nullptr, nullptr, sc);
+#pragma unroll
+    for (uint32_t r = 0; r < kDenseR; ++r) {
+      if (!((live >> r) & 1u)) continue;
+      if (sc[r] < 0.0f) live &= ~(1u << r);
+      else if (i == 0) s01[r] = sc[r];
+      else if (i == 1) s01[r] = s01[r] + sc[r];
+      else acc[r] += sc[r];
+    }
+    if (thr != 0 && i + 1 < m) {
+      const float ub = __uint_as_float(pd.ub);
+#pragma unroll
+      for (uint32_t r = 0; r < kDenseR; ++r)
+        if ((live & (1u << r)) && make_key(inflate_bound(s01[r] + acc[r] + ub), doc[r]) < thr) live &= ~(1u << r);
+    }
+  }
+#pragma unroll
+  for (uint32_t r = 0; r < kDenseR; ++r) {
+    bool keep = (live >> r) & 1u;
+    uint64_t key = 0;
+    if (keep && ix.alive && !((ix.alive[doc[r] >> 5] >> (doc[r] & 31)) & 1u)) keep = false;
+    if (keep) {
+      key = make_key(s01[r] + acc[r], doc[r]);
+      keep = key >= thr;
+    }
+    wave_append(keep, key, sh.buf, &sh.n_buf, kDenseBuf);
+  }
+  }
+}
+
+template <bool kMulti>
+__global__ __launch_bounds__(kThreads, FG_WAVES) void k_dense(DevIndex ix0, DevPlan pl) {
+  __shared__ DenseShared sh;
+  const uint32_t tid = threadIdx.x, lane = lane_id();
+  const uint32_t nwg = gridDim.x, bid = blockIdx.x;
+  const uint32_t xcd = bid & 7, q8 = nwg >> 3, r8 = nwg & 7;
+  const uint32_t w = pl.total_chunks + pl.n_scan + pl.n_phrase +
+                     (xcd < r8 ? xcd * (q8 + 1) : r8 * (q8 + 1) + (xcd - r8) * q8) + (bid >> 3);
+  const uint32_t q = pl.work_q[w];
+  const DevIndex ix = kMulti ? seg_index(pl, __builtin_amdgcn_readfirstlane(q / pl.seg_nq)) : ix0;
+  const uint32_t ql = kMulti ? __builtin_amdgcn_readfirstlane(q % pl.seg_nq) : q;
+  const uint32_t p0 = pl.work_c[w], np = pl.work_n[w];
+  const uint32_t m = qm_terms(pl.q_m[q]);
+  const uint32_t* terms = pl.q_terms + (size_t)q * kMaxTerms;
+  const ProbeDesc* probes = pl.q_probe + (size_t)q * kMaxTerms;
+  static_assert(sizeof(DenseQuery) == sizeof(ProbeDesc), "probe_load's scalar load");
+  const ProbeDesc dw = probe_load(reinterpret_cast<const ProbeDesc*>(pl.q_dense + q));
+  const uint32_t tab_lo[kDenseMaxTerms] = {dw.base_lo, dw.bytes, dw.sc_lo, dw.sc_bytes};
+  const uint32_t tab_hi[kDenseMaxTerms] = {dw.aux_lo & 0xFFFFu, dw.aux_lo >> 16, dw.hi & 0xFFFFu, dw.hi >> 16};
+  DenseCut cut;
+  cut.w = dw.kind;
+  cut.inv = __uint_as_float(dw.ub);
+  const uint32_t K = pl.k;
+  unsigned long long* gthr = reinterpret_cast<unsigned long long*>(&pl.thresh[ql]);
+  const uint64_t thr0 = pl.q_thr0[q];
+  uint64_t pend = 0;
+  uint32_t* const gh = pl.hist + (size_t)ql * kQBins;
+  const uint32_t h_lo = pl.q_hlo[q], h_sh = pl.q_hsh[q];
+  if (tid == 0) {
+    sh.n_buf = 0;
+    sh.n_q = 0;
+    sh.thr = thr0;
+    pend = atomicMax(gthr, (unsigned long long)(thr0 & pl.pub_mask));
+    peer_thr_max(pl, ql, thr0);
+  }
+  uint64_t local_T = 0, thr_k = thr0;
+  const uint32_t stride = ix.dtab8_stride;
+
+  uint32_t n_held = 0;
+
+  auto drain = [&](uint32_t nd, bool end) {
+    if (nd < kDenseFlush && !end) return nd;
+    if (nd) {
+      const uint32_t n = min(sh.n_buf, kDenseBuf);
+      if (n > kTrunc) {
+        local_T = truncate_keys<kDenseBuf, kConjHistBits>(sh.buf, &sh.n_buf, sh.hist, sh.scratch, n, K);
+        if (local_T > thr_k) thr_k = local_T;
+      }
+      dense_flush(ix, sh, probes, terms, m, thr_k, nd);
+      __syncthreads();
+      if (tid == 0) sh.n_q = 0;
+    }
+    const uint32_t n = min(sh.n_buf, kDenseBuf);
+    if (n > kTrunc || (end && n > K)) {
+      local_T = truncate_keys<kDenseBuf, kConjHistBits>(sh.buf, &sh.n_buf, sh.hist, sh.scratch, n, K);
+      if (local_T > thr_k) thr_k = local_T;
+    }
+    __syncthreads();
+    return 0u;
+  };
+
+  auto load_pass = [&](uint32_t pp, uint32_t (&o)[kDenseMaxTerms][kDenseDwords]) {
+    const uint32_t d0 = (p0 + pp) * kDensePass;
+    const uint32_t span = pp < np && d0 < stride ? min(kDensePass, stride - d0) : 0u;
+#pragma unroll
+    for (uint32_t i = 0; i < kDenseMaxTerms; ++i)
+      buf_u128(pd_rsrc((((uint64_t)tab_hi[i] << 32) | tab_lo[i]) + d0, i < m ? span : 0u), tid << 4, o[i]);
+  };
+  uint32_t v[kDenseMaxTerms][kDenseDwords];
+  load_pass(0, v);
+  if (tid == 0 && pend > sh.thr) sh.thr = pend;
+
+  for (uint32_t pp = 0; pp < np; ++pp) {
+    const uint32_t d0 = (p0 + pp) * kDensePass;
+    auto test = [&](uint32_t j, uint32_t a0, uint32_t a1, uint32_t a2, uint32_t a3, uint32_t T) {
+      uint32_t b[4];
+#if defined(__HIP_DEVICE_COMPILE__)
+      const uint32_t t0 = __builtin_amdgcn_perm(a1, a0, 0x05010400u), t1 = __builtin_amdgcn_perm(a1, a0, 0x07030602u);
+      const uint32_t u0 = __builtin_amdgcn_perm(a3, a2, 0x05010400u), u1 = __builtin_amdgcn_perm(a3, a2, 0x07030602u);
+      b[0] = __builtin_amdgcn_perm(u0, t0, 0x05040100u);
+      b[1] = __builtin_amdgcn_perm(u0, t0, 0x07060302u);
+      b[2] = __builtin_amdgcn_perm(u1, t1, 0x05040100u);
+      b[3] = __builtin_amdgcn_perm(u1, t1, 0x07060302u);
+#else
+      for (uint32_t x = 0; x < 4; ++x)
+        b[x] = ((a0 >> (8 * x)) & 0xFFu) | (((a1 >> (8 * x)) & 0xFFu) << 8) | (((a2 >> (8 * x)) & 0xFFu) << 16) |
+               (((a3 >> (8 * x)) & 0xFFu) << 24);
+#endif
+      bool ge[4];
+#pragma unroll
+      for (uint32_t x = 0; x < 4; ++x) ge[x] = dense_cut_sum(cut.w, b[x]) >= T;
+      if (!__any(ge[0] || ge[1] || ge[2] || ge[3])) return;
+      const uint32_t d = d0 + (tid << 4) + (j << 2);
+#pragma unroll
+      for (uint32_t x = 0; x < 4; ++x) {
+        const bool on = ge[x] && dense_present(b[x], m);
+        const unsigned long long bal = __ballot(on);
+        const uint32_t nw = (uint32_t)__popcll(bal);
+        if (!nw) continue;
+        uint32_t base = 0;
+        if (lane == 0) base = atomicAdd(&sh.n_q, nw);
+        base = (uint32_t)__shfl((int)base, 0, 64);
+        const uint32_t at = base + (uint32_t)__popcll(bal & ((1ull << lane) - 1ull));
+        if (on && at < kDenseQueue) sh.q[at] = d + x;
+      }
+    };
+    uint32_t nx[kDenseMaxTerms][kDenseDwords];
+    load_pass(pp + 1, nx);
+    __syncthreads();
+    const uint64_t thr = sh.thr;
+    if (thr > thr_k) thr_k = thr;
+    {
+      const uint32_t T = __builtin_amdgcn_readfirstlane(dense_cut_T(cut, thr_k));
+#pragma unroll
+      for (uint32_t j = 0; j < kDenseDwords; ++j) test(j, v[0][j], v[1][j], v[2][j], v[3][j], T);
+    }
+    __syncthreads();
+    uint32_t nd = sh.n_q;
+    const bool redo = nd > kDenseQueue;
+    if (redo) {
+      __syncthreads();
+      if (tid == 0) sh.n_q = n_held;
+      __syncthreads();
+    }
+    const bool last = pp + 1 == np;
+#pragma unroll 1
+    for (uint32_t j = redo ? 0u : kDenseDwords - 1; j < kDenseDwords; ++j) {
+      if (redo) {
+        const uint32_t span = d0 < stride ? min(kDensePass, stride - d0) : 0u;
+        uint32_t a[kDenseMaxTerms];
+#pragma unroll
+        for (uint32_t i = 0; i < kDenseMaxTerms; ++i)
+          a[i] = buf_u32(pd_rsrc((((uint64_t)tab_hi[i] << 32) | tab_lo[i]) + d0, i < m ? span : 0u), (tid << 4) + (j << 2));
+        test(j, a[0], a[1], a[2], a[3], __builtin_amdgcn_readfirstlane(dense_cut_T(cut, thr_k)));
+        __syncthreads();
+        nd = min(sh.n_q, kDenseQueue);
+        __syncthreads();
+      }
+      n_held = drain(nd, last && j + 1 == kDenseDwords);
+    }
+    if (tid == 0) {
+      if (pend > sh.thr) sh.thr = pend;
+      if (local_T > sh.thr) sh.thr = local_T;
+      pend = atomicMax(gthr, (unsigned long long)(local_T & pl.pub_mask));
+    }
+#pragma unroll
+    for (uint32_t i = 0; i < kDenseMaxTerms; ++i)
+#pragma unroll
+      for (uint32_t j = 0; j < kDenseDwords; ++j) v[i][j] = nx[i][j];
+  }
+  if (tid == 0 && pend > sh.thr) sh.thr = pend;
+  {
+    const uint32_t n = min(sh.n_buf, kDenseBuf);
+    for (uint32_t b = tid; b < kQBins; b += kThreads) sh.hist[b] = 0;
+    __syncthreads();
+    for (uint32_t i = tid; i < n; i += kThreads) {
+      const uint32_t b = qbin(sh.buf[i], h_lo, h_sh);
+      if (b < kQBins) atomicAdd(&sh.hist[b], 1u);
+    }
+    __syncthreads();
+    if (pl.opts & kOptConjHistThr) {
+      const uint64_t cur = sh.thr;
+      const uint32_t cb = qbin(cur, h_lo, h_sh);
+      const uint64_t edge = hist_add_kth(sh.hist, gh, pl, ql, cur && cb < kQBins ? cb : 0u, K, h_lo, h_sh, sh.scratch);
+      if (tid == 0 && edge > cur) {
+        sh.thr = edge;
+        atomicMax(gthr, (unsigned long long)(edge & pl.pub_mask));
+      }
+    } else {
+      hist_add(sh.hist, gh, pl, ql);
+    }
+  }
+  if (tid == 0) peer_thr_max(pl, ql, sh.thr);
+  __syncthreads();
+  flush_candidates(pl, q, sh.buf, sh.n_buf, sh.thr, sh.scratch);
 }
 
 constexpr uint32_t kTileShift = kDisjTileShift;
@@ -2191,6 +2439,14 @@
   return hipGetLastError();
 }
 
+hipError_t launch_dense(const DevIndex& ix, const DevPlan& pl, hipStream_t s) {
+  if (pl.n_dense == 0) return hipSuccess;
+  if (pl.feat & kFQt) return hipErrorInvalidValue;
+  if (pl.segs) k_dense<true><<<pl.n_dense, kThreads, 0, s>>>(ix, pl);
+  else k_dense<false><<<pl.n_dense, kThreads, 0, s>>>(ix, pl);
+  return hipGetLastError();
+}
+
 hipError_t launch_final(const DevPlan& pl, float* out_score, uint32_t* out_doc, uint32_t* out_n, hipStream_t s,
                         uint32_t* out_shard) {
   const bool merged = out_shard != nullptr;
diff --git a/fugu_amd/csrc/model.cpp b/fugu_amd/csrc/model.cpp
--- a/fugu_amd/csrc/model.cpp
+++ b/fugu_amd/csrc/model.cpp
@@ -24,6 +24,9 @@
   uint32_t pw = 2;
   uint32_t tab_lead = 0;
   uint32_t tab8_lead = 0;
+  bool tab8_bound = false;
+  uint32_t dense_div = 0;
+  mutable std::atomic<uint64_t> dense_passed{0};
   std::vector<float> psc, tmax, bmax, cmax;
   std::vector<uint64_t> tsub, srank;
   std::vector<uint32_t> dir_off, toff, coff;
@@ -106,6 +109,8 @@
     tab_lead = fgh::doctab_lead();
     bytes[A_DTAB8] = x->dtab8_bytes;
     tab8_lead = fgh::doctab8_lead();
+    tab8_bound = fgh::doctab8_bound();
+    dense_div = fgh::dense_div();
     return FG_OK;
   }
   template <class Acc>
@@ -294,6 +299,46 @@
       qub[j] = acc;
     }
   }
+  uint32_t sl8[fg::kDenseMaxTerms];
+  if (has_thr && fgh::dense_sweep(ix, terms, m, m, false, !ix->same_stats, S.dense_div, sl8)) {
+    float M[fg::kDenseMaxTerms];
+    const uint32_t* l[fg::kDenseMaxTerms];
+    uint64_t n[fg::kDenseMaxTerms], c[fg::kDenseMaxTerms] = {0}, b0[fg::kDenseMaxTerms];
+    uint32_t tab[fg::kDenseMaxTerms] = {0};
+    for (uint32_t j = 0; j < m; ++j) {
+      M[j] = ix->tmaxs[terms[j]];
+      l[j] = S.list(terms[j]);
+      n[j] = S.len(terms[j]);
+      b0[j] = ix->off[terms[j]];
+      A.range(j, A_DTAB8, (uint64_t)(sl8[j] - 1) * ix->d.dtab8_stride, ix->d.dtab8_stride, 1, A.stream);
+      const uint32_t s4 = ix->dtab_map.empty() ? 0u : fgh::doctab_slot(*ix, terms[j]);
+      if (s4 && fg::probe_uses_table(ix->n_docs, n[j], df, S.tab_lead)) tab[j] = s4;
+    }
+    const fg::DenseCut cut = fg::dense_cut_make(M, m);
+    const uint32_t T = fg::dense_cut_T(cut, thk);
+    for (uint64_t p = 0; p < df; ++p) {
+      const uint32_t d = ld[p];
+      uint32_t bytes = 0;
+      bool all = true;
+      for (uint32_t j = 0; j < m && all; ++j) {
+        while (c[j] < n[j] && l[j][c[j]] < d) ++c[j];
+        all = c[j] < n[j] && l[j][c[j]] == d;
+        if (all) bytes |= std::max(1u, fg::quant8(S.psc[b0[j] + c[j]], M[j])) << (8 * j);
+      }
+      if (!all || fg::dense_cut_sum(cut.w, bytes) < T) continue;
+      S.dense_passed.fetch_add(1, std::memory_order_relaxed);
+      float s0 = 0.0f, acc = 0.0f;
+      bool ok = true;
+      for (uint32_t j = 0; j < m && ok; ++j) {
+        const float sc = probe_term(S, A, j, terms[j], d, A.probe, tab[j]);
+        if (sc < 0.0f) { ok = false; break; }
+        if (j == 0) s0 = sc; else if (j == 1) s0 = s0 + sc; else acc += sc;
+        if (thk && j + 1 < m && key_of((s0 + acc + qub[j + 1]) * kInflate, d) < thk) ok = false;
+      }
+      if (ok && key_of(s0 + acc, d) >= thk) ++kept;
+    }
+    return kept;
+  }
   A.range(0, A_DOC, base, df, 4, A.stream);
   A.range(0, A_TFN, base, df, S.pw, A.stream);
   uint32_t tab[fg::kMaxTerms] = {0};
@@ -304,7 +349,7 @@
     }
   uint32_t tab8 = 0;
   float M8 = 0.0f;
-  if (ix->same_stats && !ix->dtab8_map.empty() && m >= 3 && thk) {
+  if (S.tab8_bound && ix->same_stats && !ix->dtab8_map.empty() && m >= 3 && thk) {
     const uint32_t sl = fgh::doctab8_slot(*ix, terms[1]);
     M8 = ix->tmaxs[terms[1]];
     const uint32_t k1 = fg::meta_slot(ix->tmeta[terms[1]]) ? 0u : fg::kPdDir;
@@ -618,6 +663,7 @@
   out->alg_bytes = out->stream_bytes + out->probe_bytes + out->output_bytes;
   out->line_bytes = (double)kLine * (double)U.count();
   if (trace) {
+    fprintf(stderr, "[fg model] dense sweep: %llu docs past the integer test\n", (unsigned long long)S.dense_passed.load());
     static const char* names[A_N] = {"doc", "tfn", "rank", "srank", "srankw", "dir", "bmax", "tmax", "tdir", "cmax", "tsub", "dtab", "dtab8"};
     for (uint32_t a = 0; a < A_N; ++a)
       fprintf(stderr, "[fg model] %-6s floor %8.3f GB  per-query sum %8.3f GB\n", names[a],
diff --git a/fugu_amd/csrc/plan.cpp b/fugu_amd/csrc/plan.cpp
--- a/fugu_amd/csrc/plan.cpp
+++ b/fugu_amd/csrc/plan.cpp
@@ -35,16 +35,17 @@
   std::vector<uint64_t> thr0;
   std::vector<float> q_ub, q_wt, q_wn, q_rup;
   std::vector<fg::ProbeDesc> q_probe;
+  std::vector<fg::DenseQuery> q_dense;
   uint32_t nf = 0;
   std::vector<uint32_t> f_shift, f_seg;
   std::vector<uint64_t> f_woff;
   std::vector<float> f_tab, f_max;
   std::vector<uint32_t> ch_f, ch_c, ch_t, ch_s;
-  std::vector<WItem> citems, ditems, scan, phrase, items;
+  std::vector<WItem> citems, ditems, scan, phrase, dense, items;
   void clear() {
     auto all = [](auto&... v) { (v.clear(), ...); };
     all(q_m, q_terms, lead, q_filter, ngroup, q_hlo, q_hhi, q_hsh, thr0, q_ub, q_wt, q_wn, q_rup, f_shift, f_seg, f_woff,
-        f_tab, f_max, ch_f, ch_c, ch_t, ch_s, citems, ditems, scan, phrase, items, q_pterm, q_ppos, q_probe);
+        f_tab, f_max, ch_f, ch_c, ch_t, ch_s, citems, ditems, scan, phrase, dense, items, q_pterm, q_ppos, q_probe, q_dense);
     nf = 0;
   }
 };
@@ -130,6 +131,8 @@
   const uint64_t N = ix->n_docs;
   const bool disj = q->mode == FG_MODE_OR;
   const uint32_t tab_lead = fgh::doctab_lead(), tab8_lead = fgh::doctab8_lead();
+  const bool tab8_bound = fgh::doctab8_bound();
+  const uint32_t dense_div = fgh::dense_div(), dense_passes = fgh::dense_passes();
   h.clear();
   const size_t nqt = (size_t)nq * fg::kMaxTerms;
   for (auto* v : {&h.q_m, &h.lead}) v->assign(nq, 0);
@@ -343,7 +346,7 @@
         h.q_probe[row + j] =
             fg::probe_desc(ix->d, pt, j == 0, qtime, j + 1 < mt ? h.q_ub[row + j + 1] : 0.0f, lead_df, tab_lead);
       }
-      if (!qtime && !ix->dtab8_map.empty() && mt >= 3 && nm == mt && flt == 0xFFFFFFFFu)
+      if (tab8_bound && !qtime && !ix->dtab8_map.empty() && mt >= 3 && nm == mt && flt == 0xFFFFFFFFu)
         fg::probe_desc_bound(ix->d, h.q_probe[row], h.q_probe[row + 1], fgh::doctab8_slot(*ix, qt[1]), ix->tmaxs[qt[1]],
                              true, qtime, ix->off[qt[1] + 1] - ix->off[qt[1]], lead_df, tab8_lead);
     }
@@ -359,6 +362,31 @@
     }
     const uint64_t df0 = ix->off[qt[0] + 1] - ix->off[qt[0]];
     h.lead[i] = (uint32_t)df0;
+    uint32_t slots8[fg::kDenseMaxTerms];
+    if (fgh::dense_sweep(ix, qt, mt, nm, flt != 0xFFFFFFFFu, qtime, dense_div, slots8)) {
+      const size_t row = (size_t)i * fg::kMaxTerms;
+      if (h.q_dense.empty()) h.q_dense.assign(nq, fg::DenseQuery{});
+      fg::DenseQuery& dq = h.q_dense[i];
+      float M[fg::kDenseMaxTerms];
+      for (uint32_t j = 0; j < mt; ++j) {
+        const uint64_t a = (uint64_t)(uintptr_t)(ix->d.dtab8 + (uint64_t)(slots8[j] - 1) * ix->d.dtab8_stride);
+        dq.tab_lo[j] = (uint32_t)a;
+        dq.tab_hi[j >> 1] |= (uint32_t)((a >> 32) & 0xFFFFu) << (16 * (j & 1));
+        M[j] = ix->tmaxs[qt[j]];
+      }
+      dq.cut = fg::dense_cut_make(M, mt);
+      const uint32_t tab0 = ix->dtab_map.empty() ? 0u : fgh::doctab_slot(*ix, qt[0]);
+      const fg::ProbeTerm pt{ix->off[qt[0]], ix->off[qt[0] + 1], ix->tmeta[qt[0]], ix->dir_off[qt[0]], tab0};
+      h.q_probe[row + mt] = fg::probe_desc(ix->d, pt, false, false, h.q_ub[row + 1], df0, tab_lead);
+      const uint32_t npass = (uint32_t)((N + fg::kDensePass - 1) / fg::kDensePass);
+      const uint32_t ng = (npass + dense_passes - 1) / dense_passes;
+      if (h.dense.size() + ng > 0x7FFFFFFFull)
+        return fail(FG_EUNSUPPORTED, "batch too large (%zu work items)", h.dense.size());
+      h.ngroup[i] = ng;
+      for (uint32_t g = 0; g < ng; ++g)
+        h.dense.push_back(WItem{(double)g, i, g * dense_passes, std::min(dense_passes, npass - g * dense_passes)});
+      continue;
+    }
     const uint32_t nch = (uint32_t)((df0 + fg::kChunk - 1) / fg::kChunk);
     if (h.citems.size() + nch > 0x7FFFFFFFull)
       return fail(FG_EUNSUPPORTED, "batch too large (%zu work items)", h.citems.size());
@@ -408,6 +436,7 @@
   J.q_terms.resize(nqt);
   for (auto* v : {&J.q_ub, &J.q_wt, &J.q_wn, &J.q_rup}) v->resize(nqt);
   J.q_probe.resize(nqt);
+  if (fgh::dense_div()) J.q_dense.assign(nq, fg::DenseQuery{});
   if (q->phrase_len)
     for (auto* v : {&J.q_pterm, &J.q_ppos}) v->resize(nqt);
   auto put_slot = [&](uint32_t p) {
@@ -418,6 +447,7 @@
     cp(J.q_terms, h.q_terms, t0);
     cp(J.q_ub, h.q_ub, t0); cp(J.q_wt, h.q_wt, t0); cp(J.q_wn, h.q_wn, t0); cp(J.q_rup, h.q_rup, t0);
     cp(J.q_probe, h.q_probe, t0);
+    if (!h.q_dense.empty()) cp(J.q_dense, h.q_dense, v0);
     cp(J.q_pterm, h.q_pterm, t0); cp(J.q_ppos, h.q_ppos, t0);
   };
   if (par) {
@@ -467,6 +497,7 @@
     for (WItem x : h.ditems) { x.q += vb; J.ditems.push_back(x); }
     for (WItem x : h.scan) { x.q += vb; J.scan.push_back(x); }
     for (WItem x : h.phrase) { x.q += vb; J.phrase.push_back(x); }
+    for (WItem x : h.dense) { x.q += vb; J.dense.push_back(x); }
     J.nf += h.nf;
   }
   const uint32_t nq = S * nq1;
@@ -503,7 +534,8 @@
   static thread_local std::vector<uint64_t> ka, kb;
   ka.clear();
   for (uint32_t v = 0; v < nq; ++v)
-    if (t.ngroup[v] && fg::qm_must(t.q_m[v]) && t.q_m[v] != fg::qm_pack(1, 1, 0))
+    if (t.ngroup[v] && fg::qm_must(t.q_m[v]) && t.q_m[v] != fg::qm_pack(1, 1, 0) &&
+        !(v < t.q_dense.size() && t.q_dense[v].cut.w))
       ka.push_back(((uint64_t)probe_term(v) << 32) | v);
   radix_sort_hi32(ka, kb);
   std::vector<std::pair<uint64_t, uint32_t>> by;
@@ -549,16 +581,16 @@
 struct WorkList {
   std::vector<uint32_t> work_q, work_c, work_n;
   std::vector<uint64_t> cand_off;
-  uint64_t n_single = 0, n_conj = 0, n_main = 0, n_scan = 0, n_phrase = 0;
-  uint64_t count() const { return n_main + n_scan + n_phrase; }
+  uint64_t n_single = 0, n_conj = 0, n_main = 0, n_scan = 0, n_phrase = 0, n_dense = 0;
+  uint64_t count() const { return n_main + n_scan + n_phrase + n_dense; }
 };
 
 int order_items(PlanTables& t, uint32_t nq, uint32_t k, WorkList& w) {
   if (t.f_woff[t.nf] * 4 > (8ull << 30)) return fail(FG_EUNSUPPORTED, "facet masks of this batch exceed 8 GiB");
   if (t.ch_f.size() > 0x7FFFFFFFull) return fail(FG_EUNSUPPORTED, "facet postings of this batch too large");
-  if (t.citems.size() + t.ditems.size() + t.scan.size() + t.phrase.size() > 0x7FFFFFFFull)
+  if (t.citems.size() + t.ditems.size() + t.scan.size() + t.phrase.size() + t.dense.size() > 0x7FFFFFFFull)
     return fail(FG_EUNSUPPORTED, "batch too large (%zu work items)",
-                t.citems.size() + t.ditems.size() + t.scan.size() + t.phrase.size());
+                t.citems.size() + t.ditems.size() + t.scan.size() + t.phrase.size() + t.dense.size());
   sort_sweep(t.citems, true, t, nq);
   sort_sweep(t.ditems, false, t, nq);
   auto& items = t.items;
@@ -573,10 +605,13 @@
   w.n_scan = t.scan.size();
   std::stable_sort(t.phrase.begin(), t.phrase.end(), [](const WItem& a, const WItem& b) { return a.key < b.key; });
   w.n_phrase = t.phrase.size();
+  std::stable_sort(t.dense.begin(), t.dense.end(), [](const WItem& a, const WItem& b) { return a.key < b.key; });
+  w.n_dense = t.dense.size();
   const uint64_t chunks = w.count();
   if (chunks > 0x7FFFFFFFull) return fail(FG_EUNSUPPORTED, "batch too large (%llu work items)", (unsigned long long)chunks);
   items.insert(items.end(), t.scan.begin(), t.scan.end());
   items.insert(items.end(), t.phrase.begin(), t.phrase.end());
+  items.insert(items.end(), t.dense.begin(), t.dense.end());
   w.work_q.resize(chunks);
   w.work_c.resize(chunks);
   w.work_n.resize(chunks);
@@ -648,6 +683,7 @@
   L.in(d.q_thr0, t.thr0.data(), 8ull * nq);
   L.in(d.q_ub, t.q_ub.data(), 4 * nqt);
   L.in(d.q_probe, t.q_probe.data(), sizeof(fg::ProbeDesc) * nqt);
+  L.in(d.q_dense, t.q_dense.data(), sizeof(fg::DenseQuery) * (w.n_dense ? t.q_dense.size() : 0));
   L.in(d.q_wt, t.q_wt.data(), 4 * nqt);
   L.in(d.q_wn, t.q_wn.data(), 4 * nqt);
   L.in(d.q_rup, t.q_rup.data(), 4 * nqt);
@@ -745,6 +781,9 @@
   p->d.n_conj = (uint32_t)w.n_conj;
   p->d.n_scan = (uint32_t)w.n_scan;
   p->d.n_phrase = (uint32_t)w.n_phrase;
+  p->d.n_dense = (uint32_t)w.n_dense;
+  p->n_dense_slots = 0;
+  for (uint32_t v = 0; v < nq && w.n_dense; ++v) p->n_dense_slots += t.q_dense[v].cut.w ? 1u : 0u;
   p->d.n_single = (uint32_t)w.n_single;
   p->d.k = p->k;
   p->d.seg_nq = S > 1 ? nq1 : 0;
diff --git a/fugu_amd/native.py b/fugu_amd/native.py
--- a/fugu_amd/native.py
+++ b/fugu_amd/native.py
@@ -187,6 +187,8 @@
 _sig("fg_plan_diag", C.c_int, _p, _u64p, C.c_size_t, _u32p)
 if hasattr(_lib, "fg_plan_seed_thr0"):
     _sig("fg_plan_seed_thr0", C.c_int, _p, _f32p, C.c_uint32)
+if hasattr(_lib, "fg_plan_dense_get"):
+    _sig("fg_plan_dense_get", C.c_int, _p, _u32p, _u32p)
 _sig("fg_plan_destroy", C.c_int, _p)
 _sig("fg_search_batch", C.c_int, _p, C.POINTER(QueryBatch), C.c_uint32, _f32p, _u32p, _u32p)
 _sig("fg_search_sharded", C.c_int, _p, C.POINTER(_p), C.c_uint32, C.POINTER(QueryBatch), C.c_uint32, _f32p, _u32p,
@@ -698,6 +700,11 @@
             raise ValueError(f"scores of {s.shape}, expected ({self.n_batch},)")
         _check(_lib.fg_plan_seed_thr0(self._h, _ptr(s, _f32p), self.n_batch))
 
+    def dense(self):
+        n = np.zeros(2, np.uint32)
+        _check(_lib.fg_plan_dense_get(self._h, _ptr(n[0:1], _u32p), _ptr(n[1:2], _u32p)))
+        return int(n[0]), int(n[1])
+
     def candidate_counts(self):
         cnt = np.zeros(self.n_queries, np.uint32)
         _check(_lib.fg_plan_diag(self._h, None, 0, _ptr(cnt, _u32p)))
```

Result: no change. 1.194 million queries/s (-0.0%).
